# wustl-cig/FLAIR

Measured on AMD Instinct MI355X. Metric: restored frames/sec at 256x256, 16-frame clip, 250-step DDIM, higher is better.
Workload: dtype bf16

## Files before the change

flair_amd/csrc/chain.hip:

```cpp
#include <type_traits>

#include "common.h"
#include "mfma_tile.h"

namespace {

struct ChainArgs {
    const void* x[4];
    int segC[4], segLd[4], nseg;
    unsigned segBytes[4];
    const void* wA; const float* biasA; int actA; int CinA; unsigned wABytes;
    const void* wB; const float* biasB; int actB; int CoutB; unsigned wBBytes;
    const void* res0; const void* res1; int res0Ld, res1Ld;
    float outScale;
    float actParam; int actPeriod;
    void* y; int yLd;
    int T, H, W;
};

template <int N>
__device__ __forceinline__ void act_vec(float (&v)[N], int act) {
    if (act == FLAIR_ACT_SILU) {
#pragma unroll
        for (int e = 0; e < N; ++e) v[e] = silu_f(v[e]);
    } else if (act != FLAIR_ACT_NONE) {
        const float slope = act == FLAIR_ACT_RELU ? 0.f : 0.1f;
#pragma unroll
        for (int e = 0; e < N; ++e) v[e] = fmaxf(v[e], v[e] * slope);
    }
}

constexpr int CHAIN_MAX_COUTB = 512;

template <typename E, int C, int TH, int TW, bool HASA>
__global__ __launch_bounds__(512, 2) void conv_chain_kernel(ChainArgs a) {
    prefetch_kernargs<sizeof(ChainArgs)>();
    constexpr int NT = 512, NW = 8;
    constexpr int BKE = Mma<E>::BKE;
    constexpr int VEC = ET<E>::VEC;
    constexpr unsigned ESZ = sizeof(E);
    constexpr int PITCH = 80;
    constexpr int WM = TW + 2, RM = TH + 2, NPM = RM * WM;
    constexpr int WA = TW + 4, RA = TH + 4, NPA = RA * WA;
    constexpr int NCH = C / BKE;
    constexpr int NB = C / 64;
    constexpr int WROWS = 64 * NB;
    constexpr int MID_BYTES = NCH * NPM * PITCH;
    constexpr int W_BYTES = WROWS * 9 * PITCH;
    constexpr int NGA = (NPM + 31) / 32, NITA = NGA * NB, MAXIA = (NITA + NW - 1) / NW;
    constexpr int NGB = TH * TW / 32, NITB = NGB * NB, MAXIB = (NITB + NW - 1) / NW;
    constexpr int IN_PIECES = (HASA ? NPA : NCH * NPM) * 4;
    constexpr int HI = (IN_PIECES + NT - 1) / NT;
    constexpr int W_PIECES = WROWS * 9 * 4;
    constexpr int WI = (W_PIECES + NT - 1) / NT;
    static_assert(TH * TW % 32 == 0 && C % 64 == 0, "tile");
    extern __shared__ __attribute__((aligned(16))) char smem[];
    char* smid = smem;
    char* sw = smem + MID_BYTES;
    char* sin = sw + W_BYTES;
    float* sbias = reinterpret_cast<float*>(sin + (HASA ? NPA * PITCH : 0));

    const int tid = threadIdx.x, lane = tid & 63, wave = tid >> 6;
    const int lr = lane & 31, lh = lane >> 5;
    const int tilesW = a.W / TW, tilesH = (a.H + TH - 1) / TH;
    const int perFrame = tilesW * tilesH;
    const int bid = xcd_remap(blockIdx.x, gridDim.x);
    const int t = bid / perFrame;
    const int tile = bid % perFrame;
    const int h0 = (tile / tilesW) * TH, w0 = (tile % tilesW) * TW;
    const long frameOff = (long)t * a.H * a.W;
    for (int i = C + tid; i < C + CHAIN_MAX_COUTB; i += NT)
        sbias[i] = (a.biasB && i - C < a.CoutB) ? a.biasB[i - C] : 0.f;

    int ipix[HI], idst[HI];
    unsigned iq[HI];
#pragma unroll
    for (int i = 0; i < HI; ++i) {
        const int id = i * NT + tid;
        constexpr int NP = HASA ? NPA : NPM, WR = HASA ? WA : WM, ORG = HASA ? 2 : 1;
        const int pc = id >> 2;
        const int ch = HASA ? 0 : pc / NP;
        const int pix = HASA ? pc : pc % NP;
        const int r = pix / WR, c = pix % WR;
        const int hh = h0 - ORG + r, ww = w0 - ORG + c;
        const bool ok = id < IN_PIECES && (unsigned)hh < (unsigned)a.H && (unsigned)ww < (unsigned)a.W;
        ipix[i] = ok ? hh * a.W + ww : -1;
        iq[i] = (unsigned)(ch * BKE + (id & 3) * VEC) * ESZ;
        idst[i] = id < IN_PIECES ? (ch * NP + pix) * PITCH + (id & 3) * 16 : -1;
    }
    uint4 hreg[2][HI], wreg[2][WI];

    int seg = 0, cb = 0, segOff = 0;
    auto issue_in = [&](int set) {
        const unsigned ld = (unsigned)a.segLd[seg] * ESZ;
        const char* frame = reinterpret_cast<const char*>(a.x[seg]) + (size_t)frameOff * ld;
        const __amdgpu_buffer_rsrc_t xr = make_rsrc(frame, a.segBytes[seg]);
        const unsigned cofs = (unsigned)(cb * BKE) * ESZ;
#pragma unroll
        for (int i = 0; i < HI; ++i)
            hreg[set][i] = buf_load16(xr, ipix[i] >= 0 ? (unsigned)ipix[i] * ld + cofs + iq[i] : FLAIR_OOB);
    };
    auto advance_in = [&]() {
        ++cb;
        if (cb * BKE >= a.segC[seg]) {
            cb = 0;
            segOff += a.segC[seg];
            ++seg;
        }
    };
    auto issue_w = [&](int set, const __amdgpu_buffer_rsrc_t& wrs, int co0, int coutTot, int cin, int kofs) {
#pragma unroll
        for (int i = 0; i < WI; ++i) {
            const int id = i * NT + tid;
            const int row = id >> 2;
            const int co = row / 9, tap9 = row % 9;
            const bool ok = id < W_PIECES && co0 + co < coutTot;
            wreg[set][i] = buf_load16(wrs, ok ? (unsigned)(((co0 + co) * 9 + tap9) * cin + kofs + (id & 3) * VEC) * ESZ
                                              : FLAIR_OOB);
        }
    };
    auto write_w = [&](int set) {
#pragma unroll
        for (int i = 0; i < WI; ++i) {
            const int id = i * NT + tid;
            if (id < W_PIECES) *reinterpret_cast<uint4*>(sw + (id >> 2) * PITCH + (id & 3) * 16) = wreg[set][i];
        }
    };
    auto write_in = [&](char* dst, int set) {
#pragma unroll
        for (int i = 0; i < HI; ++i)
            if (idst[i] >= 0) *reinterpret_cast<uint4*>(dst + idst[i]) = hreg[set][i];
    };

    auto compute = [&](const char* pb, int inW, const char* wb0, const char* wb1, f32x16 (&acc)[2]) {
        uint4 fa0[2][2], fa1[2][2], fb[2][2];
        auto load_tap = [&](int set, int tap9) {
            const int kh = tap9 / 3, kw = tap9 % 3;
            fa0[set][0] = *reinterpret_cast<const uint4*>(wb0 + tap9 * PITCH + 16 * Mma<E>::chunk(0, lh));
            fa0[set][1] = *reinterpret_cast<const uint4*>(wb0 + tap9 * PITCH + 16 * Mma<E>::chunk(1, lh));
            fa1[set][0] = *reinterpret_cast<const uint4*>(wb1 + tap9 * PITCH + 16 * Mma<E>::chunk(0, lh));
            fa1[set][1] = *reinterpret_cast<const uint4*>(wb1 + tap9 * PITCH + 16 * Mma<E>::chunk(1, lh));
            const char* hp = pb + (kh * inW + kw) * PITCH;
            fb[set][0] = *reinterpret_cast<const uint4*>(hp + 16 * Mma<E>::chunk(0, lh));
            fb[set][1] = *reinterpret_cast<const uint4*>(hp + 16 * Mma<E>::chunk(1, lh));
        };
        load_tap(0, 0);
        __builtin_amdgcn_sched_group_barrier(0x100, 6, 0);
#pragma unroll
        for (int tap9 = 0; tap9 < 9; ++tap9) {
            const int set = tap9 & 1;
            if (tap9 < 8) load_tap(set ^ 1, tap9 + 1);
            Mma<E>::run(fa0[set], fb[set], acc[0]);
            Mma<E>::run(fa1[set], fb[set], acc[1]);
            if (tap9 < 8) __builtin_amdgcn_sched_group_barrier(0x100, 6, 0);
            __builtin_amdgcn_sched_group_barrier(0x8, 2 * Mma<E>::MFMA_PER_STEP, 0);
        }
    };

    const __amdgpu_buffer_rsrc_t wBrs = make_rsrc(a.wB, a.wBBytes);
    const int nBatch = (a.CoutB + WROWS - 1) / WROWS;

    if constexpr (HASA) {
        const __amdgpu_buffer_rsrc_t wArs = make_rsrc(a.wA, a.wABytes);
        const int nkA = a.CinA / BKE;
        auto issue_step = [&](int k, int set) {
            if (k < nkA) {
                issue_in(set);
                issue_w(set, wArs, 0, C, a.CinA, segOff + cb * BKE);
                advance_in();
            } else if (k == nkA) {
                issue_w(set, wBrs, 0, a.CoutB, C, 0);
            }
        };
        issue_step(0, 0);
        issue_step(1, 1);
        f32x16 accA[MAXIA][2];
        int pbOff[MAXIA], wbOff[MAXIA];
#pragma unroll
        for (int ii = 0; ii < MAXIA; ++ii) {
            const int it = wave + ii * NW;
            const int g = it % NGA, blk = (it / NGA) % NB;
            int q = g * 32 + lr;
            if (q >= NPM) q = NPM - 1;
            pbOff[ii] = ((q / WM) * WA + (q % WM)) * PITCH;
            wbOff[ii] = ((blk * 64 + lr) * 9) * PITCH;
#pragma unroll
            for (int i = 0; i < 2; ++i)
#pragma unroll
                for (int gq = 0; gq < 4; ++gq) {
                    float4 bq = make_float4(0.f, 0.f, 0.f, 0.f);
                    if (a.biasA) bq = *reinterpret_cast<const float4*>(a.biasA + blk * 64 + i * 32 + 8 * gq + 4 * lh);
                    accA[ii][i][4 * gq] = bq.x; accA[ii][i][4 * gq + 1] = bq.y;
                    accA[ii][i][4 * gq + 2] = bq.z; accA[ii][i][4 * gq + 3] = bq.w;
                }
        }
        write_in(sin, 0);
        write_w(0);
        __syncthreads();
        auto step = [&](int k, auto setTag) {
            constexpr int SET = decltype(setTag)::value;
            issue_step(k + 2, SET);
#pragma unroll
            for (int ii = 0; ii < MAXIA; ++ii)
                if (wave + ii * NW < NITA)
                    compute(sin + pbOff[ii], WA, sw + wbOff[ii], sw + wbOff[ii] + 32 * 9 * PITCH, accA[ii]);
            __syncthreads();
            if (k + 1 < nkA) write_in(sin, SET ^ 1);
            write_w(SET ^ 1);
            if (k + 1 < nkA) __syncthreads();
        };
        for (int k = 0; k < nkA; k += 2) {
            step(k, std::integral_constant<int, 0>{});
            if (k + 1 < nkA) step(k + 1, std::integral_constant<int, 1>{});
        }
#pragma unroll
        for (int ii = 0; ii < MAXIA; ++ii) {
            const int it = wave + ii * NW;
            if (it >= NITA) continue;
            const int g = it % NGA, blk = (it / NGA) % NB;
            const int q = g * 32 + lr;
            if (q >= NPM) continue;
            const int hh = h0 - 1 + q / WM, ww = w0 - 1 + q % WM;
            const bool inimg = (unsigned)hh < (unsigned)a.H && (unsigned)ww < (unsigned)a.W;
#pragma unroll
            for (int i = 0; i < 2; ++i)
#pragma unroll
                for (int gq = 0; gq < 4; ++gq) {
                    const int co = blk * 64 + i * 32 + 8 * gq + 4 * lh;
                    float v[4] = {accA[ii][i][4 * gq], accA[ii][i][4 * gq + 1], accA[ii][i][4 * gq + 2],
                                  accA[ii][i][4 * gq + 3]};
                    act_vec<4>(v, a.actA);
                    char* dst = smid + ((co / BKE) * NPM + q) * PITCH + (co % BKE) * ESZ;
                    if constexpr (sizeof(E) == 4) {
                        *reinterpret_cast<float4*>(dst) = inimg ? make_float4(v[0], v[1], v[2], v[3])
                                                                : make_float4(0.f, 0.f, 0.f, 0.f);
                    } else {
                        uint2 pk;
                        pk.x = inimg ? pack2bf(v[0], v[1]) : 0u;
                        pk.y = inimg ? pack2bf(v[2], v[3]) : 0u;
                        *reinterpret_cast<uint2*>(dst) = pk;
                    }
                }
        }
        __syncthreads();
    } else {
        issue_in(0);
        issue_w(0, wBrs, 0, a.CoutB, C, 0);
        write_in(smid, 0);
        write_w(0);
        __syncthreads();
    }

    int pbB[MAXIB], wbB[MAXIB];
#pragma unroll
    for (int ii = 0; ii < MAXIB; ++ii) {
        const int it = wave + ii * NW;
        const int g = it % NGB, blk = it / NGB;
        const int q = g * 32 + lr;
        pbB[ii] = ((q / TW) * WM + (q % TW)) * PITCH;
        wbB[ii] = ((blk * 64 + lr) * 9) * PITCH;
    }
    for (int batch = 0; batch < nBatch; ++batch) {
        f32x16 acc[MAXIB][2];
#pragma unroll
        for (int ii = 0; ii < MAXIB; ++ii) {
            const int blk = ((wave + ii * NW) / NGB) % NB;
#pragma unroll
            for (int i = 0; i < 2; ++i)
#pragma unroll
                for (int gq = 0; gq < 4; ++gq) {
                    const float4 bq = *reinterpret_cast<const float4*>(sbias + C + batch * WROWS + blk * 64 + i * 32 +
                                                                       8 * gq + 4 * lh);
                    acc[ii][i][4 * gq] = bq.x; acc[ii][i][4 * gq + 1] = bq.y;
                    acc[ii][i][4 * gq + 2] = bq.z; acc[ii][i][4 * gq + 3] = bq.w;
                }
        }
        for (int ch = 0; ch < NCH; ++ch) {
            const bool lastChunk = ch + 1 == NCH;
            const bool more = !lastChunk || batch + 1 < nBatch;
            if (more) issue_w(0, wBrs, lastChunk ? (batch + 1) * WROWS : batch * WROWS, a.CoutB, C, lastChunk ? 0 : (ch + 1) * BKE);
#pragma unroll
            for (int ii = 0; ii < MAXIB; ++ii)
                if (wave + ii * NW < NITB)
                    compute(smid + ch * NPM * PITCH + pbB[ii], WM, sw + wbB[ii], sw + wbB[ii] + 32 * 9 * PITCH, acc[ii]);
            __syncthreads();
            if (!lastChunk) {
                write_w(0);
                __syncthreads();
            }
        }
#pragma unroll
        for (int ii = 0; ii < MAXIB; ++ii) {
            const int it = wave + ii * NW;
            if (it >= NITB) continue;
            const int g = it % NGB, blk = it / NGB;
            const int q = g * 32 + lr;
            const int hh = h0 + q / TW, ww = w0 + q % TW;
            const long p = frameOff + (long)hh * a.W + ww;
#pragma unroll
            for (int i = 0; i < 2; ++i) {
                const int cofrag = batch * WROWS + blk * 64 + i * 32;
                if constexpr (sizeof(E) == 4) {
#pragma unroll
                    for (int gq = 0; gq < 4; ++gq) {
                        const int co = cofrag + 8 * gq + 4 * lh;
                        float v[4] = {acc[ii][i][4 * gq], acc[ii][i][4 * gq + 1], acc[ii][i][4 * gq + 2], acc[ii][i][4 * gq + 3]};
                        if (a.actB == FLAIR_ACT_DCN_OFFSETS)
                            dcn_offset_act<4>(v, co, a.actParam, a.actPeriod);
                        else
                            act_vec<4>(v, a.actB);
                        if (co < a.CoutB && hh < a.H) {
                            if (a.res0) add_piece<E>(v, reinterpret_cast<const E*>(a.res0) + p * a.res0Ld + co);
                            if (a.res1) add_piece<E>(v, reinterpret_cast<const E*>(a.res1) + p * a.res1Ld + co);
#pragma unroll
                            for (int e = 0; e < VEC; ++e) v[e] *= a.outScale;
                            Vec16<E>::store(reinterpret_cast<E*>(a.y) + p * a.yLd + co, v);
                        }
                    }
                } else {
#pragma unroll
                    for (int j = 0; j < 2; ++j) {
// ... 358 lines not shown
#pragma unroll
                for (int cf = 0; cf < 2; ++cf)
#pragma unroll
                    for (int ks = 0; ks < 2; ++ks)
                        accA[1][cf] = __builtin_amdgcn_mfma_f32_32x32x16_bf16(__builtin_bit_cast(bf16x8, fa[set][cf][ks]), __builtin_bit_cast(bf16x8, fb[set][1][ks]), accA[1][cf], 0, 0, 0);
            }
        }
    };

    asm volatile("s_waitcnt vmcnt(%0)" ::"n"(NH + NWS) : "memory");
    __builtin_amdgcn_s_barrier();
    init_from_bias(accA[0], sbias);
    init_from_bias(accA[1], sbias);
    compute_A(0, 0);
    asm volatile("s_waitcnt vmcnt(0)" ::: "memory");
    __builtin_amdgcn_s_barrier();
    issue_w(wBdesc, 0, 0);
    compute_A(1, 1);
    __builtin_amdgcn_s_barrier();
    issue_w(wBdesc, 1, 1);

    {
        const float slopeA = a.actA == FLAIR_ACT_NONE ? 1.f : a.actA == FLAIR_ACT_RELU ? 0.f : 0.1f;
#pragma unroll
        for (int ii = 0; ii < 2; ++ii) {
            if (ii == 1 && !two) break;
            const int qraw = (wave + ii * NW) * 32 + lr;
            const int hh = h0 - 1 + qr_[ii], ww = w0 - 1 + qc_[ii];
            const bool inimg = (unsigned)hh < (unsigned)a.H && (unsigned)ww < (unsigned)a.W;
            const unsigned sw = (unsigned)((qc_[ii] >> 2) & 3);
#pragma unroll
            for (int cf = 0; cf < 2; ++cf)
#pragma unroll
                for (int jj = 0; jj < 2; ++jj) {
                    float v[8];
                    acc_octet(accA[ii][cf], jj, v);
#pragma unroll
                    for (int e = 0; e < 8; ++e) v[e] = inimg ? fmaxf(v[e], v[e] * slopeA) : 0.f;
                    alignas(16) E out[8];
                    Vec16<E>::store(out, v);
                    if (qraw < NPMID)
                        *reinterpret_cast<uint4*>(smem + cf * MID_IMG + q_[ii] * 64 + (((2 * jj + lh) ^ sw) << 4)) = *reinterpret_cast<const uint4*>(out);
                }
        }
    }

    const long prow = ((long)t * a.H + h0 + wave) * a.W + w0;
    const unsigned yLdB = (unsigned)a.yLd * 2u, r0LdB = (unsigned)a.res0Ld * 2u, r1LdB = (unsigned)a.res1Ld * 2u;
    const __amdgpu_buffer_rsrc_t yd = make_rsrc(reinterpret_cast<char*>(a.y) + prow * a.yLd * 2, (unsigned)a.W * yLdB);
    const __amdgpu_buffer_rsrc_t r0d = make_rsrc(a.res0 ? reinterpret_cast<const char*>(a.res0) + prow * a.res0Ld * 2 : nullptr, a.res0 ? (unsigned)a.W * r0LdB : 0u);
    const __amdgpu_buffer_rsrc_t r1d = make_rsrc(a.res1 ? reinterpret_cast<const char*>(a.res1) + prow * a.res1Ld * 2 : nullptr, a.res1 ? (unsigned)a.W * r1LdB : 0u);
    uint4 r0v[4], r1v[4];
#pragma unroll
    for (int g = 0; g < 4; ++g) r0v[g] = r1v[g] = make_uint4(0u, 0u, 0u, 0u);
    const int nres = (a.res0 ? 4 : 0) + (a.res1 ? 4 : 0);
    if (a.res0) {
#pragma unroll
        for (int g = 0; g < 4; ++g) r0v[g] = buf_load16(r0d, (unsigned)lr * r0LdB + (unsigned)(32 * g + 16 * lh));
    }
    if (a.res1) {
#pragma unroll
        for (int g = 0; g < 4; ++g) r1v[g] = buf_load16(r1d, (unsigned)lr * r1LdB + (unsigned)(32 * g + 16 * lh));
    }
    unsigned aoffB[2], boffB[3][2];
    dma_frag_offsets(lr, lh, wave * WMID, aoffB, boffB);
    f32x16 accB[2];
    auto compute_B = [&](int slot, int ch) { dma_tap_loop(smem + RING + slot * SLOT, smem + ch * MID_IMG, aoffB, boffB, accB, dma_no_hook{}); };
    if (nres == 0) asm volatile("s_waitcnt vmcnt(%0) lgkmcnt(0)" ::"n"(NWS) : "memory");
    else if (nres == 4) asm volatile("s_waitcnt vmcnt(%0) lgkmcnt(0)" ::"n"(NWS + 4) : "memory");
    else asm volatile("s_waitcnt vmcnt(%0) lgkmcnt(0)" ::"n"(NWS + 8) : "memory");
    __builtin_amdgcn_s_barrier();
    init_from_bias(accB, sbias + 256);
    compute_B(0, 0);
    if (nres == 0) asm volatile("s_waitcnt vmcnt(0)" ::: "memory");
    else if (nres == 4) asm volatile("s_waitcnt vmcnt(4)" ::: "memory");
    else asm volatile("s_waitcnt vmcnt(8)" ::: "memory");
    __builtin_amdgcn_s_barrier();
    compute_B(1, 1);

    const float slopeB = a.actB == FLAIR_ACT_NONE ? 1.f : a.actB == FLAIR_ACT_RELU ? 0.f : 0.1f;
    const float scale = a.outScale;
#pragma unroll
    for (int cf = 0; cf < 2; ++cf)
#pragma unroll
        for (int jj = 0; jj < 2; ++jj) {
            const int g = 2 * cf + jj;
            float v[8];
            acc_octet(accB[cf], jj, v);
            leaky_act(v, slopeB);
            add_piece<E>(v, r0v[g]);
            add_piece<E>(v, r1v[g]);
#pragma unroll
            for (int e = 0; e < 8; ++e) v[e] *= scale;
            store_piece(yd, pack_piece<E>(v), (unsigned)lr * yLdB + (unsigned)(32 * g + 16 * lh));
        }
}

int launch_pair(const ChainArgs& c, hipStream_t s) {
    PairArgs a;
    a.x = c.x[0]; a.xLd = c.segLd[0]; a.xBytes = c.segBytes[0];
    a.wA = c.wA; a.wB = c.wB; a.wBytes = 64u * 9u * 64u * 2u;
    a.biasA = c.biasA; a.biasB = c.biasB; a.actA = c.actA; a.actB = c.actB; a.outScale = c.outScale;
    a.res0 = c.res0; a.res1 = c.res1; a.res0Ld = c.res0Ld; a.res1Ld = c.res1Ld;
    a.y = c.y; a.yLd = c.yLd; a.T = c.T; a.H = c.H; a.W = c.W;
    constexpr size_t lds = 2 * 27 * 1024 + 2 * 36 * 1024 + 2048;
    static LdsAttrOnce attr;
    const hipError_t e = flair_max_lds_once(attr, reinterpret_cast<const void*>(&conv_pair_kernel));
    FLAIR_CHECK(e == hipSuccess, "flair_conv_chain: hipFuncSetAttribute: %s", hipGetErrorString(e));
    hipLaunchKernelGGL(conv_pair_kernel, dim3(c.T * (c.H / 8) * (c.W / 32)), dim3(512), lds, s, a);
    FLAIR_LAUNCH_CHECK();
    return FLAIR_OK;
}

template <typename E, int C, int TH, int TW, bool HASA>
int launch_chain(const ChainArgs& a, hipStream_t s) {
    constexpr int BKE = Mma<E>::BKE;
    constexpr size_t lds = (size_t)(C / BKE) * (TH + 2) * (TW + 2) * 80 + (size_t)C * 9 * 80 +
                           (HASA ? (size_t)(TH + 4) * (TW + 4) * 80 : 0) + (size_t)(C + CHAIN_MAX_COUTB) * 4;
    static_assert(lds <= 160 * 1024, "LDS budget");
    static LdsAttrOnce attr;
    {
        const hipError_t e = flair_max_lds_once(attr, reinterpret_cast<const void*>(&conv_chain_kernel<E, C, TH, TW, HASA>));
        FLAIR_CHECK(e == hipSuccess, "flair_conv_chain: hipFuncSetAttribute: %s", hipGetErrorString(e));
    }
    const int grid = a.T * cdiv(a.H, TH) * (a.W / TW);
    hipLaunchKernelGGL((conv_chain_kernel<E, C, TH, TW, HASA>), dim3(grid), dim3(512), lds, s, a);
    FLAIR_LAUNCH_CHECK();
    return FLAIR_OK;
}

template <typename E, bool HASA>
int dispatch_chain(const ChainArgs& a, int C, hipStream_t s) {
    constexpr int TALL = sizeof(E) == 4 ? 4 : 8;
    const bool wide = a.W % 32 == 0 && (long)a.T * cdiv(a.H, TALL) * (a.W / 32) >= 192;
    if (C == 64) return wide ? launch_chain<E, 64, TALL, 32, HASA>(a, s) : launch_chain<E, 64, TALL, 8, HASA>(a, s);
    return launch_chain<E, 128, TALL, 8, HASA>(a, s);
}

}

extern "C" int flair_conv_chain(const flair_chain_params* p, const void* const* x, const void* wA, const float* biasA,
                                const void* wB, const float* biasB, const void* res0, const void* res1, void* y,
                                hipStream_t stream) {
    FLAIR_CHECK(p && x && wB && y, "flair_conv_chain: null argument");
    FLAIR_CHECK_DTYPE("flair_conv_chain", p->dtype);
    FLAIR_CHECK(p->nseg >= 1 && p->nseg <= 4, "flair_conv_chain: nseg %d not in 1..4", p->nseg);
    FLAIR_CHECK(p->T > 0 && p->H > 0 && p->W > 0, "flair_conv_chain: empty shape");
    FLAIR_CHECK(p->C == 64 || p->C == 128, "flair_conv_chain: intermediate width %d unsupported (64 or 128)", p->C);
    FLAIR_CHECK(p->W % 8 == 0, "flair_conv_chain: W %% 8 must be 0 (got %d x %d)", p->H, p->W);
    const int esz = p->dtype == FLAIR_BF16 ? 2 : 4, bke = p->dtype == FLAIR_BF16 ? 32 : 16;
    FLAIR_CHECK(p->CoutB > 0 && p->CoutB % (16 / esz) == 0 && p->CoutB <= CHAIN_MAX_COUTB,
                "flair_conv_chain: CoutB %d must be a multiple of %d and at most %d", p->CoutB, 16 / esz, CHAIN_MAX_COUTB);
    ChainArgs a{};
    int cin = 0;
    for (int i = 0; i < p->nseg; ++i) {
        FLAIR_CHECK(x[i], "flair_conv_chain: segment %d is null", i);
        FLAIR_CHECK(p->seg_c[i] > 0 && p->seg_c[i] % bke == 0, "flair_conv_chain: segment %d has %d channels; must be a "
                    "multiple of %d", i, p->seg_c[i], bke);
        FLAIR_CHECK(p->seg_ld[i] >= p->seg_c[i] && (p->seg_ld[i] * esz) % 16 == 0 && ((uintptr_t)x[i]) % 16 == 0,
                    "flair_conv_chain: segment %d stride/alignment", i);
        const unsigned long long bytes = (unsigned long long)p->H * p->W * p->seg_ld[i] * esz;
        FLAIR_CHECK(bytes < 0x40000000ull, "flair_conv_chain: one frame of segment %d spans %llu bytes (limit 1 GiB)", i, bytes);
        a.x[i] = x[i]; a.segC[i] = p->seg_c[i]; a.segLd[i] = p->seg_ld[i]; a.segBytes[i] = (unsigned)bytes;
        cin += p->seg_c[i];
    }
    a.nseg = p->nseg;
    const bool hasA = wA != nullptr;
    FLAIR_CHECK(hasA || (p->nseg == 1 && cin == p->C), "flair_conv_chain: without stage A the single input must have C channels");
    a.wA = wA; a.biasA = biasA; a.actA = p->actA; a.CinA = cin;
    a.wABytes = (unsigned)((unsigned long long)p->C * 9 * cin * esz);
    a.wB = wB; a.biasB = biasB; a.actB = p->actB; a.CoutB = p->CoutB;
    {
        const unsigned long long wb = (unsigned long long)p->CoutB * 9 * p->C * esz;
        FLAIR_CHECK(wb < 0x80000000ull, "flair_conv_chain: stage-B weights span %llu bytes", wb);
        a.wBBytes = (unsigned)wb;
    }
    FLAIR_CHECK(((uintptr_t)wB) % 16 == 0 && (!wA || ((uintptr_t)wA) % 16 == 0), "flair_conv_chain: weight alignment");
    FLAIR_CHECK_VIEW("flair_conv_chain", "y", y, p->y_ld, p->CoutB, 16 / esz);
    if (res0) FLAIR_CHECK_VIEW("flair_conv_chain", "res0", res0, p->res_ld[0], p->CoutB, 16 / esz);
    if (res1) FLAIR_CHECK_VIEW("flair_conv_chain", "res1", res1, p->res_ld[1], p->CoutB, 16 / esz);
    a.res0 = res0; a.res1 = res1; a.res0Ld = p->res_ld[0]; a.res1Ld = p->res_ld[1];
    a.outScale = p->out_scale;
    a.actParam = p->act_param; a.actPeriod = p->act_period;
    FLAIR_CHECK(p->actA != FLAIR_ACT_DCN_OFFSETS && (p->actB != FLAIR_ACT_DCN_OFFSETS ||
                                                       (p->act_period > 0 && p->act_period % 24 == 0)),
                "flair_conv_chain: FLAIR_ACT_DCN_OFFSETS is a stage-B activation with act_period = 3 * deform_groups");
    {
        auto plain = [](int c) { return c == FLAIR_ACT_NONE || c == FLAIR_ACT_RELU || c == FLAIR_ACT_LRELU01 || c == FLAIR_ACT_SILU; };
        FLAIR_CHECK(plain(p->actA) && (plain(p->actB) || p->actB == FLAIR_ACT_DCN_OFFSETS),
                    "flair_conv_chain: activation codes (%d, %d) unsupported: NONE / RELU / LRELU01 / SILU (+ DCN_OFFSETS for stage B)",
                    p->actA, p->actB);
    }
    a.y = y; a.yLd = p->y_ld;
    a.T = p->T; a.H = p->H; a.W = p->W;
    if (!hasA && p->dtype == FLAIR_BF16 && p->C == 64 && p->W % 32 == 0 && p->H % 8 == 0 && !res0 && !res1 &&
        (p->y_ld * 2) % 16 == 0 && p->CoutB % 8 == 0 &&
        (unsigned long long)p->H * p->W * p->y_ld * 2 < 0x40000000ull)
        return launch_resident(a, stream);
    {
        auto lin = [](int c) { return c == FLAIR_ACT_NONE || c == FLAIR_ACT_RELU || c == FLAIR_ACT_LRELU01; };
        if (hasA && p->dtype == FLAIR_BF16 && p->C == 64 && p->nseg == 1 && cin == 64 && p->CoutB == 64 && p->W % 32 == 0 &&
            p->H % 8 == 0 && lin(p->actA) && lin(p->actB) && (unsigned long long)p->H * p->W * p->y_ld * 2 < 0x40000000ull &&
            (!res0 || (unsigned long long)p->H * p->W * p->res_ld[0] * 2 < 0x40000000ull) &&
            (!res1 || (unsigned long long)p->H * p->W * p->res_ld[1] * 2 < 0x40000000ull))
            return launch_pair(a, stream);
    }
    if (p->dtype == FLAIR_BF16)
        return hasA ? dispatch_chain<bf16_t, true>(a, p->C, stream) : dispatch_chain<bf16_t, false>(a, p->C, stream);
    return hasA ? dispatch_chain<float, true>(a, p->C, stream) : dispatch_chain<float, false>(a, p->C, stream);
}
```

flair_amd/csrc/conv.hip:

```cpp
#include <type_traits>

#include "common.h"
#include "mfma_tile.h"

namespace {

struct ConvArgs {
    const void* x[4];
    int segC[4];
    int segLd[4];
    int nseg;
    const void* w;
    const float* bias;
    const void* res0;
    const void* res1;
    int res0Ld, res1Ld;
    void* y;
    int yLd;
    int T, H, W;
    int KT, KH, KW;
    int Cout, CinTot;
    int act;
    float outScale;
    long P;
    int nPixTiles, nCoTiles;
    int tFast;
    unsigned segBytes[4];
    unsigned wBytes;
    float* part;
    int splitK;
    const float* fbias;
    int fbiasLd;
    int stride;
    int tapShift;
    int reflect;
    float actParam;
    int actPeriod;
    int Hin, Win;
    int esz;
};

__device__ __forceinline__ int lds_off(int row, int chunk) {
    return row * 64 + ((chunk ^ ((row >> 2) & 3)) << 4);
}

__device__ __forceinline__ int staged_row(int id) {
    const int g = id >> 3;
    return (g >> 2) * 8 + (g & 3) + 4 * ((id >> 2) & 1);
}

template <typename E>
__device__ __forceinline__ void store_quad(const ConvArgs& a, long p, int co, float v0, float v1, float v2, float v3) {
    if (co >= a.Cout) return;
    float v[4] = {v0, v1, v2, v3};
    if (a.bias) {
        const float4 b = *reinterpret_cast<const float4*>(a.bias + co);
        v[0] += b.x; v[1] += b.y; v[2] += b.z; v[3] += b.w;
    }
    if (a.fbias) {
        const float* fb = a.fbias + (p / ((long)a.H * a.W)) * a.fbiasLd + co;
        v[0] += fb[0]; v[1] += fb[1]; v[2] += fb[2]; v[3] += fb[3];
    }
    if (a.act == FLAIR_ACT_DCN_OFFSETS) {
        dcn_offset_act<4>(v, co, a.actParam, a.actPeriod);
    } else {
#pragma unroll
        for (int e = 0; e < 4; ++e) v[e] = apply_act(v[e], a.act);
    }
    const E* r0 = reinterpret_cast<const E*>(a.res0);
    const E* r1 = reinterpret_cast<const E*>(a.res1);
    if (r0) {
#pragma unroll
        for (int e = 0; e < 4; ++e) v[e] += ET<E>::ld(r0 + p * a.res0Ld + co + e);
    }
    if (r1) {
#pragma unroll
        for (int e = 0; e < 4; ++e) v[e] += ET<E>::ld(r1 + p * a.res1Ld + co + e);
    }
#pragma unroll
    for (int e = 0; e < 4; ++e) v[e] *= a.outScale;
    E* dst = reinterpret_cast<E*>(a.y) + p * a.yLd + co;
    if constexpr (sizeof(E) == 4) {
        *reinterpret_cast<float4*>(dst) = make_float4(v[0], v[1], v[2], v[3]);
    } else {
        uint2 pk;
        pk.x = pack2bf(v[0], v[1]);
        pk.y = pack2bf(v[2], v[3]);
        *reinterpret_cast<uint2*>(dst) = pk;
    }
}

template <typename E, int ACT, int FC, int FP>
__device__ __forceinline__ void igemm_epilogue(const ConvArgs& a, const f32x16 (&acc)[FC][FP], long pbase, int cobase, int lr, int lh) {
    constexpr unsigned ESZ = sizeof(E);
    constexpr int VEC = ET<E>::VEC, NV = 8 / VEC;
    const float slope = leaky_slope(a.act);
    const unsigned yLdB = (unsigned)a.yLd * ESZ, r0LdB = (unsigned)a.res0Ld * ESZ, r1LdB = (unsigned)a.res1Ld * ESZ;
    constexpr unsigned SPAN = FP * 32;
    const __amdgpu_buffer_rsrc_t yd = make_rsrc(reinterpret_cast<char*>(a.y) + ((size_t)pbase * a.yLd + cobase) * ESZ, SPAN * yLdB);
    const __amdgpu_buffer_rsrc_t r0d = make_rsrc(reinterpret_cast<const char*>(a.res0) + (a.res0 ? ((size_t)pbase * a.res0Ld + cobase) * ESZ : 0),
                                                 a.res0 ? SPAN * r0LdB : 0u);
    const __amdgpu_buffer_rsrc_t r1d = make_rsrc(reinterpret_cast<const char*>(a.res1) + (a.res1 ? ((size_t)pbase * a.res1Ld + cobase) * ESZ : 0),
                                                 a.res1 ? SPAN * r1LdB : 0u);
    const int coLeft = a.Cout - cobase;
    const __amdgpu_buffer_rsrc_t bd = make_rsrc(a.bias ? a.bias + cobase : nullptr, a.bias && coLeft > 0 ? (unsigned)coLeft * 4u : 0u);
    const long hw = (long)a.H * a.W;
#pragma unroll
    for (int j = 0; j < FP; ++j) {
        const long p = pbase + j * 32 + lr;
        const bool pvalid = p < a.P;
        const unsigned pl = (unsigned)(j * 32 + lr);
        const float* fbrow = a.fbias ? a.fbias + (pvalid ? p / hw : 0) * a.fbiasLd + cobase : nullptr;
#pragma unroll
        for (int i = 0; i < FC; ++i) {
            uint4 bq[2][2], r0v[2][NV], r1v[2][NV], fq[2][2];
#pragma unroll
            for (int jj = 0; jj < 2; ++jj) {
                const int cw = i * 32 + 16 * jj + 8 * lh;
                const bool ok = pvalid && cw < coLeft;
                bq[jj][0] = buf_load16(bd, 4u * (unsigned)cw);
                bq[jj][1] = buf_load16(bd, 4u * (unsigned)cw + 16u);
#pragma unroll
                for (int q = 0; q < NV; ++q) {
                    r0v[jj][q] = buf_load16(r0d, ok ? pl * r0LdB + (unsigned)(cw + q * VEC) * ESZ : FLAIR_OOB);
                    r1v[jj][q] = buf_load16(r1d, ok ? pl * r1LdB + (unsigned)(cw + q * VEC) * ESZ : FLAIR_OOB);
                }
                fq[jj][0] = fq[jj][1] = make_uint4(0u, 0u, 0u, 0u);
            }
            if (a.fbias) {
#pragma unroll
                for (int jj = 0; jj < 2; ++jj) {
                    const int cw = i * 32 + 16 * jj + 8 * lh;
                    const float* fp = fbrow + (cw < coLeft ? cw : 0);
                    fq[jj][0] = *reinterpret_cast<const uint4*>(fp);
                    fq[jj][1] = *reinterpret_cast<const uint4*>(fp + 4);
                }
            }
#pragma unroll
            for (int jj = 0; jj < 2; ++jj) {
                float v[8];
                acc_octet(acc[i][j], jj, v);
                const int cw = i * 32 + 16 * jj + 8 * lh;
                const bool ok = pvalid && cw < coLeft;
                {
                    const uint4 b0 = bq[jj][0], b1 = bq[jj][1], f0 = fq[jj][0], f1 = fq[jj][1];
                    v[0] += __uint_as_float(b0.x) + __uint_as_float(f0.x); v[1] += __uint_as_float(b0.y) + __uint_as_float(f0.y);
                    v[2] += __uint_as_float(b0.z) + __uint_as_float(f0.z); v[3] += __uint_as_float(b0.w) + __uint_as_float(f0.w);
                    v[4] += __uint_as_float(b1.x) + __uint_as_float(f1.x); v[5] += __uint_as_float(b1.y) + __uint_as_float(f1.y);
                    v[6] += __uint_as_float(b1.z) + __uint_as_float(f1.z); v[7] += __uint_as_float(b1.w) + __uint_as_float(f1.w);
                }
                if constexpr (ACT == 0) {
                    leaky_act(v, slope);
                } else if constexpr (ACT == 1) {
                    dcn_offset_act<8>(v, cobase + cw, a.actParam, a.actPeriod);
                } else if constexpr (ACT == 2) {
#pragma unroll
                    for (int e = 0; e < 8; ++e) v[e] = silu_f(v[e]);
                } else {
#pragma unroll
                    for (int e = 0; e < 8; ++e) v[e] = 0.5f * v[e] * (1.f + erff(v[e] * 0.70710678118654752f));
                }
                add_piece<E>(v, r0v[jj][0]);
                add_piece<E>(v, r1v[jj][0]);
                if constexpr (NV == 2) {
                    add_piece<E, VEC>(v, r0v[jj][1]);
                    add_piece<E, VEC>(v, r1v[jj][1]);
                }
#pragma unroll
                for (int e = 0; e < 8; ++e) v[e] *= a.outScale;
#pragma unroll
                for (int q = 0; q < NV; ++q)
                    store_piece(yd, pack_piece<E>(v + q * VEC), ok ? pl * yLdB + (unsigned)(cw + q * VEC) * ESZ : FLAIR_OOB);
            }
        }
    }
}

template <typename E, int TH>
__global__ __launch_bounds__(64 * TH, (2 * 64 * TH + 255) / 256)
void conv3x3_halo_kernel(ConvArgs a) {
    prefetch_kernargs<sizeof(ConvArgs)>();
    constexpr int RPW = 1, PF = 1;
    constexpr int BKE = Mma<E>::BKE;
    constexpr int VEC = ET<E>::VEC;
    constexpr int NT = 64 * TH / RPW;
    constexpr int HW_ = 34;
    constexpr int PITCH = 80;
    constexpr int HALO_ROWS = (TH + 2) * HW_;
    constexpr int HALO_PIECES = (HALO_ROWS + 7) / 8 * 8 * 4;
    constexpr int W_PIECES = 64 * 9 * 4;
    constexpr int HI = (HALO_PIECES + NT - 1) / NT;
    constexpr int WI = (W_PIECES + NT - 1) / NT;
    constexpr int HALO_BYTES = (TH + 2) * HW_ * PITCH;
    extern __shared__ __attribute__((aligned(16))) char smem[];
    char* sh = smem;
    char* sw = smem + HALO_BYTES;

    const int tid = threadIdx.x, lane = tid & 63, wave = tid >> 6;
    const int lr = lane & 31, lh = lane >> 5;
    const int bid = xcd_remap(blockIdx.x, gridDim.x);
    const int coTile = bid % a.nCoTiles;
    int rest = bid / a.nCoTiles;
    const int tilesW = a.W / 32, tilesH = (a.H + TH - 1) / TH;
    const int tw = rest % tilesW;
    rest /= tilesW;
    const int th = rest % tilesH;
    const int t = rest / tilesH;
    const int h0 = th * TH, w0 = tw * 32, co0 = coTile * 64;
    const int taps = a.KT * 9;
    const int pt = a.KT / 2;

    uint4 hreg[PF][HI], wreg[PF][WI];
    int dt = -pt, seg = 0, cb = 0, segOff = 0;
    auto dt_valid = [&](int d) { return (unsigned)(t + d) < (unsigned)a.T; };
    while (dt <= pt && !dt_valid(dt)) ++dt;

    constexpr unsigned ESZ = sizeof(E);
    int hpix[HI];
    unsigned hq[HI], woff[WI];
#pragma unroll
    for (int i = 0; i < HI; ++i) {
        const int id = i * NT + tid;
        const int pix = staged_row(id);
        const int r = pix / HW_, c = pix % HW_;
        const int hh = h0 + r - 1, ww = w0 + c - 1;
        const bool ok = pix < HALO_ROWS && (unsigned)hh < (unsigned)a.H && (unsigned)ww < (unsigned)a.W;
        hpix[i] = ok ? hh * a.W + ww : -1;
        hq[i] = (id & 3) * VEC * ESZ;
    }
    const __amdgpu_buffer_rsrc_t wrs = make_rsrc(a.w, a.wBytes);
#pragma unroll
    for (int i = 0; i < WI; ++i) {
        const int id = i * NT + tid;
        const int row = staged_row(id);
        const int co = row / 9, tap9 = row % 9;
        const bool ok = id < W_PIECES && co0 + co < a.Cout;
        woff[i] = ok ? (unsigned)(((co0 + co) * taps + tap9) * a.CinTot + (id & 3) * VEC) * ESZ : FLAIR_OOB;
    }

    auto issue = [&](uint4 (&hr)[HI], uint4 (&wr)[WI]) {
        const unsigned ld = (unsigned)a.segLd[seg] * ESZ;
        const char* frame = reinterpret_cast<const char*>(a.x[seg]) + (size_t)(t + dt) * a.H * a.W * ld;
        const __amdgpu_buffer_rsrc_t xr = make_rsrc(frame, a.segBytes[seg]);
        const unsigned cofs = (unsigned)(cb * BKE) * ESZ;
#pragma unroll
        for (int i = 0; i < HI; ++i) {
            const unsigned off = hpix[i] >= 0 ? (unsigned)hpix[i] * ld + cofs + hq[i] : FLAIR_OOB;
            hr[i] = buf_load16(xr, off);
        }
        const unsigned kofs = (unsigned)((dt + pt) * 9 * a.CinTot + segOff + cb * BKE) * ESZ;
#pragma unroll
        for (int i = 0; i < WI; ++i) wr[i] = buf_load16(wrs, woff[i] == FLAIR_OOB ? FLAIR_OOB : woff[i] + kofs);
    };
    auto advance = [&]() {
        ++cb;
        if (cb * BKE >= a.segC[seg]) {
            cb = 0;
            segOff += a.segC[seg];
            if (++seg >= a.nseg) {
                seg = 0;
                segOff = 0;
                ++dt;
                while (dt <= pt && !dt_valid(dt)) ++dt;
            }
        }
    };
    auto write_lds = [&](const uint4 (&hr)[HI], const uint4 (&wr)[WI]) {
#pragma unroll
        for (int i = 0; i < HI; ++i) {
            const int id = i * NT + tid;
            const int row = staged_row(id);
            if (row < HALO_ROWS) *reinterpret_cast<uint4*>(sh + row * PITCH + (id & 3) * 16) = hr[i];
        }
#pragma unroll
        for (int i = 0; i < WI; ++i) {
            const int id = i * NT + tid;
            if (id < W_PIECES) *reinterpret_cast<uint4*>(sw + staged_row(id) * PITCH + (id & 3) * 16) = wr[i];
        }
    };
    int nValidDt = 0;
    for (int d = -pt; d <= pt; ++d) nValidDt += dt_valid(d) ? 1 : 0;
    const int nch = nValidDt * (a.CinTot / BKE);

    f32x16 acc[RPW][2];
#pragma unroll
    for (int j = 0; j < RPW; ++j)
#pragma unroll
        for (int i = 0; i < 2; ++i)
#pragma unroll
            for (int r = 0; r < 16; ++r) acc[j][i][r] = 0.f;

    auto compute = [&]() {
        const char* hb = sh + ((wave * RPW * HW_) + lr) * PITCH;
        const char* wb0 = sw + (lr * 9) * PITCH;
        const char* wb1 = sw + ((lr + 32) * 9) * PITCH;
        uint4 fa0[2][2], fa1[2][2], fb[2][RPW][2];
        auto load_tap = [&](int set, int tap9) {
            const int kh = tap9 / 3, kw = tap9 % 3;
            fa0[set][0] = *reinterpret_cast<const uint4*>(wb0 + tap9 * PITCH + 16 * Mma<E>::chunk(0, lh));
            fa0[set][1] = *reinterpret_cast<const uint4*>(wb0 + tap9 * PITCH + 16 * Mma<E>::chunk(1, lh));
            fa1[set][0] = *reinterpret_cast<const uint4*>(wb1 + tap9 * PITCH + 16 * Mma<E>::chunk(0, lh));
            fa1[set][1] = *reinterpret_cast<const uint4*>(wb1 + tap9 * PITCH + 16 * Mma<E>::chunk(1, lh));
#pragma unroll
            for (int j = 0; j < RPW; ++j) {
                const char* hp = hb + ((j + kh) * HW_ + kw) * PITCH;
                fb[set][j][0] = *reinterpret_cast<const uint4*>(hp + 16 * Mma<E>::chunk(0, lh));
                fb[set][j][1] = *reinterpret_cast<const uint4*>(hp + 16 * Mma<E>::chunk(1, lh));
            }
        };
        load_tap(0, 0);
        __builtin_amdgcn_sched_group_barrier(0x100, 4 + 2 * RPW, 0);
#pragma unroll
        for (int tap9 = 0; tap9 < 9; ++tap9) {
            const int set = tap9 & 1;
            if (tap9 < 8) load_tap(set ^ 1, tap9 + 1);
#pragma unroll
            for (int j = 0; j < RPW; ++j) {
                Mma<E>::run(fa0[set], fb[set][j], acc[j][0]);
                Mma<E>::run(fa1[set], fb[set][j], acc[j][1]);
            }
            if (tap9 < 8) __builtin_amdgcn_sched_group_barrier(0x100, 4 + 2 * RPW, 0);
            __builtin_amdgcn_sched_group_barrier(0x8, (sizeof(E) == 2 ? 4 : 16) * RPW, 0);
        }
    };

    int issued = 0;
#pragma unroll
    for (int s_ = 0; s_ < PF; ++s_)
        if (issued < nch) {
            issue(hreg[s_], wreg[s_]);
            advance();
            ++issued;
        }
    write_lds(hreg[0], wreg[0]);
    __syncthreads();
    for (int k = 0; k < nch; k += PF) {
#pragma unroll
        for (int par = 0; par < PF; ++par) {
            const int kk = k + par;
            if (kk < nch) {
                if (issued < nch) {
                    issue(hreg[par], wreg[par]);
                    advance();
                    ++issued;
                }
                compute();
                if (kk + 1 < nch) {
                    __syncthreads();
                    write_lds(hreg[(par + 1) % PF], wreg[(par + 1) % PF]);
                    __syncthreads();
                }
            }
        }
    }

    if ((a.Cout & 7) == 0) {
        constexpr int VEC = ET<E>::VEC;
        constexpr int CHUNKS = 64 / VEC;
        __syncthreads();
#pragma unroll
        for (int j = 0; j < RPW; ++j) {
            char* tile = smem + (wave * RPW + j) * 32 * (64 * 4 + 16);
#pragma unroll
            for (int i = 0; i < 2; ++i)
#pragma unroll
                for (int g = 0; g < 4; ++g)
                    *reinterpret_cast<float4*>(tile + lr * (64 * 4 + 16) + (i * 32 + 8 * g + 4 * lh) * 4) =
                        make_float4(acc[j][i][4 * g], acc[j][i][4 * g + 1], acc[j][i][4 * g + 2],
                                    acc[j][i][4 * g + 3]);
        }
        __syncthreads();
        constexpr int FPITCH = 64 * 4 + 16;
#pragma unroll
        for (int j = 0; j < RPW; ++j) {
            const int h = h0 + wave * RPW + j;
            if (h >= a.H) continue;
            const char* tile = smem + (wave * RPW + j) * 32 * FPITCH;
            const long prow = ((long)t * a.H + h) * a.W + w0;
#pragma unroll
            for (int it = 0; it < 32 * CHUNKS / 64; ++it) {
                const int id = it * 64 + lane;
                const int px = id / CHUNKS, ch = id % CHUNKS;
                const int co = co0 + ch * VEC;
                if (co >= a.Cout) continue;
                const long p = prow + px;
                float v[VEC];
                const float* src = reinterpret_cast<const float*>(tile + px * FPITCH) + ch * VEC;
#pragma unroll
                for (int e = 0; e < VEC; e += 4) {
                    const float4 q = *reinterpret_cast<const float4*>(src + e);
                    v[e] = q.x; v[e + 1] = q.y; v[e + 2] = q.z; v[e + 3] = q.w;
                }
                if (a.bias) {
#pragma unroll
                    for (int e = 0; e < VEC; ++e) v[e] += a.bias[co + e];
                }
                if (a.fbias) {
                    const float* fb = a.fbias + (long)t * a.fbiasLd + co;
#pragma unroll
                    for (int e = 0; e < VEC; ++e) v[e] += fb[e];
                }
                if (a.act == FLAIR_ACT_DCN_OFFSETS) {
                    dcn_offset_act<VEC>(v, co, a.actParam, a.actPeriod);
                } else {
#pragma unroll
                    for (int e = 0; e < VEC; ++e) v[e] = apply_act(v[e], a.act);
                }
                if (a.res0) {
                    float r[VEC];
                    Vec16<E>::load(reinterpret_cast<const E*>(a.res0) + p * a.res0Ld + co, r);
#pragma unroll
                    for (int e = 0; e < VEC; ++e) v[e] += r[e];
                }
                if (a.res1) {
                    float r[VEC];
                    Vec16<E>::load(reinterpret_cast<const E*>(a.res1) + p * a.res1Ld + co, r);
#pragma unroll
                    for (int e = 0; e < VEC; ++e) v[e] += r[e];
                }
#pragma unroll
                for (int e = 0; e < VEC; ++e) v[e] *= a.outScale;
                Vec16<E>::store(reinterpret_cast<E*>(a.y) + p * a.yLd + co, v);
            }
        }
        return;
    }
#pragma unroll
    for (int j = 0; j < RPW; ++j) {
        const int h = h0 + wave * RPW + j, w = w0 + lr;
        if (h >= a.H) continue;
        const long p = ((long)t * a.H + h) * a.W + w;
#pragma unroll
        for (int i = 0; i < 2; ++i)
#pragma unroll
            for (int g = 0; g < 4; ++g)
                store_quad<E>(a, p, co0 + i * 32 + 8 * g + 4 * lh, acc[j][i][4 * g], acc[j][i][4 * g + 1],
                              acc[j][i][4 * g + 2], acc[j][i][4 * g + 3]);
    }
}

template <typename E, int TH>
int launch_halo(const ConvArgs& a0, hipStream_t s) {
    ConvArgs a = a0;
    a.nCoTiles = cdiv(a.Cout, 64);
    const int grid = a.T * cdiv(a.H, TH) * (a.W / 32) * a.nCoTiles;
    const size_t lds = (size_t)(TH + 2) * 34 * 80 + 64 * 9 * 80;
    hipLaunchKernelGGL((conv3x3_halo_kernel<E, TH>), dim3(grid), dim3(64 * TH), lds, s, a);
    FLAIR_LAUNCH_CHECK();
    return FLAIR_OK;
}

template <typename E, int TH>
__global__ __launch_bounds__(128 * TH, (128 * TH) / 256) void conv3x3_halo_ks_kernel(ConvArgs a) {
    prefetch_kernargs<sizeof(ConvArgs)>();
    constexpr int NW = 2 * TH;
    constexpr int NT = 64 * NW;
    constexpr int BKE = Mma<E>::BKE;
    constexpr int VEC = ET<E>::VEC;
    constexpr unsigned ESZ = sizeof(E);
    constexpr int HW_ = 34, PITCH = 80;
    constexpr int HALO_ROWS = (TH + 2) * HW_;
    constexpr int HALO_PIECES = (HALO_ROWS + 7) / 8 * 8 * 4;
    constexpr int W_PIECES = 64 * 9 * 4;
    constexpr int HI = (HALO_PIECES + NT - 1) / NT;
    constexpr int WI = (W_PIECES + NT - 1) / NT;
    constexpr int HALO_BYTES = (TH + 2) * HW_ * PITCH;
    constexpr int STAGE_BYTES = HALO_BYTES + 64 * 9 * PITCH;
    constexpr int FPITCH = 64 * 4 + 16;
    constexpr int CHUNKS = 64 / VEC;
    extern __shared__ __attribute__((aligned(16))) char smem[];

    const int tid = threadIdx.x, lane = tid & 63, wave = tid >> 6;
    const int lr = lane & 31, lh = lane >> 5;
    const int rp = wave % TH, kh2 = (wave / TH) & 1;
    const int bid = xcd_remap(blockIdx.x, gridDim.x);
    const int coTile = bid % a.nCoTiles;
    int rest = bid / a.nCoTiles;
    const int tilesW = a.W / 32, tilesH = (a.H + TH - 1) / TH;
    const int tw = rest % tilesW;
    rest /= tilesW;
    const int th = rest % tilesH;
    const int t = rest / tilesH;
    const int h0 = th * TH, w0 = tw * 32, co0 = coTile * 64;
    const int taps = a.KT * 9;
    const int pt = a.KT / 2;

    float biasv[VEC];
    {
        const int bco = co0 + (lane % (64 / VEC)) * VEC;
#pragma unroll
        for (int e = 0; e < VEC; ++e) biasv[e] = (a.bias && bco < a.Cout) ? a.bias[bco + e] : 0.f;
    }
    uint4 hreg[HI], wreg[WI];
    int dt = -pt, seg = 0, cb = 0, segOff = 0;
    auto dt_valid = [&](int d) { return (unsigned)(t + d) < (unsigned)a.T; };
    while (dt <= pt && !dt_valid(dt)) ++dt;

    int hpix[HI];
    unsigned hq[HI], woff[WI];
#pragma unroll
    for (int i = 0; i < HI; ++i) {
        const int id = i * NT + tid;
        const int pix = staged_row(id);
        const int r = pix / HW_, c = pix % HW_;
        const int hh = h0 + r - 1, ww = w0 + c - 1;
        const bool ok = pix < HALO_ROWS && (unsigned)hh < (unsigned)a.H && (unsigned)ww < (unsigned)a.W;
        hpix[i] = ok ? hh * a.W + ww : -1;
        hq[i] = (id & 3) * VEC * ESZ;
    }
    const __amdgpu_buffer_rsrc_t wrs = make_rsrc(a.w, a.wBytes);
#pragma unroll
    for (int i = 0; i < WI; ++i) {
        const int id = i * NT + tid;
        const int row = staged_row(id);
        const int co = row / 9, tap9 = row % 9;
        const bool ok = id < W_PIECES && co0 + co < a.Cout;
        woff[i] = ok ? (unsigned)(((co0 + co) * taps + tap9) * a.CinTot + (id & 3) * VEC) * ESZ : FLAIR_OOB;
    }
    auto issue = [&]() {
        const unsigned ld = (unsigned)a.segLd[seg] * ESZ;
        const char* frame = reinterpret_cast<const char*>(a.x[seg]) + (size_t)(t + dt) * a.H * a.W * ld;
        const __amdgpu_buffer_rsrc_t xr = make_rsrc(frame, a.segBytes[seg]);
        const unsigned cofs = (unsigned)(cb * BKE) * ESZ;
#pragma unroll
        for (int i = 0; i < HI; ++i)
            hreg[i] = buf_load16(xr, hpix[i] >= 0 ? (unsigned)hpix[i] * ld + cofs + hq[i] : FLAIR_OOB);
        const unsigned kofs = (unsigned)((dt + pt) * 9 * a.CinTot + segOff + cb * BKE) * ESZ;
#pragma unroll
        for (int i = 0; i < WI; ++i) wreg[i] = buf_load16(wrs, woff[i] == FLAIR_OOB ? FLAIR_OOB : woff[i] + kofs);
        ++cb;
        if (cb * BKE >= a.segC[seg]) {
            cb = 0;
            segOff += a.segC[seg];
            if (++seg >= a.nseg) {
                seg = 0;
                segOff = 0;
                ++dt;
                while (dt <= pt && !dt_valid(dt)) ++dt;
            }
        }
    };
    auto write_lds = [&](int stage) {
        char* sh = smem + stage * STAGE_BYTES;
        char* sw = sh + HALO_BYTES;
#pragma unroll
        for (int i = 0; i < HI; ++i) {
            const int id = i * NT + tid;
            const int row = staged_row(id);
            if (row < HALO_ROWS) *reinterpret_cast<uint4*>(sh + row * PITCH + (id & 3) * 16) = hreg[i];
        }
#pragma unroll
        for (int i = 0; i < WI; ++i) {
            const int id = i * NT + tid;
            if (id < W_PIECES) *reinterpret_cast<uint4*>(sw + staged_row(id) * PITCH + (id & 3) * 16) = wreg[i];
        }
    };
    int nValidDt = 0;
    for (int d = -pt; d <= pt; ++d) nValidDt += dt_valid(d) ? 1 : 0;
    const int nch = nValidDt * (a.CinTot / BKE);

    f32x16 acc[2];
#pragma unroll
    for (int i = 0; i < 2; ++i)
#pragma unroll
        for (int r = 0; r < 16; ++r) acc[i][r] = 0.f;

    const int ck = 16 * Mma<E>::chunk(kh2, lh);
    auto compute = [&](int stage) {
        const char* sh = smem + stage * STAGE_BYTES;
        const char* hb = sh + ((rp * HW_) + lr) * PITCH + ck;
        const char* wb0 = sh + HALO_BYTES + (lr * 9) * PITCH + ck;
        uint4 fa[2][2], fb[2];
        auto load_tap = [&](int set, int tap9) {
            const int kh = tap9 / 3, kw = tap9 % 3;
#pragma unroll
            for (int i = 0; i < 2; ++i)
                fa[set][i] = *reinterpret_cast<const uint4*>(wb0 + (i * 32 * 9 + tap9) * PITCH);
            fb[set] = *reinterpret_cast<const uint4*>(hb + (kh * HW_ + kw) * PITCH);
        };
        load_tap(0, 0);
        __builtin_amdgcn_sched_group_barrier(0x100, 3, 0);
#pragma unroll
        for (int tap9 = 0; tap9 < 9; ++tap9) {
            const int set = tap9 & 1;
            if (tap9 < 8) load_tap(set ^ 1, tap9 + 1);
#pragma unroll
            for (int i = 0; i < 2; ++i) Mma<E>::run1(fa[set][i], fb[set], acc[i]);
            if (tap9 < 8) __builtin_amdgcn_sched_group_barrier(0x100, 3, 0);
            __builtin_amdgcn_sched_group_barrier(0x8, 2 * Mma<E>::MFMA_PER_HALF, 0);
        }
    };

    issue();
    write_lds(0);
    if (nch > 1) issue();
    __syncthreads();
    for (int k = 0; k < nch; ++k) {
        compute(k & 1);
        if (k + 1 < nch) {
            write_lds((k + 1) & 1);
            if (k + 2 < nch) issue();
            __syncthreads();
        }
    }

    constexpr int PARTS = NW / TH;
    constexpr int NIT = 32 * CHUNKS / 64 / PARTS;
    const int orow = wave % TH, part = wave / TH;
    const int h = h0 + orow;
    const long prow = ((long)t * a.H + h) * a.W + w0;
    const int ech = lane % CHUNKS;
    const int eco = co0 + ech * VEC;
    const bool eok = h < a.H && eco < a.Cout;
    uint4 r0v[NIT], r1v[NIT];
#pragma unroll
    for (int k = 0; k < NIT; ++k) {
        const int px = ((k * PARTS + part) * 64 + lane) / CHUNKS;
        const long p = prow + px;
        r0v[k] = r1v[k] = make_uint4(0u, 0u, 0u, 0u);
        if (eok && a.res0) r0v[k] = *reinterpret_cast<const uint4*>(reinterpret_cast<const E*>(a.res0) + p * a.res0Ld + eco);
        if (eok && a.res1) r1v[k] = *reinterpret_cast<const uint4*>(reinterpret_cast<const E*>(a.res1) + p * a.res1Ld + eco);
    }
    __syncthreads();
#pragma unroll
    for (int pass = 0; pass < 2; ++pass) {
        if (kh2 == pass) {
            char* tile = smem + rp * 32 * FPITCH + lr * FPITCH;
#pragma unroll
            for (int i = 0; i < 2; ++i)
#pragma unroll
                for (int g = 0; g < 4; ++g) {
                    float4* dst = reinterpret_cast<float4*>(tile + (i * 32 + 8 * g + 4 * lh) * 4);
                    float4 v = make_float4(acc[i][4 * g], acc[i][4 * g + 1], acc[i][4 * g + 2], acc[i][4 * g + 3]);
                    if (pass == 1) {
                        const float4 o = *dst;
                        v.x += o.x; v.y += o.y; v.z += o.z; v.w += o.w;
                    }
                    *dst = v;
                }
        }
        __syncthreads();
    }
    if (!eok) return;
    const float slope = leaky_slope(a.act);
    const bool leaky = a.act == FLAIR_ACT_NONE || a.act == FLAIR_ACT_RELU || a.act == FLAIR_ACT_LRELU01 || a.act == FLAIR_ACT_LRELU02;
    const char* tile = smem + orow * 32 * FPITCH;
#pragma unroll
    for (int k = 0; k < NIT; ++k) {
        const int px = ((k * PARTS + part) * 64 + lane) / CHUNKS;
        const long p = prow + px;
        float v[VEC];
        const float* src = reinterpret_cast<const float*>(tile + px * FPITCH) + ech * VEC;
#pragma unroll
        for (int e = 0; e < VEC; e += 4) {
            const float4 q = *reinterpret_cast<const float4*>(src + e);
            v[e] = q.x; v[e + 1] = q.y; v[e + 2] = q.z; v[e + 3] = q.w;
        }
#pragma unroll
        for (int e = 0; e < VEC; ++e) v[e] += biasv[e];
        if (a.fbias) {
            const float* fb = a.fbias + (long)t * a.fbiasLd + eco;
#pragma unroll
            for (int e = 0; e < VEC; ++e) v[e] += fb[e];
        }
        if (leaky) {
            leaky_act(v, slope);
        } else if (a.act == FLAIR_ACT_DCN_OFFSETS) {
            dcn_offset_act<VEC>(v, eco, a.actParam, a.actPeriod);
        } else if (a.act == FLAIR_ACT_SILU) {
#pragma unroll
            for (int e = 0; e < VEC; ++e) v[e] = silu_f(v[e]);
        } else {
#pragma unroll
            for (int e = 0; e < VEC; ++e) v[e] = apply_act(v[e], a.act);
        }
        if (a.res0) add_piece<E>(v, r0v[k]);
        if (a.res1) add_piece<E>(v, r1v[k]);
#pragma unroll
        for (int e = 0; e < VEC; ++e) v[e] *= a.outScale;
        Vec16<E>::store(reinterpret_cast<E*>(a.y) + p * a.yLd + eco, v);
    }
}

template <typename E, int TH>
int launch_halo_ks(const ConvArgs& a0, hipStream_t s) {
    ConvArgs a = a0;
    a.nCoTiles = cdiv(a.Cout, 64);
    const int grid = a.T * cdiv(a.H, TH) * (a.W / 32) * a.nCoTiles;
    const size_t lds = 2 * ((size_t)(TH + 2) * 34 * 80 + 64 * 9 * 80);
    static LdsAttrOnce attr;
    {
        const hipError_t e = flair_max_lds_once(attr, reinterpret_cast<const void*>(&conv3x3_halo_ks_kernel<E, TH>));
        FLAIR_CHECK(e == hipSuccess, "flair_conv_nhwc: hipFuncSetAttribute: %s", hipGetErrorString(e));
    }
    hipLaunchKernelGGL((conv3x3_halo_ks_kernel<E, TH>), dim3(grid), dim3(128 * TH), lds, s, a);
    FLAIR_LAUNCH_CHECK();
    return FLAIR_OK;
}

struct DmaTile {
    int t, h0, w0, co0;
};

template <int RPW>
__device__ __forceinline__ void conv3x3_dma_body(const ConvArgs& a, int nTiles, int tilesPerXcd) {
    using E = bf16_t;
    static_assert(RPW == 1 || RPW == 2, "the clip-level and one-tile forms");
    constexpr int NW = 8, NSTAGE = 2;
    constexpr int KSTEPS = 2;
    constexpr int TH = NW * RPW, HWP = 34;
    constexpr int HALO_ROWS = (TH + 2) * HWP;
    constexpr int HALO_INSTR = (HALO_ROWS + 15) / 16;
    constexpr int W_INSTR = 64 * 9 / 16;
    constexpr int HALO_BYTES = HALO_INSTR * 1024;
    constexpr int STAGE_BYTES = HALO_BYTES + W_INSTR * 1024;
    constexpr int NSLOT = (HALO_INSTR + W_INSTR + NW - 1) / NW;
    constexpr int BIAS_OFF = NSTAGE * STAGE_BYTES + NW * 1024;
    extern __shared__ __attribute__((aligned(16))) char smem[];

    const int tid = threadIdx.x, lane = tid & 63;
    const int wave = __builtin_amdgcn_readfirstlane(tid >> 6);
    const int lr = lane & 31, lh = lane >> 5;
    const int taps = a.KT * 9, pt = a.KT / 2;
    const int chunksPerTap = a.CinTot / 32;
    const int H = a.H, W = a.W, T = a.T;

    const int xcd = blockIdx.x & 7, slot = blockIdx.x >> 3, slotsPerXcd = gridDim.x >> 3;
    const int tilesW = W / 32, tilesH = H / TH, nCoTiles = a.nCoTiles;
    auto tile_at = [&](int i, DmaTile& tl) -> bool {
        const int inXcd = slot + i * slotsPerXcd;
        const int id = xcd * tilesPerXcd + inXcd;
        if (inXcd >= tilesPerXcd || id >= nTiles) return false;
        int rest = id;
        tl.co0 = (rest % nCoTiles) * 64;
        rest /= nCoTiles;
        if (a.tFast) {
            tl.t = rest % T;
            rest /= T;
            tl.w0 = (rest % tilesW) * 32;
            tl.h0 = (rest / tilesW) * TH;
            return true;
        }
        tl.w0 = (rest % tilesW) * 32;
        rest /= tilesW;
        tl.h0 = (rest % tilesH) * TH;
        tl.t = rest / tilesH;
        return true;
    };

    const int lrow = lane >> 2, lchunk = lane & 3;
    unsigned slotv[NSLOT], hchunk[NSLOT];
#pragma unroll
    for (int i = 0; i < NSLOT; ++i) {
        const int id = wave * NSLOT + i;
        const int c = (id * 16 + lrow) % HWP;
        hchunk[i] = (unsigned)((lchunk ^ ((c >> 2) & 3)) << 4);
    }
    auto setup_tile = [&](const DmaTile& tl) {
#pragma unroll
        for (int i = 0; i < NSLOT; ++i) {
            const int id = wave * NSLOT + i;
            const int R = id * 16 + lrow;
            const int hr = R / HWP, c = R - hr * HWP;
            const int hh = tl.h0 - 1 + hr, ww = tl.w0 - 1 + c;
            const bool okh = R < HALO_ROWS && (unsigned)hh < (unsigned)H && (unsigned)ww < (unsigned)W;
            const unsigned hv = okh ? (unsigned)(hh * W + ww) : 0xffffffffu;
            const int row = R - HALO_INSTR * 16;
            const int tap9 = row >> 6, co = row & 63;
            const bool okw = row >= 0 && row < 576 && tl.co0 + co < a.Cout;
            const unsigned wv = okw ? (unsigned)(((tl.co0 + co) * taps + tap9) * a.CinTot) * 2u + ((lchunk ^ ((co >> 2) & 3)) << 4) : FLAIR_OOB;
            slotv[i] = id >= HALO_INSTR ? wv : hv;
        }
    };

    const u32x4_t wdesc = make_desc(a.w, a.wBytes);
    struct Walk {
        int dt, seg, cb, segOff, j;
    };
    auto dt_at = [&](int t, int j) { return a.tFast ? (j + a.KT * T - t) % a.KT - pt : j - pt; };
    auto walk_first = [&](int t, Walk& wk) {
        wk.j = 0; wk.seg = 0; wk.cb = 0; wk.segOff = 0;
        while (wk.j < a.KT && (unsigned)(t + dt_at(t, wk.j)) >= (unsigned)T) ++wk.j;
        wk.dt = dt_at(t, wk.j);
    };
    auto walk_next = [&](int t, Walk& wk) {
        ++wk.cb;
        if (wk.cb * 32 >= a.segC[wk.seg]) {
            wk.cb = 0;
            wk.segOff += a.segC[wk.seg];
            if (++wk.seg >= a.nseg) {
                wk.seg = 0;
                wk.segOff = 0;
                ++wk.j;
                while (wk.j < a.KT && (unsigned)(t + dt_at(t, wk.j)) >= (unsigned)T) ++wk.j;
                wk.dt = dt_at(t, wk.j);
            }
        }
    };
    auto chunks_of = [&](int t) {
        int n = 0;
        for (int d = -pt; d <= pt; ++d) n += (unsigned)(t + d) < (unsigned)T ? 1 : 0;
        return n * chunksPerTap;
    };
    auto issue = [&](const DmaTile& tl, const Walk& wk, int stage) {
        const unsigned ld = (unsigned)a.segLd[wk.seg] * 2u;
        const char* frame = reinterpret_cast<const char*>(a.x[wk.seg]) + (size_t)(tl.t + wk.dt) * H * W * ld;
        const u32x4_t xdesc = make_desc(frame, a.segBytes[wk.seg]);
        const unsigned cofs = (unsigned)(wk.cb * 64);
        const unsigned kofs = (unsigned)((wk.dt + pt) * 9 * a.CinTot + wk.segOff + wk.cb * 32) * 2u;
        const unsigned sbase = (unsigned)(stage * STAGE_BYTES + wave * NSLOT * 1024);
#pragma unroll
        for (int i = 0; i < NSLOT; ++i) {
            const bool isw = wave * NSLOT + i >= HALO_INSTR;
            const unsigned sv = slotv[i];
            const unsigned offh = sv == 0xffffffffu ? FLAIR_OOB : sv * ld + cofs + hchunk[i];
            const unsigned offw = sv == FLAIR_OOB ? FLAIR_OOB : sv + kofs;
            u32x4_t d;
            d.x = isw ? wdesc.x : xdesc.x;
            d.y = isw ? wdesc.y : xdesc.y;
            d.z = isw ? wdesc.z : xdesc.z;
            d.w = 0x00020000u;
            const bool idle = wave * NSLOT + i >= HALO_INSTR + W_INSTR;
            dma16(d, isw ? offw : offh, idle ? (unsigned)(NSTAGE * STAGE_BYTES + ((wave * NSLOT + i - HALO_INSTR - W_INSTR) % NW) * 1024) : sbase + i * 1024);
        }
    };

    unsigned aoff[KSTEPS], boff[3][KSTEPS];
#pragma unroll
    for (int s_ = 0; s_ < KSTEPS; ++s_) {
        aoff[s_] = (unsigned)(HALO_BYTES + lr * 64 + (((2 * s_ + lh) ^ ((lr >> 2) & 3)) << 4));
#pragma unroll
        for (int kw = 0; kw < 3; ++kw)
            boff[kw][s_] = (unsigned)((RPW * wave * HWP + kw + lr) * 64 + (((2 * s_ + lh) ^ (((kw + lr) >> 2) & 3)) << 4));
    }

    f32x16 acc[RPW][2];
    auto zero_acc = [&]() {
#pragma unroll
        for (int j = 0; j < RPW; ++j)
#pragma unroll
            for (int i = 0; i < 2; ++i)
#pragma unroll
                for (int r = 0; r < 16; ++r) acc[j][i][r] = 0.f;
    };
    auto compute = [&](int stage) {
        const char* sb = smem + stage * STAGE_BYTES;
        uint4 fb[2][RPW + 2][KSTEPS];
        uint4 fa[2][2][KSTEPS];
        auto load_b = [&](int set, int kw) {
#pragma unroll
            for (int h = 0; h < RPW + 2; ++h)
#pragma unroll
                for (int s_ = 0; s_ < KSTEPS; ++s_)
                    fb[set][h][s_] = *reinterpret_cast<const uint4*>(sb + h * (HWP * 64) + boff[kw][s_]);
        };
        auto load_a = [&](int set, int kh, int kw) {
#pragma unroll
            for (int cf = 0; cf < 2; ++cf)
#pragma unroll
                for (int s_ = 0; s_ < KSTEPS; ++s_)
                    fa[set][cf][s_] = *reinterpret_cast<const uint4*>(sb + (kh * 3 + kw) * 4096 + cf * 2048 + aoff[s_]);
        };
        load_b(0, 0);
        load_a(0, 0, 0);
        __builtin_amdgcn_sched_group_barrier(0x100, KSTEPS * (RPW + 2) + 2 * KSTEPS, 0);
#pragma unroll
        for (int step = 0; step < 9; ++step) {
            const int kq = step / 3, kh = step % 3;
            const int nkq = (step + 1) / 3, nkh = (step + 1) % 3;
            if (step < 8) {
                if (nkh == 0) load_b(nkq & 1, nkq);
                load_a((step + 1) & 1, nkh, nkq);
            }
#pragma unroll
            for (int j = 0; j < RPW; ++j)
#pragma unroll
                for (int cf = 0; cf < 2; ++cf) Mma<E>::run(fa[step & 1][cf], fb[kq & 1][j + kh], acc[j][cf]);
            if (step < 8) {
                if (nkh == 0) __builtin_amdgcn_sched_group_barrier(0x100, KSTEPS * (RPW + 2) + 2 * KSTEPS, 0);
                else __builtin_amdgcn_sched_group_barrier(0x100, 2 * KSTEPS, 0);
            }
            __builtin_amdgcn_sched_group_barrier(0x8, 2 * KSTEPS * RPW, 0);
        }
    };
    auto epilogue_as = [&](const DmaTile& tl, int biasSlot, auto actTag, auto resTag) {
        constexpr int ACT = decltype(actTag)::value;
        constexpr bool HASRES = decltype(resTag)::value;
        const float slope = leaky_slope(a.act);
        const long p0w = ((long)tl.t * H + tl.h0 + RPW * wave) * W + tl.w0;
        const int cl = 8 * lh;
        const unsigned yLdB = (unsigned)a.yLd * 2u, rLdB = (unsigned)a.res0Ld * 2u;
        const unsigned span = (unsigned)(RPW * W);
        const __amdgpu_buffer_rsrc_t yd = make_rsrc(reinterpret_cast<char*>(a.y) + (p0w * a.yLd + tl.co0) * 2, span * yLdB);
        const __amdgpu_buffer_rsrc_t r0d = make_rsrc(reinterpret_cast<const char*>(a.res0) + (a.res0 ? (p0w * a.res0Ld + tl.co0) * 2 : 0),
                                                     a.res0 ? span * rLdB : 0u);
        const E* r1b = a.res1 ? reinterpret_cast<const E*>(a.res1) + (p0w + lr) * a.res1Ld + tl.co0 + cl : nullptr;
        const float* bl = reinterpret_cast<const float*>(smem + BIAS_OFF + (biasSlot & 1) * 256) + cl;
        const float scale = a.outScale;
        const unsigned yLane = (unsigned)lr * yLdB + 2u * cl, rLane = (unsigned)lr * rLdB + 2u * cl;
        uint4 r0v[2][2][RPW];
        auto res_request = [&](int i) {
#pragma unroll
            for (int jj = 0; jj < 2; ++jj) {
                const int cofs = i * 32 + 16 * jj;
                const bool lane_ok = tl.co0 + cofs + cl < a.Cout;
#pragma unroll
                for (int j = 0; j < RPW; ++j)
                    r0v[i][jj][j] = buf_load16(r0d, lane_ok ? rLane + (unsigned)(j * W) * rLdB + 2u * cofs : FLAIR_OOB);
            }
        };
        if constexpr (HASRES) {
            res_request(0);
            res_request(1);
        }
#pragma unroll
        for (int i = 0; i < 2; ++i) {
#pragma unroll
            for (int jj = 0; jj < 2; ++jj) {
                const int cofs = i * 32 + 16 * jj;
                const bool lane_ok = tl.co0 + cofs + cl < a.Cout;
                float bv[8];
                {
                    const float4 b0 = *reinterpret_cast<const float4*>(bl + cofs);
                    const float4 b1 = *reinterpret_cast<const float4*>(bl + cofs + 4);
                    bv[0] = b0.x; bv[1] = b0.y; bv[2] = b0.z; bv[3] = b0.w; bv[4] = b1.x; bv[5] = b1.y; bv[6] = b1.z; bv[7] = b1.w;
                }
#pragma unroll
                for (int j = 0; j < RPW; ++j) {
                    float v[8];
#pragma unroll
                    for (int e = 0; e < 4; ++e) {
                        const auto sw2 = __builtin_amdgcn_permlane32_swap(__float_as_uint(acc[j][i][8 * jj + e]),
                                                                          __float_as_uint(acc[j][i][8 * jj + 4 + e]), false, false);
                        v[e] = __uint_as_float(sw2[0]) + bv[e];
                        v[4 + e] = __uint_as_float(sw2[1]) + bv[4 + e];
                    }
                    if constexpr (ACT == 0) {
#pragma unroll
                        for (int e = 0; e < 8; ++e) v[e] = fmaxf(v[e], v[e] * slope);
                    } else if constexpr (ACT == 1) {
                        dcn_offset_act_fast<8>(v, tl.co0 + cofs + cl, a.actParam, a.actPeriod, 1.f);
                    } else if constexpr (ACT == 2) {
#pragma unroll
                        for (int e = 0; e < 8; ++e) v[e] *= __builtin_amdgcn_rcpf(1.f + __expf(-v[e]));
                    }
                    if constexpr (HASRES) {
                        float r[8];
                        Vec16<E>::load(reinterpret_cast<const E*>(&r0v[i][jj][j]), r);
#pragma unroll
                        for (int e = 0; e < 8; ++e) v[e] += r[e];
                        if (r1b && lane_ok) {
                            Vec16<E>::load(r1b + (long)j * W * a.res1Ld + cofs, r);
#pragma unroll
                            for (int e = 0; e < 8; ++e) v[e] += r[e];
                        }
                    }
                    if constexpr (ACT != 3) {
#pragma unroll
                        for (int e = 0; e < 8; ++e) v[e] *= scale;
                    }
                    alignas(16) E out[8];
                    Vec16<E>::store(out, v);
// ... 43 lines not shown
                    } else if constexpr (ACT == 1) {
                        dcn_offset_act<8>(v, tl.co0 + cofs + cl, a.actParam, a.actPeriod);
                    } else {
#pragma unroll
                        for (int e = 0; e < 8; ++e) v[e] = silu_f(v[e]);
                    }
                    const long ro = (long)j * W;
                    if (r0b && lane_ok) add_piece<E>(v, r0b + ro * a.res0Ld + cofs);
                    if (r1b && lane_ok) add_piece<E>(v, r1b + ro * a.res1Ld + cofs);
#pragma unroll
                    for (int e = 0; e < 8; ++e) v[e] *= scale;
                    if (!lane_ok) continue;
                    Vec16<E>::store(yb + ro * a.yLd + cofs, v);
                }
            }
    };
    auto epilogue = [&](const DmaTile& tl, int biasSlot) {
        const bool res = a.res0 || a.res1;
        auto go = [&](auto actTag) {
            if constexpr (RPW == 1) {
                epilogue_plain_as(tl, biasSlot, actTag);
            } else {
                if (res) epilogue_as(tl, biasSlot, actTag, std::true_type{});
                else epilogue_as(tl, biasSlot, actTag, std::false_type{});
            }
        };
        if (a.act == FLAIR_ACT_DCN_OFFSETS) go(std::integral_constant<int, 1>{});
        else if (a.act == FLAIR_ACT_SILU) go(std::integral_constant<int, 2>{});
        else if (RPW >= 2 && a.act == FLAIR_ACT_NONE && a.outScale == 1.f) go(std::integral_constant<int, 3>{});
        else go(std::integral_constant<int, 0>{});
    };

    DmaTile cur, nxt;
    int iCur = 0, iNxt = 0;
    if (!tile_at(0, cur)) return;
    nxt = cur;
    Walk wk;
    walk_first(nxt.t, wk);
    setup_tile(nxt);
    float4 biasReg = make_float4(0.f, 0.f, 0.f, 0.f);
    bool biasPending = false;
    auto bias_request = [&](const DmaTile& tl) {
        if (tid < 16) {
            const int bco = tl.co0 + 4 * tid;
            biasReg = (a.bias && bco < a.Cout) ? *reinterpret_cast<const float4*>(a.bias + bco) : make_float4(0.f, 0.f, 0.f, 0.f);
            if (a.fbias && bco < a.Cout) {
                const float* fb = a.fbias + (long)tl.t * a.fbiasLd + bco;
                biasReg.x += fb[0]; biasReg.y += fb[1]; biasReg.z += fb[2]; biasReg.w += fb[3];
            }
        }
        biasPending = true;
    };
    auto bias_commit = [&](int slot_) {
        if (tid < 16) *reinterpret_cast<float4*>(smem + BIAS_OFF + (slot_ & 1) * 256 + 16 * tid) = biasReg;
        biasPending = false;
    };
    bias_request(nxt);
    bias_commit(0);
    const bool res0any = a.res0 || a.res1;
    int remIssue = chunks_of(nxt.t);
    int remCompute = remIssue;
    bool more = true;
    int stage = 0;
    issue(nxt, wk, 0);
    walk_next(nxt.t, wk);
    --remIssue;
    asm volatile("s_waitcnt vmcnt(0)" ::: "memory");
    __syncthreads();
    zero_acc();
    while (true) {
        if (more && remIssue == 0) {
            ++iNxt;
            more = tile_at(iNxt, nxt);
            if (more) {
                walk_first(nxt.t, wk);
                setup_tile(nxt);
                remIssue = chunks_of(nxt.t);
                bias_request(nxt);
            }
        }
        if (more) {
            issue(nxt, wk, stage ^ 1);
            walk_next(nxt.t, wk);
            --remIssue;
        }
        compute(stage);
        if (biasPending) bias_commit(iNxt);
        bool storesInFlight = false;
        if (--remCompute == 0) {
            epilogue(cur, iCur);
            storesInFlight = RPW >= 2 ? !a.res1 : cur.co0 + 64 <= a.Cout && !res0any;
            ++iCur;
            if (!tile_at(iCur, cur)) break;
            remCompute = chunks_of(cur.t);
            zero_acc();
        }
        if (storesInFlight) {
            asm volatile("s_waitcnt vmcnt(%0)" ::"n"(4 * RPW) : "memory");
        } else {
            asm volatile("s_waitcnt vmcnt(0)" ::: "memory");
        }
        __syncthreads();
        stage ^= 1;
    }
}

template <int RPW>
__global__ __launch_bounds__(512, 2) void conv3x3_dma_kernel(ConvArgs a, int nTiles, int tilesPerXcd) {
    prefetch_kernargs<sizeof(ConvArgs) + 8>();
    conv3x3_dma_body<RPW>(a, nTiles, tilesPerXcd);
}

template <int RPW>
int launch_dma(const ConvArgs& a0, hipStream_t s) {
    constexpr int NW = 8, NSTAGE = 2, TH = NW * RPW;
    ConvArgs a = a0;
    a.nCoTiles = cdiv(a.Cout, 64);
    a.tFast = a.KT == 3 && a.T > 1;
    const int nTiles = a.T * (a.H / TH) * (a.W / 32) * a.nCoTiles;
    const int nCu = flair_cu_count();
    int grid = nTiles < nCu ? (nTiles + 7) / 8 * 8 : nCu / 8 * 8;
    if (grid < 8) grid = 8;
    const int tilesPerXcd = (nTiles + 7) / 8;
    constexpr int HALO_INSTR = ((TH + 2) * 34 + 15) / 16;
    const size_t lds = NSTAGE * (size_t)(HALO_INSTR + 36) * 1024 + NW * 1024 + 512;
    static LdsAttrOnce attr;
    {
        const hipError_t e = flair_max_lds_once(attr, reinterpret_cast<const void*>(&conv3x3_dma_kernel<RPW>));
        FLAIR_CHECK(e == hipSuccess, "flair_conv_nhwc: hipFuncSetAttribute: %s", hipGetErrorString(e));
    }
    hipLaunchKernelGGL(conv3x3_dma_kernel<RPW>, dim3(grid), dim3(64 * NW), lds, s, a, nTiles, tilesPerXcd);
    FLAIR_LAUNCH_CHECK();
    return FLAIR_OK;
}


__global__ __launch_bounds__(512, 2) void conv_frame_kernel(ConvArgs a) {
    prefetch_kernargs<sizeof(ConvArgs)>();
    using E = bf16_t;
    constexpr int NW = 8, HWP = 34;
    constexpr int HINSTR = 22, HIMG = HINSTR * 1024, WINSTR = 36, SLOT = WINSTR * 1024;
    constexpr int HR = 3, WR = 2;
    constexpr int RING = HR * HIMG, BIAS = RING + WR * SLOT;
    constexpr int NH = (HINSTR + NW - 1) / NW, NWS = (WINSTR + NW - 1) / NW;
    extern __shared__ __attribute__((aligned(16))) char smem[];
    const int tid = threadIdx.x, lane = tid & 63;
    const int wave = __builtin_amdgcn_readfirstlane(tid >> 6);
    const int lr = lane & 31, lh = lane >> 5;
    const int lrow = lane >> 2, lchunk = lane & 3;
    const int tilesW = a.W / 32, perFrame = tilesW * (a.H / 8);
    const int bid = xcd_remap(blockIdx.x, gridDim.x);
    const int t = bid / perFrame, tile = bid - t * perFrame;
    const int h0 = (tile / tilesW) * 8, w0 = (tile % tilesW) * 32;
    const int nS = a.CinTot / 32;

    const u32x4_t wdesc = make_desc(a.w, a.wBytes);
    const u32x4_t bdesc = make_desc(a.bias, a.bias ? (unsigned)a.Cout * 4u : 0u);
    dma16(bdesc, (unsigned)(lane * 16), (unsigned)BIAS);
    unsigned hpix[NH], hpiece[NH];
#pragma unroll
    for (int i = 0; i < NH; ++i) dma_halo_coords((wave * NH + i) % HINSTR, lrow, lchunk, 10, h0, w0, a.H, a.W, hpix[i], hpiece[i]);
    unsigned wlane[NWS];
#pragma unroll
    for (int i = 0; i < NWS; ++i) {
        const int id = (wave * NWS + i) % WINSTR;
        const int row = id * 16 + lrow, tap9 = row >> 6, co = row & 63;
        wlane[i] = co < a.Cout ? (unsigned)((co * 9 + tap9) * a.CinTot) * 2u + (unsigned)((lchunk ^ ((co >> 2) & 3)) << 4) : FLAIR_OOB;
    }
    int hseg = 0, hcb = 0;
    auto issue_halo = [&](int slot) {
        const unsigned ld = (unsigned)a.segLd[hseg] * 2u;
        const u32x4_t xdesc = make_desc(reinterpret_cast<const char*>(a.x[hseg]) + (size_t)t * a.H * a.W * ld, a.segBytes[hseg]);
        const unsigned cofs = (unsigned)(hcb * 64);
#pragma unroll
        for (int i = 0; i < NH; ++i) {
            const int k = (wave * NH + i) % HINSTR;
            dma16(xdesc, hpix[i] == 0xffffffffu ? FLAIR_OOB : hpix[i] * ld + cofs + hpiece[i], (unsigned)(slot * HIMG + k * 1024));
        }
        if (++hcb * 32 >= a.segC[hseg]) {
            hcb = 0;
            ++hseg;
        }
    };
    auto issue_w = [&](int s_) {
#pragma unroll
        for (int i = 0; i < NWS; ++i) {
            const int id = (wave * NWS + i) % WINSTR;
            dma16(wdesc, wlane[i] == FLAIR_OOB ? FLAIR_OOB : wlane[i] + (unsigned)(s_ * 64), (unsigned)(RING + (s_ % WR) * SLOT + id * 1024));
        }
    };
    issue_halo(0);
    issue_w(0);
    if (nS > 1) {
        issue_halo(1);
        issue_w(1);
    }
    if (nS > 2) issue_halo(2);

    unsigned aoff[2], boff[3][2];
    dma_frag_offsets(lr, lh, wave * HWP, aoff, boff);
    f32x16 acc[2];
    auto compute = [&](int wslot, int hslot) { dma_tap_loop(smem + RING + wslot * SLOT, smem + hslot * HIMG, aoff, boff, acc, dma_no_hook{}); };

    const long prow = ((long)t * a.H + h0 + wave) * a.W + w0;
    const unsigned yLdB = (unsigned)a.yLd * 2u, r0LdB = (unsigned)a.res0Ld * 2u, r1LdB = (unsigned)a.res1Ld * 2u;
    const __amdgpu_buffer_rsrc_t yd = make_rsrc(reinterpret_cast<char*>(a.y) + prow * a.yLd * 2, (unsigned)a.W * yLdB);
    const __amdgpu_buffer_rsrc_t r0d = make_rsrc(a.res0 ? reinterpret_cast<const char*>(a.res0) + prow * a.res0Ld * 2 : nullptr, a.res0 ? (unsigned)a.W * r0LdB : 0u);
    const __amdgpu_buffer_rsrc_t r1d = make_rsrc(a.res1 ? reinterpret_cast<const char*>(a.res1) + prow * a.res1Ld * 2 : nullptr, a.res1 ? (unsigned)a.W * r1LdB : 0u);
    uint4 r0v[4], r1v[4];
#pragma unroll
    for (int g = 0; g < 4; ++g) r0v[g] = r1v[g] = make_uint4(0u, 0u, 0u, 0u);

    for (int s_ = 0; s_ < nS; ++s_) {
        if (s_ + 1 >= nS) asm volatile("s_waitcnt vmcnt(0)" ::: "memory");
        else if (s_ == 0 && nS > 2) asm volatile("s_waitcnt vmcnt(%0)" ::"n"(2 * NH + NWS) : "memory");
        else if (s_ == 0) asm volatile("s_waitcnt vmcnt(%0)" ::"n"(NH + NWS) : "memory");
        else asm volatile("s_waitcnt vmcnt(%0)" ::"n"(NH) : "memory");
        __builtin_amdgcn_s_barrier();
        if (s_ == 0) {
            const float* sb = reinterpret_cast<const float*>(smem + BIAS);
#pragma unroll
            for (int cf = 0; cf < 2; ++cf)
#pragma unroll
                for (int g = 0; g < 4; ++g) {
                    const float4 bq = *reinterpret_cast<const float4*>(sb + cf * 32 + 8 * g + 4 * lh);
                    acc[cf][4 * g] = bq.x; acc[cf][4 * g + 1] = bq.y; acc[cf][4 * g + 2] = bq.z; acc[cf][4 * g + 3] = bq.w;
                }
        }
        if (s_ >= 1 && s_ + 1 < nS) issue_w(s_ + 1);
        if (s_ >= 1 && s_ + 2 < nS) issue_halo((s_ + 2) % 3);
        if (s_ + 1 == nS) {
            if (a.res0) {
#pragma unroll
                for (int g = 0; g < 4; ++g) r0v[g] = buf_load16(r0d, 16 * g + 8 * lh < a.Cout ? (unsigned)lr * r0LdB + (unsigned)(32 * g + 16 * lh) : FLAIR_OOB);
            }
            if (a.res1) {
#pragma unroll
                for (int g = 0; g < 4; ++g) r1v[g] = buf_load16(r1d, 16 * g + 8 * lh < a.Cout ? (unsigned)lr * r1LdB + (unsigned)(32 * g + 16 * lh) : FLAIR_OOB);
            }
        }
        compute(s_ % WR, s_ % HR);
    }

    const float slope = leaky_slope(a.act);
    const float scale = a.outScale;
#pragma unroll
    for (int cf = 0; cf < 2; ++cf)
#pragma unroll
        for (int jj = 0; jj < 2; ++jj) {
            const int g = 2 * cf + jj;
            float v[8];
            acc_octet(acc[cf], jj, v);
            leaky_act(v, slope);
            add_piece<E>(v, r0v[g]);
            add_piece<E>(v, r1v[g]);
#pragma unroll
            for (int e = 0; e < 8; ++e) v[e] *= scale;
            store_piece(yd, pack_piece<E>(v), 16 * g + 8 * lh < a.Cout ? (unsigned)lr * yLdB + (unsigned)(32 * g + 16 * lh) : FLAIR_OOB);
        }
}

static bool frame_kernel_ok(const ConvArgs& a) {
    if (a.esz != 2 || a.KT != 1 || a.KH != 3 || a.KW != 3 || a.stride != 1 || a.fbias || a.Cout > 64 || a.Cout % 8 || a.W % 32 || a.H % 8) return false;
    if (!(a.act == FLAIR_ACT_NONE || a.act == FLAIR_ACT_RELU || a.act == FLAIR_ACT_LRELU01 || a.act == FLAIR_ACT_LRELU02)) return false;
    if (a.tapShift || a.reflect || a.CinTot % 32 || a.CinTot < 32) return false;
    for (int i = 0; i < a.nseg; ++i)
        if (a.segC[i] % 32) return false;
    return true;
}

static int launch_frame(const ConvArgs& a, hipStream_t s) {
    constexpr size_t lds = (3 * 22 + 2 * 36) * 1024 + 1024;
    static LdsAttrOnce attr;
    const hipError_t e = flair_max_lds_once(attr, reinterpret_cast<const void*>(&conv_frame_kernel));
    FLAIR_CHECK(e == hipSuccess, "flair_conv_nhwc: hipFuncSetAttribute: %s", hipGetErrorString(e));
    hipLaunchKernelGGL(conv_frame_kernel, dim3(a.T * (a.H / 8) * (a.W / 32)), dim3(512), lds, s, a);
    FLAIR_LAUNCH_CHECK();
    return FLAIR_OK;
}

template <typename E, int TC, int TP, int WC, int WP, int PD, int KWID>
__global__ __launch_bounds__(256) void conv_igemm_kernel(ConvArgs a) {
    prefetch_kernargs<sizeof(ConvArgs)>();
    constexpr int BKE = Mma<E>::BKE * KWID;
    constexpr int ROWB = 64 * KWID;
    constexpr int CPR = 4 * KWID;
    constexpr int RPP = 256 / CPR;
    constexpr int VEC = ET<E>::VEC;
    constexpr int FC = TC / WC / 32;
    constexpr int FP = TP / WP / 32;
    constexpr int XR = TP / RPP;
    constexpr int WR = TC / RPP;
    static_assert(WC * WP == 4 && FC >= 1 && FP >= 1 && XR >= 1 && WR >= 1, "tile");

    extern __shared__ __attribute__((aligned(16))) char smem[];
    constexpr int BUF = (TC + TP) * ROWB;
    auto loff = [](int row, int chunk) { return KWID == 1 ? lds_off(row, chunk) : row * 128 + ((chunk ^ ((row >> 1) & 7)) << 4); };

    const int tid = threadIdx.x;
    const int lane = tid & 63, wave = __builtin_amdgcn_readfirstlane(tid >> 6);
    const int wc = wave / WP, wp = wave % WP;

    const int bid = xcd_remap(blockIdx.x, gridDim.x);
    const int coTile = bid % a.nCoTiles;
    const int pixTile = bid / a.nCoTiles;
    const long p0 = (long)pixTile * TP;
    const int co0 = coTile * TC;

    const int chunk = tid % CPR;
    const int srow = tid / CPR;
    int xt[XR], xh[XR], xw[XR];
    bool xvalid[XR];
#pragma unroll
    for (int i = 0; i < XR; ++i) {
        long p = p0 + srow + RPP * i;
        xvalid[i] = p < a.P;
        if (!xvalid[i]) p = 0;
        int w_ = (int)(p % a.W);
        long q = p / a.W;
        xw[i] = w_;
        xh[i] = (int)(q % a.H);
        xt[i] = (int)(q / a.H);
    }
    const int taps = a.KT * a.KH * a.KW;
    const int pt = a.KT / 2, ph = a.KH / 2, pw = a.KW / 2;
    const int tFirst = (int)(p0 / ((long)a.H * a.W));
    const int tileFrames = (int)((TP + (long)a.H * a.W - 1) / ((long)a.H * a.W)) + 1;

    uint4 xreg[PD][XR], wreg[PD][WR];

    const int nkAll = taps * (a.CinTot / BKE);
    const int ks0 = (int)((long)blockIdx.y * nkAll / a.splitK);
    const int ks1 = (int)((long)(blockIdx.y + 1) * nkAll / a.splitK);
    int tap = ks0 / (a.CinTot / BKE), seg = 0, cb = ks0 % (a.CinTot / BKE), segOff = 0;
    while (cb * BKE >= a.segC[seg]) {
        cb -= a.segC[seg] / BKE;
        segOff += a.segC[seg];
        ++seg;
    }
    int dw = tap % a.KW - pw, dh = (tap / a.KW) % a.KH - ph, dt = tap / (a.KW * a.KH) - pt;

// ... 114 lines not shown
                    for (int j = 0; j < FP; ++j) Mma<E>::run(af[i], bfr[j], acc[i][j]);
            }
            if (k + 1 < nk) write_lds(cur ^ 1, (u + 1) % PD);
            __syncthreads();
        }
    }

    if (a.splitK > 1) {
#pragma unroll
        for (int j = 0; j < FP; ++j) {
            const long p = p0 + wp * (TP / WP) + j * 32 + lr;
            if (p >= a.P) continue;
#pragma unroll
            for (int i = 0; i < FC; ++i)
#pragma unroll
                for (int g = 0; g < 4; ++g) {
                    const int co = co0 + wc * (TC / WC) + i * 32 + 8 * g + 4 * lh;
                    if (co < a.Cout)
                        *reinterpret_cast<float4*>(a.part + ((long)blockIdx.y * a.P + p) * a.Cout + co) =
                            make_float4(acc[i][j][4 * g], acc[i][j][4 * g + 1], acc[i][j][4 * g + 2],
                                        acc[i][j][4 * g + 3]);
                }
        }
        return;
    }
    if ((a.Cout & 7) == 0 && ((uintptr_t)a.y & 15) == 0 && (a.yLd * (int)sizeof(E)) % 16 == 0 &&
        (!a.res0 || (((uintptr_t)a.res0 & 15) == 0 && (a.res0Ld * (int)sizeof(E)) % 16 == 0)) &&
        (!a.res1 || (((uintptr_t)a.res1 & 15) == 0 && (a.res1Ld * (int)sizeof(E)) % 16 == 0))) {
        auto run = [&](auto actTag) {
            igemm_epilogue<E, decltype(actTag)::value, FC, FP>(a, acc, p0 + wp * (TP / WP), co0 + wc * (TC / WC), lr, lh);
        };
        if (a.act == FLAIR_ACT_DCN_OFFSETS) run(std::integral_constant<int, 1>{});
        else if (a.act == FLAIR_ACT_SILU) run(std::integral_constant<int, 2>{});
        else if (a.act == FLAIR_ACT_GELU) run(std::integral_constant<int, 3>{});
        else run(std::integral_constant<int, 0>{});
        return;
    }
#pragma unroll
    for (int j = 0; j < FP; ++j) {
        const long p = p0 + wp * (TP / WP) + j * 32 + lr;
        if (p >= a.P) continue;
#pragma unroll
        for (int i = 0; i < FC; ++i)
#pragma unroll
            for (int g = 0; g < 4; ++g)
                store_quad<E>(a, p, co0 + wc * (TC / WC) + i * 32 + 8 * g + 4 * lh, acc[i][j][4 * g],
                              acc[i][j][4 * g + 1], acc[i][j][4 * g + 2], acc[i][j][4 * g + 3]);
    }
}

template <typename E>
__global__ void conv_splitk_reduce_kernel(ConvArgs a) {
    const unsigned cq = (unsigned)(a.Cout / 4);
    const unsigned quads = (unsigned)a.P * cq;
    const size_t slice = (size_t)a.P * a.Cout;
    for (unsigned i = blockIdx.x * blockDim.x + threadIdx.x; i < quads; i += gridDim.x * blockDim.x) {
        const unsigned p = i / cq;
        const int co = (int)(i - p * cq) * 4;
        const float* src = a.part + (size_t)p * a.Cout + co;
        float4 s = make_float4(0.f, 0.f, 0.f, 0.f);
        int k = 0;
        for (; k + 4 <= a.splitK; k += 4) {
            float4 v[4];
#pragma unroll
            for (int u = 0; u < 4; ++u) v[u] = *reinterpret_cast<const float4*>(src + (size_t)(k + u) * slice);
#pragma unroll
            for (int u = 0; u < 4; ++u) {
                s.x += v[u].x; s.y += v[u].y; s.z += v[u].z; s.w += v[u].w;
            }
        }
        for (; k < a.splitK; ++k) {
            const float4 v = *reinterpret_cast<const float4*>(src + (size_t)k * slice);
            s.x += v.x; s.y += v.y; s.z += v.z; s.w += v.w;
        }
        store_quad<E>(a, p, co, s.x, s.y, s.z, s.w);
    }
}

template <typename E, int TC, int TP, int WC, int WP, int PD, int KWID>
int launch_pd(const ConvArgs& a0, hipStream_t s) {
    ConvArgs a = a0;
    a.nPixTiles = cdiv(a.P, TP);
    a.nCoTiles = cdiv(a.Cout, TC);
    const int grid = a.nPixTiles * a.nCoTiles;
    const size_t lds = 2 * (TC + TP) * 64 * KWID;
    hipLaunchKernelGGL((conv_igemm_kernel<E, TC, TP, WC, WP, PD, KWID>), dim3(grid, a.splitK), dim3(256), lds, s, a);
    FLAIR_LAUNCH_CHECK();
    if (a.splitK > 1) {
        hipLaunchKernelGGL(conv_splitk_reduce_kernel<E>, dim3(grid_for(a.P * (a.Cout / 4), 256, 2048)), dim3(256), 0, s, a);
        FLAIR_LAUNCH_CHECK();
    }
    return FLAIR_OK;
}

template <typename E, int TC, int TP, int WC, int WP>
int launch(const ConvArgs& a, hipStream_t s) {
    if constexpr (sizeof(E) == 2) {
        bool ok = true;
        for (int i = 0; i < a.nseg; ++i) ok = ok && a.segC[i] % 64 == 0;
        if (ok) return launch_pd<E, TC, TP, WC, WP, 2, 2>(a, s);
    }
    return launch_pd<E, TC, TP, WC, WP, 4, 1>(a, s);
}

enum ConvVariant {
    IGEMM_128x128 = 0,
    IGEMM_64x128 = 1,
    IGEMM_64x64 = 2,
    HALO_8 = 3,
    HALO_4 = 4,
    HALO_2 = 5,
    HALO_KS_8 = 6,
    HALO_KS_4 = 7,
    DMA_CLIP = 8,
    DMA_FRAME = 9,
};

int choose_split(const ConvArgs& a, ConvVariant variant) {
    if (variant > IGEMM_64x64) return 1;
    const int maxBlocks = variant == IGEMM_128x128 ? 512 : 1024, maxSplit = 16;
    const int tc = variant == IGEMM_128x128 ? 128 : 64, tp = variant == IGEMM_64x64 ? 64 : 128;
    const int bke = 64 / (a.wBytes && a.CinTot ? (int)(a.wBytes / ((unsigned long long)a.Cout * a.KT * a.KH * a.KW * a.CinTot)) : 2);
    const long nk = (long)a.KT * a.KH * a.KW * (a.CinTot / bke);
    const long tiles = (long)cdiv(a.P, tp) * cdiv(a.Cout, tc);
    if (tiles >= 384 || nk < 32) return 1;
    long s = maxBlocks / tiles;
    if (s > maxSplit) s = maxSplit;
    if (s > nk / 8) s = nk / 8;
    return s < 1 ? 1 : (int)s;
}

ConvVariant choose_variant(const ConvArgs& a) {
    if (!a.reflect && a.stride == 1 && a.KH == 3 && a.KW == 3 && a.W % 32 == 0 && a.H >= 2) {
        const long per = (long)a.T * (a.W / 32) * cdiv(a.Cout, 64);
        const bool ks = a.Cout % 8 == 0;
        if (a.esz == 2 && ks && a.act != FLAIR_ACT_GELU && a.H % 16 == 0 && per * cdiv(a.H, 8) > 256 && per * (a.H / 16) >= 192) return DMA_CLIP;
        const bool dmaOk = a.esz == 2 && ks && a.act != FLAIR_ACT_GELU;
        if (per * cdiv(a.H, 8) >= 256) return ks && per * cdiv(a.H, 8) <= 256 ? (dmaOk && a.H % 8 == 0 ? DMA_FRAME : HALO_KS_8) : HALO_8;
        if (per * cdiv(a.H, 4) >= 256) return ks && per * cdiv(a.H, 4) <= 256 ? HALO_KS_4 : HALO_4;
        return HALO_2;
    }
    const long tiles128 = (long)cdiv(a.P, 128) * cdiv(a.Cout, 128);
    if (a.Cout > 64 && tiles128 >= 512) return IGEMM_128x128;
    if (a.Cout >= 128 && a.P >= 1024 && tiles128 <= 64 && (long)a.KT * a.KH * a.KW * a.CinTot >= 2304) return IGEMM_128x128;
    const long tiles64x128 = (long)cdiv(a.P, 128) * cdiv(a.Cout, 64);
    if (tiles64x128 >= 512) return IGEMM_64x128;
    return IGEMM_64x64;
}

template <typename E>
int dispatch(const ConvArgs& a0, hipStream_t s) {
    ConvArgs a = a0;
    const ConvVariant variant = choose_variant(a);
    a.splitK = a.part ? choose_split(a, variant) : 1;
    switch (variant) {
        case IGEMM_128x128: return launch<E, 128, 128, 2, 2>(a, s);
        case IGEMM_64x128: return launch<E, 64, 128, 1, 4>(a, s);
        case IGEMM_64x64: return launch<E, 64, 64, 2, 2>(a, s);
        case HALO_8: return launch_halo<E, 8>(a, s);
        case HALO_4: return launch_halo<E, 4>(a, s);
        case HALO_KS_8: return launch_halo_ks<E, 8>(a, s);
        case HALO_KS_4: return launch_halo_ks<E, 4>(a, s);
        case DMA_CLIP: return launch_dma<2>(a, s);
        case DMA_FRAME:
            if (frame_kernel_ok(a)) return launch_frame(a, s);
            return launch_dma<1>(a, s);
        case HALO_2: break;
    }
    return launch_halo<E, 2>(a, s);
}

}

extern "C" int flair_conv_variant(const flair_conv_params* p);

static void fill_geometry(ConvArgs& a, const flair_conv_params* p) {
    a.stride = p->stride > 1 ? p->stride : 1;
    a.Hin = p->H; a.Win = p->W;
    a.T = p->T; a.KT = p->KT; a.KH = p->KH; a.KW = p->KW; a.Cout = p->Cout;
    a.reflect = p->reflect_pad ? 1 : 0;
    a.act = p->act;
    a.H = (p->H + a.stride - 1) / a.stride;
    a.W = (p->W + a.stride - 1) / a.stride;
    a.P = (long)p->T * a.H * a.W;
    a.CinTot = 0;
    for (int i = 0; i < p->nseg && i < 4; ++i) a.CinTot += p->seg_c[i];
    const int esz = p->dtype == FLAIR_BF16 ? 2 : 4;
    a.esz = esz;
    a.wBytes = (unsigned)((unsigned long long)p->Cout * p->KT * p->KH * p->KW * a.CinTot * esz);
}

extern "C" size_t flair_conv_workspace_bytes(const flair_conv_params* p) {
    if (!p) return 0;
    ConvArgs a{};
    fill_geometry(a, p);
    const int split = choose_split(a, choose_variant(a));
    return split > 1 ? (size_t)split * a.P * a.Cout * sizeof(float) : 0;
}

extern "C" int flair_conv_nhwc(const flair_conv_params* p, const void* const* x, const void* w,
                               const float* bias, const float* frame_bias, const void* res0, const void* res1,
                               void* y, void* workspace, size_t workspace_bytes, hipStream_t stream) {
    FLAIR_CHECK(p && x && w && y, "flair_conv_nhwc: null argument");
    FLAIR_CHECK_DTYPE("flair_conv_nhwc", p->dtype);
    FLAIR_CHECK(p->nseg >= 1 && p->nseg <= 4, "flair_conv_nhwc: nseg %d not in 1..4", p->nseg);
    FLAIR_CHECK(p->T > 0 && p->H > 0 && p->W > 0 && p->Cout > 0, "flair_conv_nhwc: empty shape");
    FLAIR_CHECK((p->KT & 1) && (p->KH & 1) && (p->KW & 1), "flair_conv_nhwc: kernel taps must be odd");
    FLAIR_CHECK(p->Cout % 4 == 0, "flair_conv_nhwc: Cout %d must be a multiple of 4", p->Cout);
    const int bke = p->dtype == FLAIR_BF16 ? 32 : 16;
    const int esz = p->dtype == FLAIR_BF16 ? 2 : 4;
    ConvArgs a{};
    fill_geometry(a, p);
    for (int i = 0; i < p->nseg; ++i) {
        FLAIR_CHECK(x[i], "flair_conv_nhwc: segment %d is null", i);
        FLAIR_CHECK(p->seg_c[i] > 0 && p->seg_c[i] % bke == 0,
                    "flair_conv_nhwc: segment %d has %d channels; must be a multiple of %d", i, p->seg_c[i], bke);
        FLAIR_CHECK(p->seg_ld[i] >= p->seg_c[i] && (p->seg_ld[i] * esz) % 16 == 0 &&
                        ((uintptr_t)x[i]) % 16 == 0,
                    "flair_conv_nhwc: segment %d stride/alignment", i);
        a.x[i] = x[i];
        a.segC[i] = p->seg_c[i];
        a.segLd[i] = p->seg_ld[i];
        const unsigned long long bytes = (unsigned long long)p->H * p->W * p->seg_ld[i] * esz;
        FLAIR_CHECK(bytes < 0x40000000ull, "flair_conv_nhwc: one frame of segment %d spans %llu bytes (limit 1 GiB)",
                    i, bytes);
        a.segBytes[i] = (unsigned)bytes;
    }
    {
        const unsigned long long wb = (unsigned long long)p->Cout * p->KT * p->KH * p->KW * a.CinTot * esz;
        FLAIR_CHECK(wb < 0x80000000ull, "flair_conv_nhwc: weights span %llu bytes (limit 2 GiB)", wb);
    }
    const int gran = (p->dtype == FLAIR_BF16 && p->Cout % 8 != 0) ? 8 : 16;
    FLAIR_CHECK(p->y_ld >= p->Cout && (p->y_ld * esz) % gran == 0 && ((uintptr_t)y) % 16 == 0,
                "flair_conv_nhwc: output stride/alignment (y_ld = %d: >= Cout = %d, a multiple of %d bytes; y 16-byte aligned)",
                p->y_ld, p->Cout, gran);
    FLAIR_CHECK(!res0 || (p->res_ld[0] >= p->Cout && (p->res_ld[0] * esz) % gran == 0 && ((uintptr_t)res0) % gran == 0),
                "flair_conv_nhwc: res0 stride/alignment (res_ld = %d: >= Cout = %d; stride and pointer multiples of %d bytes)",
                p->res_ld[0], p->Cout, gran);
    FLAIR_CHECK(!res1 || (p->res_ld[1] >= p->Cout && (p->res_ld[1] * esz) % gran == 0 && ((uintptr_t)res1) % gran == 0),
                "flair_conv_nhwc: res1 stride/alignment (res_ld = %d: >= Cout = %d; stride and pointer multiples of %d bytes)",
                p->res_ld[1], p->Cout, gran);
    FLAIR_CHECK(((uintptr_t)w) % 16 == 0, "flair_conv_nhwc: weight alignment");
    FLAIR_CHECK(!bias || ((uintptr_t)bias) % 16 == 0, "flair_conv_nhwc: bias alignment");
    a.nseg = p->nseg;
    a.w = w;
    a.bias = bias;
    a.fbias = frame_bias;
    a.fbiasLd = p->frame_bias_ld;
    FLAIR_CHECK(!frame_bias || p->frame_bias_ld >= p->Cout, "flair_conv_nhwc: frame_bias_ld");
    {
        const unsigned long long hw = (unsigned long long)p->H * p->W * esz;
        FLAIR_CHECK(hw * p->y_ld < 0x40000000ull && (!res0 || hw * p->res_ld[0] < 0x40000000ull) && (!res1 || hw * p->res_ld[1] < 0x40000000ull),
                    "flair_conv_nhwc: one frame of the output / a residual spans more than 1 GiB");
    }
    a.res0 = res0;
    a.res1 = res1;
    a.res0Ld = p->res_ld[0];
    a.res1Ld = p->res_ld[1];
    a.y = y;
    a.yLd = p->y_ld;
    a.actParam = p->act_param;
    a.actPeriod = p->act_period;
    FLAIR_CHECK(p->act != FLAIR_ACT_DCN_OFFSETS || (p->act_period > 0 && p->act_period % 24 == 0),
                "flair_conv_nhwc: FLAIR_ACT_DCN_OFFSETS needs act_period = 3 * deform_groups (multiple of 24), got %d",
                p->act_period);
    a.outScale = p->out_scale;
    FLAIR_CHECK(a.stride == 1 || a.stride == 2, "flair_conv_nhwc: stride %d unsupported", p->stride);
    FLAIR_CHECK(!p->asym_pad || (a.stride == 2 && a.KH == a.KW && a.KT == 1 && p->H % 2 == 0 && p->W % 2 == 0),
                "flair_conv_nhwc: asym_pad needs a square 2-D stride-2 kernel on even frames");
    a.tapShift = p->asym_pad ? a.KH / 2 : 0;
    FLAIR_CHECK(!p->reflect_pad || (!p->asym_pad && a.KT == 1 && p->H > a.KH / 2 && p->W > a.KW / 2),
                "flair_conv_nhwc: reflect_pad needs a 2-D kernel smaller than the frame");
    a.part = nullptr;
    a.splitK = 1;

    const size_t need = flair_conv_workspace_bytes(p);
    if (workspace && need > 0 && workspace_bytes >= need) {
        FLAIR_CHECK(((uintptr_t)workspace) % 16 == 0, "flair_conv_nhwc: workspace alignment");
        a.part = reinterpret_cast<float*>(workspace);
    }
    if (p->dtype == FLAIR_BF16) return dispatch<bf16_t>(a, stream);
    return dispatch<float>(a, stream);
}

extern "C" int flair_conv_variant(const flair_conv_params* p) {
    if (!p) return -1;
    ConvArgs a{};
    fill_geometry(a, p);
    return choose_variant(a);
}
```

flair_amd/csrc/dcn.hip:

```cpp


#include "common.h"
#include "mfma_tile.h"

namespace {

struct DcnArgs {
    const void* x[2];
    int xLd[2];
    int Cin;
    const void* raw; int rawLd;
    const float* flow1;
    const float* flow2;
    const void* w;
    const float* bias;
    void* y; int yLd;
    int F, H, W, Cout, G;
    float maxMag;
    int activated;
    long P;
    unsigned xBytes[2], rawBytes, wBytes;
};

template <int CPR>
__device__ __forceinline__ int tile_off(int row, int chunk) {
    const int s = CPR == 4 ? (row >> 2) & 3 : CPR == 8 ? (row >> 1) & 7 : row & 15;
    return row * (CPR * 16) + ((chunk ^ s) << 4);
}

__device__ __forceinline__ int mul_i24(int a, int b) {
    int r;
    asm("v_mul_i32_i24 %0, %1, %2" : "=v"(r) : "v"(a), "v"(b));
    return r;
}

__device__ __forceinline__ unsigned cvt_pk_bf16(float lo, float hi) {
    unsigned r;
    asm("v_cvt_pk_bf16_f32 %0, %1, %2" : "=v"(r) : "v"(lo), "v"(hi));
    return r;
}

__device__ __forceinline__ float fast_tanh(float x) {
    const float e = __expf(2.f * x);
    return 1.f - 2.f * __builtin_amdgcn_rcpf(e + 1.f);
}

constexpr bool dcn_dot2(int esz, int offs, bool oneframe) { return esz == 2 && offs == 1 && oneframe; }
constexpr int dcn_pfd(int esz, int ncf, int npf, int tpp, int offs, bool oneframe) {
    return dcn_dot2(esz, offs, oneframe) && ncf == 2 && npf == 4 ? 1 : ncf >= 4 && tpp <= 8 ? 3 : 2;
}

template <typename E, int NCF, int NPF, int TPP, int OFFS, bool ONEFRAME>
__global__ __launch_bounds__(32 * NPF * TPP, (dcn_pfd(sizeof(E), NCF, NPF, TPP, OFFS, ONEFRAME) == 1 ? 8 : NCF >= 4 ? 32 * NPF * TPP / 256 : 4))
void dcn_kernel(DcnArgs a) {
    constexpr int PFD = dcn_pfd(sizeof(E), NCF, NPF, TPP, OFFS, ONEFRAME);
    constexpr bool DOT2 = dcn_dot2(sizeof(E), OFFS, ONEFRAME);
    static_assert(OFFS != 2 || !ONEFRAME, "raw offsets: the general (batched) form only");
    prefetch_kernargs<sizeof(DcnArgs)>();
    constexpr int NT = 32 * NPF * TPP, NW = NT / 64;

    constexpr int TP = 32 * NPF, TC = 32 * NCF, CPR = TPP;
    constexpr int VEC = ET<E>::VEC;
    constexpr unsigned ESZ = sizeof(E);
    constexpr int BKE = CPR * VEC;
    constexpr int NPAIR = NCF * NPF;
    constexpr int KSPLIT = NW > NPAIR ? NW / NPAIR : 1;
    constexpr int PAIRS = NW > NPAIR ? 1 : NPAIR / NW;
    constexpr int KSUB = CPR / 4 / KSPLIT;
    static_assert((NW > NPAIR ? NPAIR * KSPLIT == NW : PAIRS * NW == NPAIR) && KSUB >= 1 && KSUB * KSPLIT * 4 == CPR,
                  "tile shape");
    constexpr int WR = (TC * CPR + NT - 1) / NT;
    constexpr int RAWR = (TP * 3 * (int)ESZ + NT - 1) / NT;
    constexpr int BUF = (TC + TP) * CPR * 16;
    extern __shared__ __attribute__((aligned(16))) char smem[];
    const int G = a.G;
    const int slabBytes = OFFS == 2 ? (3 * G * (int)ESZ + 15) & ~15 : 3 * G * (int)ESZ;
    const int slabPieces = slabBytes / 16;
    const int rawPitch = slabBytes + 16;
    char* sraw = smem;
    char* stile = smem + 2 * TP * rawPitch;

    const int tid = threadIdx.x, lane = tid & 63, wave = tid >> 6;
    const int lr = lane & 31, lh = lane >> 5;
    const long p0 = (long)xcd_remap(blockIdx.x, gridDim.x) * TP;
    const int q = tid % TPP, srow = tid / TPP;
    long p = p0 + srow;
    const bool pvalid = p < a.P;
    if (!pvalid) p = a.P - 1;
    const int pw = (int)(p % a.W);
    const int ph = (int)((p / a.W) % a.H);
    const int pf = (int)((ONEFRAME ? p0 : p) / ((long)a.W * a.H));
    float2 fl1 = make_float2(0.f, 0.f), fl2 = make_float2(0.f, 0.f);
    if (a.flow1) fl1 = *reinterpret_cast<const float2*>(a.flow1 + p * 2);
    if (a.flow2) fl2 = *reinterpret_cast<const float2*>(a.flow2 + p * 2);

    const __amdgpu_buffer_rsrc_t rr = make_rsrc(a.raw, a.rawBytes);
    auto raw_issue = [&](int tap, uint4 (&reg)[RAWR]) {
#pragma unroll
        for (int j = 0; j < RAWR; ++j) {
            const int id = tid + j * NT;
            const int px = id / slabPieces, pc = id - px * slabPieces;
            const long pp = p0 + px;
            const unsigned within = (unsigned)(3 * tap * G) * ESZ + pc * 16;
            reg[j] = buf_load16(rr, px < TP && pp < a.P ? (unsigned)(pp * a.rawLd * ESZ) + within : FLAIR_OOB);
        }
    };
    auto raw_write = [&](int tap, const uint4 (&reg)[RAWR]) {
#pragma unroll
        for (int j = 0; j < RAWR; ++j) {
            const int id = tid + j * NT;
            const int px = id / slabPieces, pc = id - px * slabPieces;
            if (px < TP) *reinterpret_cast<uint4*>(sraw + ((tap & 1) * TP + px) * rawPitch + pc * 16) = reg[j];
        }
    };
    auto stage_raw = [&](int tap) {
        uint4 reg[RAWR];
        raw_issue(tap, reg);
        raw_write(tap, reg);
    };

    const int cpg = a.Cin / G;
    int cpgShift = 0;
    while ((1 << cpgShift) < cpg) ++cpgShift;
    const int halfC = a.Cin / 2;
    const int cbPerTap = a.Cin / BKE;
    const int nk = 9 * cbPerTap;
    const size_t fo0 = ONEFRAME ? (size_t)pf * a.H * a.W * a.xLd[0] * ESZ : 0, fo1 = ONEFRAME ? (size_t)pf * a.H * a.W * a.xLd[1] * ESZ : 0;
    const __amdgpu_buffer_rsrc_t xr0 = make_rsrc(reinterpret_cast<const char*>(a.x[0]) + fo0, a.xBytes[0]);
    const __amdgpu_buffer_rsrc_t xr1 = make_rsrc(reinterpret_cast<const char*>(a.x[1]) + fo1, a.xBytes[1]);
    const __amdgpu_buffer_rsrc_t wrs = make_rsrc(a.w, a.wBytes);
    const unsigned frameBase = (unsigned)pf * a.H * a.W;

    struct Regs {
        uint4 c[4];
        uint4 w[WR];
        float wt[4];
    } rs[PFD];

    unsigned wrow[WR];
#pragma unroll
    for (int j = 0; j < WR; ++j) {
        const int id = tid + j * NT;
        const int n = id / CPR, ch = id % CPR;
        wrow[j] = n < a.Cout && n < TC ? (unsigned)(n * 9 * a.Cin + ch * VEC) * ESZ : FLAIR_OOB;
    }
    int itap = 0, icb = 0, ikh = 0, ikw = 0;
    const int rawRow = srow * rawPitch;
    const float fH = (float)a.H, fW = (float)a.W;
    const float phm1 = (float)(ph - 1), pwm1 = (float)(pw - 1);
    auto issue = [&](Regs& r) {
        const int tap = itap, cb = icb;
        const int c = cb * BKE + q * VEC;
        const int g = c >> cpgShift;
        const E* myraw = reinterpret_cast<const E*>(sraw + (tap & 1) * TP * rawPitch + rawRow);
        const float ry = ET<E>::ld(myraw + 2 * g), rx = ET<E>::ld(myraw + 2 * g + 1);
        const float rm = ET<E>::ld(myraw + 2 * G + g);
        const bool second = cb * BKE >= halfC;
        const float2 fl = second ? fl2 : fl1;
        float sy = phm1 + (float)ikh + fl.y, sx = pwm1 + (float)ikw + fl.x, mk;
        if constexpr (OFFS == 1) {
            sy += ry;
            sx += rx;
            mk = rm;
        } else if constexpr (OFFS == 2) {
            sy += ry;
            sx += rx;
            mk = __builtin_amdgcn_rcpf(1.f + __expf(-rm));
        } else {
            sy += a.maxMag * fast_tanh(ry);
            sx += a.maxMag * fast_tanh(rx);
            mk = __builtin_amdgcn_rcpf(1.f + __expf(-rm));
        }
        const float fy = floorf(sy), fx = floorf(sx);
        const float ay = sy - fy, ax = sx - fx;
        const int y0 = (int)__builtin_amdgcn_fmed3f(fy, -2.f, fH), x0 = (int)__builtin_amdgcn_fmed3f(fx, -2.f, fW);
        const unsigned ld = (unsigned)(second ? a.xLd[1] : a.xLd[0]) * ESZ;
        const unsigned coff = (unsigned)(c - (second ? halfC : 0)) * ESZ;
        const __amdgpu_buffer_rsrc_t xr = second ? xr1 : xr0;
        const unsigned rowStep = (unsigned)a.W * ld;
        if constexpr (ONEFRAME) {
            const float wx0 = (unsigned)x0 < (unsigned)a.W ? (1.f - ax) * mk : 0.f;
            const float wx1 = (unsigned)(x0 + 1) < (unsigned)a.W ? ax * mk : 0.f;
            r.wt[0] = (1.f - ay) * wx0;
            r.wt[1] = (1.f - ay) * wx1;
            r.wt[2] = ay * wx0;
            r.wt[3] = ay * wx1;
            const unsigned o00 =
                (unsigned)mul_i24(mul_i24(y0, a.W) + x0, (int)ld) + coff;
            r.c[0] = buf_load16(xr, o00);
            r.c[1] = buf_load16(xr, o00 + ld);
            r.c[2] = buf_load16(xr, o00 + rowStep);
            r.c[3] = buf_load16(xr, o00 + rowStep + ld);
        } else {
            r.wt[0] = (1.f - ay) * (1.f - ax) * mk;
            r.wt[1] = (1.f - ay) * ax * mk;
            r.wt[2] = ay * (1.f - ax) * mk;
            r.wt[3] = ay * ax * mk;
            const unsigned o00 = (unsigned)mul_i24(
                                     (int)frameBase + mul_i24(y0, a.W) + x0, (int)ld) + coff;
            const bool yok0 = pvalid && (unsigned)y0 < (unsigned)a.H, yok1 = pvalid && (unsigned)(y0 + 1) < (unsigned)a.H;
            const bool xok0 = (unsigned)x0 < (unsigned)a.W, xok1 = (unsigned)(x0 + 1) < (unsigned)a.W;
            r.c[0] = buf_load16(xr, yok0 && xok0 ? o00 : FLAIR_OOB);
            r.c[1] = buf_load16(xr, yok0 && xok1 ? o00 + ld : FLAIR_OOB);
            r.c[2] = buf_load16(xr, yok1 && xok0 ? o00 + rowStep : FLAIR_OOB);
            r.c[3] = buf_load16(xr, yok1 && xok1 ? o00 + rowStep + ld : FLAIR_OOB);
        }
        const unsigned wk = (unsigned)(tap * a.Cin + cb * BKE) * ESZ;
#pragma unroll
        for (int j = 0; j < WR; ++j) r.w[j] = buf_load16(wrs, wrow[j] == FLAIR_OOB ? FLAIR_OOB : wrow[j] + wk);
        if (++icb == cbPerTap) {
            icb = 0;
            ++itap;
            if (++ikw == 3) {
                ikw = 0;
                ++ikh;
            }
        }
    };
    auto blend_and_stage = [&](const Regs& r, int buf) {
        char* base = stile + buf * BUF;
        uint4 outv;
        if constexpr (sizeof(E) == 2 && DOT2) {
            typedef __attribute__((ext_vector_type(2))) __bf16 bf16x2_t;
            const bf16x2_t w01 = __builtin_bit_cast(bf16x2_t, cvt_pk_bf16(r.wt[0], r.wt[1]));
            const bf16x2_t w23 = __builtin_bit_cast(bf16x2_t, cvt_pk_bf16(r.wt[2], r.wt[3]));
            unsigned o[4];
            const unsigned c0[4] = {r.c[0].x, r.c[0].y, r.c[0].z, r.c[0].w}, c1[4] = {r.c[1].x, r.c[1].y, r.c[1].z, r.c[1].w};
            const unsigned c2[4] = {r.c[2].x, r.c[2].y, r.c[2].z, r.c[2].w}, c3[4] = {r.c[3].x, r.c[3].y, r.c[3].z, r.c[3].w};
            float lo[4], hi[4];
#pragma unroll
            for (int d = 0; d < 4; ++d) {
                const bf16x2_t tlo = __builtin_bit_cast(bf16x2_t, __builtin_amdgcn_perm(c1[d], c0[d], 0x05040100u));
                const bf16x2_t thi = __builtin_bit_cast(bf16x2_t, __builtin_amdgcn_perm(c1[d], c0[d], 0x07060302u));
                const bf16x2_t blo = __builtin_bit_cast(bf16x2_t, __builtin_amdgcn_perm(c3[d], c2[d], 0x05040100u));
                const bf16x2_t bhi = __builtin_bit_cast(bf16x2_t, __builtin_amdgcn_perm(c3[d], c2[d], 0x07060302u));
                lo[d] = __builtin_amdgcn_fdot2_f32_bf16(tlo, w01, 0.f, false);
                hi[d] = __builtin_amdgcn_fdot2_f32_bf16(thi, w01, 0.f, false);
                lo[d] = __builtin_amdgcn_fdot2_f32_bf16(blo, w23, lo[d], false);
                hi[d] = __builtin_amdgcn_fdot2_f32_bf16(bhi, w23, hi[d], false);
            }
            asm volatile("s_nop 2" : "+v"(lo[0]), "+v"(lo[1]), "+v"(lo[2]), "+v"(lo[3]), "+v"(hi[0]), "+v"(hi[1]), "+v"(hi[2]), "+v"(hi[3]));
#pragma unroll
            for (int d = 0; d < 4; ++d) o[d] = cvt_pk_bf16(lo[d], hi[d]);
            outv = make_uint4(o[0], o[1], o[2], o[3]);
        } else if constexpr (sizeof(E) == 2) {
            typedef float f32x2 __attribute__((ext_vector_type(2)));
            f32x2 lo[2] = {{0.f, 0.f}, {0.f, 0.f}}, hi[2] = {{0.f, 0.f}, {0.f, 0.f}};
#pragma unroll
            for (int i = 0; i < 4; ++i) {
                const unsigned d[4] = {r.c[i].x, r.c[i].y, r.c[i].z, r.c[i].w};
                const f32x2 w = {r.wt[i], r.wt[i]};
#pragma unroll
                for (int j = 0; j < 2; ++j) {
                    const f32x2 vl = {__uint_as_float(d[2 * j] << 16), __uint_as_float(d[2 * j + 1] << 16)};
                    const f32x2 vh = {__uint_as_float(d[2 * j] & 0xffff0000u), __uint_as_float(d[2 * j + 1] & 0xffff0000u)};
                    lo[j] = __builtin_elementwise_fma(w, vl, lo[j]);
                    hi[j] = __builtin_elementwise_fma(w, vh, hi[j]);
                }
            }
            outv = make_uint4(cvt_pk_bf16(lo[0].x, hi[0].x), cvt_pk_bf16(lo[0].y, hi[0].y), cvt_pk_bf16(lo[1].x, hi[1].x),
                              cvt_pk_bf16(lo[1].y, hi[1].y));
        } else {
            float acc[VEC];
#pragma unroll
            for (int e = 0; e < VEC; ++e) acc[e] = 0.f;
#pragma unroll
            for (int i = 0; i < 4; ++i) {
                float v[VEC];
                Vec16<E>::load(reinterpret_cast<const E*>(&r.c[i]), v);
#pragma unroll
                for (int e = 0; e < VEC; ++e) acc[e] = fmaf(r.wt[i], v[e], acc[e]);
            }
            alignas(16) E out[VEC];
            Vec16<E>::store(out, acc);
            outv = *reinterpret_cast<const uint4*>(out);
        }
        *reinterpret_cast<uint4*>(base + TC * CPR * 16 + tile_off<CPR>(srow, q)) = outv;
#pragma unroll
        for (int j = 0; j < WR; ++j) {
            const int id = tid + j * NT;
            if (id < TC * CPR) *reinterpret_cast<uint4*>(base + tile_off<CPR>(id / CPR, id % CPR)) = r.w[j];
        }
    };

    f32x16 acc[PAIRS];
#pragma unroll
    for (int i = 0; i < PAIRS; ++i)
#pragma unroll
        for (int r = 0; r < 16; ++r) acc[i][r] = 0.f;

    constexpr int LEAD = PFD + 1;
    int stageTap = 0;
    {
        uint4 r0[RAWR], r1[RAWR];
        const bool two = cbPerTap - LEAD < 0;
        raw_issue(0, r0);
        if (two) raw_issue(1, r1);
        raw_write(0, r0);
        if (two) raw_write(1, r1);
        stageTap = two ? 2 : 1;
    }
    int stageAt = stageTap * cbPerTap - LEAD;
    __syncthreads();
    auto mfma_step = [&](int buf) {
        const char* wb = stile + buf * BUF;
        const char* xb = wb + TC * CPR * 16;
#pragma unroll
        for (int i = 0; i < PAIRS; ++i) {
            const int pair = KSPLIT > 1 ? wave % NPAIR : wave * PAIRS + i;
            const int kpart = KSPLIT > 1 ? wave / NPAIR : 0;
            const int pfrag = pair % NPF, cf = pair / NPF;
#pragma unroll
            for (int kk = 0; kk < KSUB; ++kk) {
                const int ks = kpart * KSUB + kk;
                uint4 af[2], bf[2];
#pragma unroll
                for (int h = 0; h < 2; ++h) {
                    const int ch = ks * 4 + Mma<E>::chunk(h, lh);
                    bf[h] = *reinterpret_cast<const uint4*>(xb + tile_off<CPR>(pfrag * 32 + lr, ch));
                    af[h] = *reinterpret_cast<const uint4*>(wb + tile_off<CPR>(cf * 32 + lr, ch));
                }
                Mma<E>::run(af, bf, acc[i]);
            }
        }
    };
#pragma unroll
    for (int u = 0; u < PFD - 1; ++u)
        if (u < nk) issue(rs[u]);
    constexpr int UNR = 2 * PFD;
    for (int k = 0; k < nk; k += UNR) {
#pragma unroll
        for (int u = 0; u < UNR; ++u) {
            if (k + u < nk) {
                if (k + u + PFD - 1 < nk) issue(rs[(u + PFD - 1) % PFD]);
                blend_and_stage(rs[u % PFD], u & 1);
                __syncthreads();
                mfma_step(u & 1);
                if (k + u == stageAt && stageTap < 9) {
                    stage_raw(stageTap);
                    ++stageTap;
                    stageAt += cbPerTap;
                }
            }
        }
    }
    if constexpr (KSPLIT > 1) {
        __syncthreads();
        float* red = reinterpret_cast<float*>(stile);
        const int pair0 = wave % NPAIR, kpart0 = wave / NPAIR;
        if (kpart0 > 0) {
            float* dst = red + ((kpart0 - 1) * NPAIR + pair0) * 64 * 16 + lane * 16;
#pragma unroll
            for (int r = 0; r < 16; r += 4)
                *reinterpret_cast<float4*>(dst + r) = make_float4(acc[0][r], acc[0][r + 1], acc[0][r + 2], acc[0][r + 3]);
        }
        __syncthreads();
        if (kpart0 > 0) return;
#pragma unroll
        for (int kp = 1; kp < KSPLIT; ++kp) {
            const float* src = red + ((kp - 1) * NPAIR + pair0) * 64 * 16 + lane * 16;
#pragma unroll
            for (int r = 0; r < 16; r += 4) {
                const float4 v = *reinterpret_cast<const float4*>(src + r);
                acc[0][r] += v.x; acc[0][r + 1] += v.y; acc[0][r + 2] += v.z; acc[0][r + 3] += v.w;
            }
        }
    }
    E* y = reinterpret_cast<E*>(a.y);
    if constexpr (sizeof(E) == 2) {
        if ((a.Cout & 7) == 0 && (a.yLd & 7) == 0 && (reinterpret_cast<uintptr_t>(a.y) & 15) == 0) {
            const __amdgpu_buffer_rsrc_t bd = make_rsrc(a.bias, a.bias ? (unsigned)a.Cout * 4u : 0u);
            const __amdgpu_buffer_rsrc_t yd = make_rsrc(a.y, (unsigned)a.P * a.yLd * 2u);
#pragma unroll
            for (int i = 0; i < PAIRS; ++i) {
                const int pair = KSPLIT > 1 ? wave % NPAIR : wave * PAIRS + i;
                const int pfrag = pair % NPF, cf = pair / NPF;
                const long po = p0 + pfrag * 32 + lr;
                uint4 bq[2][2];
#pragma unroll
                for (int j = 0; j < 2; ++j) {
                    const int co = cf * 32 + 16 * j + 8 * lh;
                    bq[j][0] = buf_load16(bd, co < a.Cout ? 4u * co : FLAIR_OOB);
                    bq[j][1] = buf_load16(bd, co < a.Cout ? 4u * co + 16u : FLAIR_OOB);
                }
#pragma unroll
                for (int j = 0; j < 2; ++j) {
                    const int co = cf * 32 + 16 * j + 8 * lh;
                    float v[8];
                    acc_octet(acc[i], j, v);
                    v[0] += __uint_as_float(bq[j][0].x); v[1] += __uint_as_float(bq[j][0].y);
                    v[2] += __uint_as_float(bq[j][0].z); v[3] += __uint_as_float(bq[j][0].w);
                    v[4] += __uint_as_float(bq[j][1].x); v[5] += __uint_as_float(bq[j][1].y);
                    v[6] += __uint_as_float(bq[j][1].z); v[7] += __uint_as_float(bq[j][1].w);
                    store_piece(yd, pack_piece<E>(v), po < a.P && co < a.Cout ? ((unsigned)po * a.yLd + co) * 2u : FLAIR_OOB);
                }
            }
            return;
        }
    }
#pragma unroll
    for (int i = 0; i < PAIRS; ++i) {
        const int pair = KSPLIT > 1 ? wave % NPAIR : wave * PAIRS + i;
        const int pfrag = pair % NPF, cf = pair / NPF;
        const long po = p0 + pfrag * 32 + lr;
        if (po >= a.P) continue;
#pragma unroll
        for (int g = 0; g < 4; ++g) {
            const int co = cf * 32 + 8 * g + 4 * lh;
            if (co >= a.Cout) continue;
            float v[4];
#pragma unroll
            for (int e = 0; e < 4; ++e) v[e] = acc[i][4 * g + e] + (a.bias ? a.bias[co + e] : 0.f);
            E* dst = y + po * a.yLd + co;
            if constexpr (sizeof(E) == 4) {
                *reinterpret_cast<float4*>(dst) = make_float4(v[0], v[1], v[2], v[3]);
            } else {
                uint2 pk;
                pk.x = pack2bf(v[0], v[1]);
                pk.y = pack2bf(v[2], v[3]);
                *reinterpret_cast<uint2*>(dst) = pk;
            }
        }
    }
}

}

template <typename E, int NCF, int NPF, int TPP, int OFFS, bool ONEFRAME>
static int launch_dcn_v(const DcnArgs& a0, hipStream_t stream) {
    DcnArgs a = a0;
    if (ONEFRAME) {
        const unsigned long long half = a.Cin / 2, hw = (unsigned long long)a.H * a.W;
        a.xBytes[0] = (unsigned)(((hw - 1) * a.xLd[0] + half) * sizeof(E));
        a.xBytes[1] = (unsigned)(((hw - 1) * a.xLd[1] + half) * sizeof(E));
    }
    constexpr int NT = 32 * NPF * TPP, TP = 32 * NPF, TC = 32 * NCF;
    const int rawPitch = (OFFS == 2 ? (3 * a.G * (int)sizeof(E) + 15) & ~15 : 3 * a.G * (int)sizeof(E)) + 16;
    const size_t lds = (size_t)2 * TP * rawPitch + 2 * (TC + TP) * TPP * 16;
    static LdsAttrOnce attr;
    {
        const hipError_t e = flair_max_lds_once(attr, reinterpret_cast<const void*>(&dcn_kernel<E, NCF, NPF, TPP, OFFS, ONEFRAME>));
        FLAIR_CHECK(e == hipSuccess, "flair_dcn_align: hipFuncSetAttribute: %s", hipGetErrorString(e));
    }
    hipLaunchKernelGGL((dcn_kernel<E, NCF, NPF, TPP, OFFS, ONEFRAME>), dim3(cdiv(a.P, TP)), dim3(NT), lds, stream, a);
    FLAIR_LAUNCH_CHECK();
    return FLAIR_OK;
}

template <typename E, int NCF, int NPF, int TPP>
static int launch_dcn(const DcnArgs& a, hipStream_t stream) {
    const bool oneframe = ((long)a.H * a.W) % (32 * NPF) == 0;
    if (a.activated && oneframe) return launch_dcn_v<E, NCF, NPF, TPP, 1, true>(a, stream);
    if (a.activated) return launch_dcn_v<E, NCF, NPF, TPP, 1, false>(a, stream);
    return launch_dcn_v<E, NCF, NPF, TPP, 0, false>(a, stream);
}

struct VqfrTile {
    int bke, tc;
};

static VqfrTile vqfr_tile(const flair_dcn_params* p) {
    if (p->dtype == FLAIR_BF16) {
        if ((p->Cin / 2) % 64 != 0) return {32, 64};
        if (p->Cout <= 64) return {64, 64};
        const long P = (long)p->F * p->H * p->W;
        return {P >= 64 * 256 && (p->Cin / 2) % 128 == 0 ? 128 : 64, 128};
    }
    return p->Cout <= 64 ? VqfrTile{16, 64} : VqfrTile{32, 128};
}

template <typename E>
static int launch_dcn_vqfr(const flair_dcn_params* p, const DcnArgs& a, hipStream_t stream) {
    if constexpr (sizeof(E) == 2) {
        if ((a.Cin / 2) % 64 != 0) return launch_dcn_v<E, 2, 4, 4, 2, false>(a, stream);
        if (a.Cout <= 64) return a.P >= 128 * 512 ? launch_dcn_v<E, 2, 4, 8, 2, false>(a, stream) : launch_dcn_v<E, 2, 2, 8, 2, false>(a, stream);
        if (a.P >= 64 * 256 && (a.Cin / 2) % 128 == 0) return launch_dcn_v<E, 4, 2, 16, 2, false>(a, stream);
        if (a.P >= 64 * 256) return launch_dcn_v<E, 4, 2, 8, 2, false>(a, stream);
        return launch_dcn_v<E, 4, 1, 8, 2, false>(a, stream);
    } else {
        (void)p;
        return a.Cout <= 64 ? launch_dcn_v<E, 2, 2, 4, 2, false>(a, stream) : launch_dcn_v<E, 4, 1, 8, 2, false>(a, stream);
    }
}

static int dcn_vqfr(const flair_dcn_params* p, const DcnArgs& a0, hipStream_t stream) {
    const VqfrTile t = vqfr_tile(p);
    const int esz = p->dtype == FLAIR_BF16 ? 2 : 4;
    for (int co0 = 0; co0 < p->Cout; co0 += t.tc) {
        DcnArgs a = a0;
        a.Cout = p->Cout - co0 < t.tc ? p->Cout - co0 : t.tc;
        a.w = static_cast<const char*>(a0.w) + (size_t)co0 * 9 * p->Cin * esz;
        a.bias = a0.bias ? a0.bias + co0 : nullptr;
        a.y = static_cast<char*>(a0.y) + (size_t)co0 * esz;
        a.wBytes = (unsigned)((unsigned long long)a.Cout * 9 * p->Cin * esz);
        const int rc = p->dtype == FLAIR_BF16 ? launch_dcn_vqfr<bf16_t>(p, a, stream) : launch_dcn_vqfr<float>(p, a, stream);
        if (rc != FLAIR_OK) return rc;
    }
    return FLAIR_OK;
}

extern "C" int flair_dcn_align(const flair_dcn_params* p, const void* x0, const void* x1, const void* raw,
                               const float* flow1, const float* flow2, const void* w, const float* bias, void* y,
                               hipStream_t stream) {
    FLAIR_CHECK(p && x0 && x1 && raw && w && y, "flair_dcn_align: null argument");
    FLAIR_CHECK_DTYPE("flair_dcn_align", p->dtype);
    FLAIR_CHECK(p->raw_activated >= 0 && p->raw_activated <= 2, "flair_dcn_align: raw_activated = %d (0, 1 or 2)", p->raw_activated);
    const bool vqfr = p->raw_activated == 2;
    FLAIR_CHECK(!vqfr || (!flow1 && !flow2), "flair_dcn_align: raw_activated = 2 takes no flows");
    const int vec = p->dtype == FLAIR_BF16 ? 8 : 4;
    const int bke = vqfr ? vqfr_tile(p).bke : vec * (p->Cout <= 64 && p->dtype != FLAIR_BF16 ? 4 : 8);
    const int esz = p->dtype == FLAIR_BF16 ? 2 : 4;
    const int cpg = p->G > 0 ? p->Cin / p->G : 0;
    FLAIR_CHECK(p->G > 0 && (p->G % 8 == 0 || (vqfr && p->G == 4)) && p->G <= 16 && p->Cin % p->G == 0 && cpg % vec == 0 &&
                    (cpg & (cpg - 1)) == 0 && (p->Cin / 2) % bke == 0 && (!vqfr || p->Cin <= 1024),
                "flair_dcn_align: Cin=%d G=%d not supported", p->Cin, p->G);
    FLAIR_CHECK(p->Cout > 0 && p->Cout % 4 == 0 && (vqfr ? p->Cout <= 1024 : p->Cout <= 128) && p->raw_ld >= 27 * p->G &&
                    (p->raw_ld * esz) % 16 == 0,
                "flair_dcn_align: Cout = %d (a multiple of 4, <= 128; <= 1024 with raw_activated = 2) / raw_ld = %d (>= 27 G, "
                "16-byte granular)", p->Cout, p->raw_ld);
    FLAIR_CHECK(p->x_ld[0] >= p->Cin / 2 && p->x_ld[1] >= p->Cin / 2 && (p->x_ld[0] * esz) % 16 == 0 &&
                    (p->x_ld[1] * esz) % 16 == 0 && ((uintptr_t)x0) % 16 == 0 && ((uintptr_t)x1) % 16 == 0 &&
                    ((uintptr_t)raw) % 16 == 0 && p->y_ld >= p->Cout,
                "flair_dcn_align: strides/alignment (x_ld = %d, %d: >= Cin / 2 = %d, 16-byte granular; x0, x1, raw 16-byte "
                "aligned; y_ld = %d >= Cout = %d)", p->x_ld[0], p->x_ld[1], p->Cin / 2, p->y_ld, p->Cout);
    DcnArgs a;
    a.x[0] = x0; a.x[1] = x1; a.xLd[0] = p->x_ld[0]; a.xLd[1] = p->x_ld[1];
    a.Cin = p->Cin; a.raw = raw; a.rawLd = p->raw_ld; a.flow1 = flow1; a.flow2 = flow2;
    a.w = w; a.bias = bias; a.y = y; a.yLd = p->y_ld;
    a.F = p->F; a.H = p->H; a.W = p->W; a.Cout = p->Cout; a.G = p->G; a.maxMag = p->max_residue_magnitude;
    a.activated = p->raw_activated;
    a.P = (long)p->F * p->H * p->W;
    const unsigned long long half = p->Cin / 2;
    const unsigned long long b0 = ((unsigned long long)(a.P - 1) * p->x_ld[0] + half) * esz;
    const unsigned long long b1 = ((unsigned long long)(a.P - 1) * p->x_ld[1] + half) * esz;
    const unsigned long long br = ((unsigned long long)(a.P - 1) * p->raw_ld + 27 * p->G) * esz;
    const unsigned long long by = (unsigned long long)a.P * p->y_ld * esz;
    FLAIR_CHECK(b0 < 0x80000000ull && b1 < 0x80000000ull && br < 0x80000000ull && by < 0x80000000ull, "flair_dcn_align: tensor spans >= 2 GiB");
    FLAIR_CHECK(a.P + 2l * p->W + 2 < (1l << 23) && (long)p->x_ld[0] * esz < (1l << 23) && (long)p->x_ld[1] * esz < (1l << 23),
                "flair_dcn_align: F*H*W = %ld pixels (limit 2^23 per call: call per frame)", a.P);
    a.xBytes[0] = (unsigned)b0; a.xBytes[1] = (unsigned)b1; a.rawBytes = (unsigned)((br + 15) / 16 * 16);
    a.wBytes = (unsigned)((unsigned long long)p->Cout * 9 * p->Cin * esz);
    if (vqfr) return dcn_vqfr(p, a, stream);
    if (p->dtype == FLAIR_BF16) {
        if (p->Cout > 64) {
            if (a.P >= 64 * 256 && (p->Cin / 2) % 128 == 0) return launch_dcn<bf16_t, 4, 2, 16>(a, stream);
            if (a.P >= 64 * 256) return launch_dcn<bf16_t, 4, 2, 8>(a, stream);
            return launch_dcn<bf16_t, 4, 1, 8>(a, stream);
        }
        return a.P >= 128 * 512 ? launch_dcn<bf16_t, 2, 4, 8>(a, stream) : launch_dcn<bf16_t, 2, 2, 8>(a, stream);
    }
    return p->Cout <= 64 ? launch_dcn<float, 2, 2, 4>(a, stream) : launch_dcn<float, 4, 1, 8>(a, stream);
}
```

flair_amd/guided_diffusion/unet_new.py:

```python
import math

import torch
import torch.nn as nn

from .. import ops
from .clip_model import ClipModel
from .nn_new import conv_nd, linear, normalization, zero_module
from .packing import LinearStack, dev_f32, pack_w, packed_conv, pk_int, run_conv

A = ops


class PlaceHolder(nn.Module):

    def __init__(self, module):
        super().__init__()
        self.wrapped_module = module


LazyReshaper2D = LazyReshaper3D = PlaceHolder


class TemporalWrapper(PlaceHolder):
    """unet_new.py:50-59 (skipped when ``enable_cross_frames`` is False)."""
# ... 135 lines not shown
        self._pk = dict(
            film_off=film_off,
            g=dev_f32(self.norm.wrapped_module.weight, device), be=dev_f32(self.norm.wrapped_module.bias, device),
            wqkv=pack_w(self.qkv.weight.unsqueeze(-1), dtype, device, [(c, c)]), bqkv=dev_f32(self.qkv.bias, device),
            wp=pack_w(self.proj_out.weight.unsqueeze(-1), dtype, device, [(c, c)]),
            bp=dev_f32(self.proj_out.bias, device))

    def run(self, ctx, x):
        pk, c = self._pk, self.channels
        n = ops.group_norm(x, pk["g"], pk["be"], eps=self.norm.wrapped_module.eps)
        qkv = ops.conv(n, pk["wqkv"], pk["bqkv"], 3 * c, (1, 1, 1))
        a = ops.qkv_attention(qkv, self.num_heads, new_order=self.new_order)
        if self.bottleneck:
            ops.add_frame_bias(a, ctx.film_all[:, pk["film_off"]:pk["film_off"] + c])
        return ops.conv(a, pk["wp"], pk["bp"], c, (1, 1, 1), res0=x)


class AttentionbottleBlock(AttentionBlock):

    bottleneck = True


class FalshAttn(nn.Module):
    """nn.py:389-394 -- marker only (the window attention kernel replaces flash-attn)."""


class TemporalAttention(nn.Module):

    def __init__(self, channels, num_frames, num_heads=1, num_head_channels=-1, use_checkpoint=False):
        super().__init__()
        self.channels = channels
        if num_head_channels == -1:
            self.num_heads = num_heads
        else:
            assert channels % num_head_channels == 0
            self.num_heads = channels // num_head_channels
        assert num_frames % 2 == 1, "num_frames must be odd"
        self.head_dim = temporal_head_width(channels, self.num_heads)
        self.num_frames = num_frames
        self.q_linear = linear(channels, channels)
        self.k_linear = linear(channels, channels)
        self.v_linear = linear(channels, channels)
        self.attn = FalshAttn()
        self.proj = zero_module(PlaceHolder(conv_nd(2, channels, channels, 1)))
        self.norm = PlaceHolder(normalization(channels))

    def pack(self, dtype, device):
        c, f = self.channels, self.num_frames
        offs = torch.arange(f, dtype=torch.float32, device=device) - f // 2
        mid = f // 2
        wq, wk, wv = (dev_f32(m.weight, device) for m in (self.q_linear, self.k_linear, self.v_linear))
        if torch.device(device).type == "cuda":
            pe = ops.timestep_embedding(offs, c)
            bq = ops.linear(pe[mid:mid + 1].contiguous(), wq, dev_f32(self.q_linear.bias, device))
            kpos = ops.linear(torch.cat([pe[:mid], pe[mid + 1:]]).contiguous(), wk, None)
        else:
            freqs = torch.exp(-math.log(10000.0) * torch.arange(c // 2, dtype=torch.float32) / (c // 2))
            ang = offs[:, None] * freqs[None]
            pe = torch.cat([torch.cos(ang), torch.sin(ang)], dim=-1)
            bq = pe[mid:mid + 1] @ wq.t() + dev_f32(self.q_linear.bias, device)
            kpos = torch.cat([pe[:mid], pe[mid + 1:]]) @ wk.t()
        wqkv = torch.cat([wq, wk, wv]).reshape(3 * c, c, 1, 1)
        bqkv = torch.cat([bq.reshape(-1), dev_f32(self.k_linear.bias, device), dev_f32(self.v_linear.bias, device)])
        self._pk = dict(
            g=dev_f32(self.norm.wrapped_module.weight, device), be=dev_f32(self.norm.wrapped_module.bias, device),
            wqkv=pack_w(wqkv, dtype, device, [(c, c)]), bqkv=bqkv.contiguous(), kpos=kpos,
            wp=pack_w(self.proj.wrapped_module.weight, dtype, device, [(c, c)]),
            bp=dev_f32(self.proj.wrapped_module.bias, device))

    def run(self, ctx, h):
        pk, c = self._pk, self.channels
        n = ops.group_norm(h, pk["g"], pk["be"], eps=self.norm.wrapped_module.eps)
        qkv = ops.conv(n, pk["wqkv"], pk["bqkv"], 3 * c, (1, 1, 1))
        a = ops.temporal_attention(qkv, pk["kpos"], self.num_frames,
                                   round_fp16=(ctx.dtype == torch.float32), head_dim=self.head_dim)
        return ops.conv(a, pk["wp"], pk["bp"], c, (1, 1, 1), res0=h)


class ResidualBlockNoBN(nn.Module):
    def __init__(self, mid_channels):
        super().__init__()
        self.conv1 = nn.Conv2d(mid_channels, mid_channels, 3, 1, 1, bias=True)
        self.conv2 = nn.Conv2d(mid_channels, mid_channels, 3, 1, 1, bias=True)


class ResidualBlocksWithInputConv(nn.Module):

    def __init__(self, in_channels, out_channels=64, num_blocks=1):
        super().__init__()
        if num_blocks != 1:
            raise NotImplementedError("flair_amd: FLAIR uses one residual block per trunk")
        self.main = nn.Sequential(nn.Conv2d(in_channels, out_channels, 3, 1, 1, bias=True),
                                  nn.LeakyReLU(negative_slope=0.1),
                                  nn.Sequential(ResidualBlockNoBN(out_channels)))

    def pack(self, dtype, device, split):
        c = self.main[0].out_channels
        rb = self.main[2][0]
        return dict(w0=pack_w(self.main[0].weight, dtype, device, [(s, s) for s in split]),
                    b0=dev_f32(self.main[0].bias, device),
                    w1=pack_w(rb.conv1.weight, dtype, device, [(c, c)]), b1=dev_f32(rb.conv1.bias, device),
                    w2=pack_w(rb.conv2.weight, dtype, device, [(c, c)]), b2=dev_f32(rb.conv2.bias, device))




def run_trunk(pk, segs, c, *, extra_res=None, out=None, out_scale=1.0):
    k = (1, 3, 3)
    t1 = ops.conv(segs, pk["w0"], pk["b0"], c, k, act=A.ACT_LRELU01)
    if c == 64 and ops.chain_supported(t1, c):
        return ops.conv_chain(t1, pk["w1"], pk["b1"], A.ACT_RELU, pk["w2"], pk["b2"], A.ACT_NONE, c, c,
                              res0=t1, res1=extra_res, out=out, out_scale=out_scale)
    t2 = ops.conv(t1, pk["w1"], pk["b1"], c, k, act=A.ACT_RELU)
    return ops.conv(t2, pk["w2"], pk["b2"], c, k, res0=t1, res1=extra_res, out=out, out_scale=out_scale)


class SecondOrderDeformableAlignment(nn.Module):

    def __init__(self, in_channels, out_channels, kernel_size=3, padding=1, deform_groups=16,
                 max_residue_magnitude=10):
        super().__init__()
        assert kernel_size == 3 and padding == 1
        self.in_channels, self.out_channels = in_channels, out_channels
        self.deform_groups, self.max_residue_magnitude = deform_groups, max_residue_magnitude
        self.weight = nn.Parameter(torch.empty(out_channels, in_channels, 3, 3))
        self.bias = nn.Parameter(torch.zeros(out_channels))
        stdv = 1.0 / math.sqrt(in_channels * 9)
        with torch.no_grad():
            self.weight.uniform_(-stdv, stdv)
        c = out_channels
        self.conv_offset = nn.Sequential(
            nn.Conv2d(3 * c + 4, c, 3, 1, 1), nn.LeakyReLU(negative_slope=0.1),
            nn.Conv2d(c, c, 3, 1, 1), nn.LeakyReLU(negative_slope=0.1),
            nn.Conv2d(c, c, 3, 1, 1), nn.LeakyReLU(negative_slope=0.1),
            nn.Conv2d(c, 27 * deform_groups, 3, 1, 1))
        zero_module(self.conv_offset[-1])

    def pack(self, dtype, device):
        c = self.out_channels
        ka = ops.k_align(dtype)
        co = self.conv_offset
        perm = ops.dcn_raw_permutation(self.deform_groups)
        w6, b6 = co[6].weight.detach()[perm], co[6].bias.detach()[perm]
        return dict(
            w0=pack_w(co[0].weight, dtype, device, [(c, c), (c, c), (c, c), (4, ka)]), b0=dev_f32(co[0].bias, device),
            w2=pack_w(co[2].weight, dtype, device, [(c, c)]), b2=dev_f32(co[2].bias, device),
            w4=pack_w(co[4].weight, dtype, device, [(c, c)]), b4=dev_f32(co[4].bias, device),
            w6=pack_w(w6, dtype, device, [(c, c)]), b6=dev_f32(b6, device),
            wd=pack_w(self.weight, dtype, device, [(2 * c, 2 * c)]), bd=dev_f32(self.bias, device))


class BasicVSRPP(nn.Module):

    def __init__(self, mid_channels=64, max_residue_magnitude=10, use_checkpoint=False):
        super().__init__()
        self.mid_channels = mid_channels
        self.deform_align = nn.ModuleDict()
        self.backbone = nn.ModuleDict()
        for i, name in enumerate(["backward_1", "forward_1"]):
            self.deform_align[name] = SecondOrderDeformableAlignment(
                2 * mid_channels, mid_channels, 3, padding=1, deform_groups=16,
                max_residue_magnitude=max_residue_magnitude)
            self.backbone[name] = ResidualBlocksWithInputConv((2 + i) * mid_channels, mid_channels, 1)
        self.reconstruction = ResidualBlocksWithInputConv(3 * mid_channels, mid_channels, 1)
        self.conv_last = zero_module(nn.Conv2d(mid_channels, mid_channels, 1, 1))

    def pack(self, dtype, device):
        c = self.mid_channels
        self._pk = dict(
            align={n: m.pack(dtype, device) for n, m in self.deform_align.items()},
            trunk={"backward_1": self.backbone["backward_1"].pack(dtype, device, [c, c]),
                   "forward_1": self.backbone["forward_1"].pack(dtype, device, [c, c, c])},
            recon=self.reconstruction.pack(dtype, device, [c, c, c]),
            wl=pack_w(self.conv_last.weight, dtype, device, [(c, c)]), bl=dev_f32(self.conv_last.bias, device))

    def _propagate(self, ctx, hidden, flows, name, others, weight, wmaps, dest):
        pk_a, pk_t = self._pk["align"][name], self._pk["trunk"][name]
        T, H, W, c = hidden.shape
        order = list(range(T))
        flow_idx = list(range(-1, T - 1))
        if "backward" in name:
            order = order[::-1]
            flow_idx = order
        zero_c = torch.zeros((1, H, W, c), dtype=ctx.dtype, device=ctx.device)
        ka = ops.k_align(ctx.dtype)
        k3 = (1, 3, 3)
        G = self.deform_align[name].deform_groups
        mag = float(self.deform_align[name].max_residue_magnitude)
        store = ctx.flows.get("_prop") if isinstance(ctx.flows, dict) else None
        key = (name, H, W, ctx.dtype, ka)
        cached = store.get(key) if store is not None else None
        fill = [] if (cached is None and store is not None) else None
        prop, prev2 = zero_c, None
        for i, idx in enumerate(order):
            cur = hidden[idx:idx + 1]
            if i > 0:
                flow_n1 = flows[flow_idx[i]:flow_idx[i] + 1]
                cond_n1 = torch.empty_like(zero_c)
                second = i > 1
                feat_n2 = prev2 if second else zero_c
                cond_n2 = torch.empty_like(zero_c) if second else zero_c
                if cached is not None:
                    flow_n2, flowpad = cached[i - 1]
                    ops.vsrpp_warp2(prop, feat_n2 if second else None, flow_n1, flow_n2, cond_n1, cond_n2 if second else None)
                else:
                    flowpad = torch.zeros((1, H, W, ka), dtype=ctx.dtype, device=ctx.device)
                    flow_n2 = torch.empty_like(flow_n1) if second else None
                    ops.vsrpp_prep(prop, feat_n2 if second else None, flow_n1,
                                   flows[flow_idx[i - 1]:flow_idx[i - 1] + 1] if second else None,
                                   cond_n1, cond_n2 if second else None, flow_n2, flowpad)
                    if fill is not None:
                        fill.append((flow_n2, flowpad))
                o = ops.conv([cond_n1, cur, cond_n2, flowpad], pk_a["w0"], pk_a["b0"], c, k3, act=A.ACT_LRELU01)
                if c == 64 and ops.chain_supported(o, c):
                    o = ops.conv_chain(o, pk_a["w2"], pk_a["b2"], A.ACT_LRELU01, pk_a["w4"], pk_a["b4"],
                                       A.ACT_LRELU01, c, c)
                else:
                    o = ops.conv(o, pk_a["w2"], pk_a["b2"], c, k3, act=A.ACT_LRELU01)
                    o = ops.conv(o, pk_a["w4"], pk_a["b4"], c, k3, act=A.ACT_LRELU01)
                if c == 64 and ops.chain_supported(o, c) and W % 32 == 0:
                    raw = ops.conv_chain(o, None, None, A.ACT_NONE, pk_a["w6"], pk_a["b6"], A.ACT_DCN_OFFSETS, c, 27 * G,
                                         act_param=mag, act_period=3 * G)
                else:
                    raw = ops.conv(o, pk_a["w6"], pk_a["b6"], 27 * G, k3, act=A.ACT_DCN_OFFSETS, act_param=mag,
                                   act_period=3 * G)
                aligned = ops.dcn_align(prop, feat_n2, raw, flow_n1, flow_n2, pk_a["wd"], pk_a["bd"], c,
                                        groups=G, max_mag=mag, raw_activated=True)

            else:
                aligned = zero_c
            segs = [cur] + [o_[idx:idx + 1] for o_ in others] + [aligned]
            new = run_trunk(pk_t, segs, c, extra_res=aligned, out=dest[idx:idx + 1], out_scale=weight)
            if wmaps is not None:
                ops.scale_pixels(new, wmaps[idx])
            prev2, prop = (prop if i > 0 else None), new
        if fill is not None:
            store[key] = fill
        return dest

    def run(self, ctx, hidden):
        T, H, W, c = hidden.shape
        flows_forward, flows_backward = ctx.flows[W]
        weight, wmaps = 1.0, None
        vw = ctx.vsrpp_weights
        if isinstance(vw, (float, int)):
            weight = float(vw)
        elif vw is not None:
            wm = vw.reshape(T, vw.shape[-2], vw.shape[-1], 1).float().contiguous()
            if wm.shape[1] != H or wm.shape[2] != W:
                wm = ops.resize(wm, (H, W), ops.RESIZE_NEAREST)
            wmaps = [wm[i] for i in range(T)]
        bwd = torch.empty_like(hidden)
        fwd = torch.empty_like(hidden)
        self._propagate(ctx, hidden, flows_backward, "backward_1", [], weight, wmaps, bwd)
        ff = flows_forward if flows_forward is not None else flows_backward.flip(0)
        self._propagate(ctx, hidden, ff, "forward_1", [bwd], weight, wmaps, fwd)
        rec = run_trunk(self._pk["recon"], [hidden, bwd, fwd], c)
        return ops.conv(rec, self._pk["wl"], self._pk["bl"], c, (1, 1, 1), res0=hidden)


class _ConvModule(nn.Module):
    def __init__(self, cin, cout):
        super().__init__()
        self.conv = nn.Conv2d(cin, cout, kernel_size=7, stride=1, padding=3)


class SPyNetBasicModule(nn.Module):
    def __init__(self):
        super().__init__()
        ch = [8, 32, 64, 32, 16, 2]
        self.basic_module = nn.Sequential(*[_ConvModule(ch[i], ch[i + 1]) for i in range(5)])


class SPyNet(nn.Module):

    def __init__(self, pretrained=None):
        super().__init__()
        self.basic_module = nn.ModuleList([SPyNetBasicModule() for _ in range(6)])
        self.register_buffer("mean", torch.tensor([0.485, 0.456, 0.406]).view(1, 3, 1, 1))
        self.register_buffer("std", torch.tensor([0.229, 0.224, 0.225]).view(1, 3, 1, 1))

    def pack(self, dtype, device):
        f32 = torch.float32
        levels = []
        for bm in self.basic_module:
            convs = [m.conv for m in bm.basic_module]
            ws = [pack_w(convs[0].weight, f32, device, [(3, 4), (3, 4), (2, 8)])]
            ws += [pack_w(convs[j].weight, f32, device, [(convs[j].in_channels,) * 2]) for j in (1, 2, 3)]
            ws.append(pack_w(convs[4].weight, f32, device, [(16, 16)], cout_pad=4))
            bs = [dev_f32(convs[j].bias, device) for j in range(4)]
            bs.append(torch.cat([dev_f32(convs[4].bias, device), torch.zeros(2, device=device)]).contiguous())
            levels.append((ws, bs))
        mean = dev_f32(self.mean.reshape(-1), device)
        istd = (1.0 / dev_f32(self.std.reshape(-1), device)).contiguous()
        self._pk = dict(levels=levels, mean=mean, istd=istd)

    def pair_flows(self, raw):
        if raw.shape[0] < 2:
            empty = torch.zeros((0, raw.shape[1], raw.shape[2], 2), dtype=torch.float32, device=raw.device)
            return empty, empty
        norm = torch.zeros_like(raw)
        ops.affine_channels(raw, 3, 0.5, 0.5, 0.0, 1.0, self._pk["mean"], self._pk["istd"], norm)
        a, b = norm[:-1], norm[1:]
        flows_backward = self.run(a, b)
        return self.run(b, a), flows_backward

    def run(self, ref, supp):
        F_, h0, w0, _ = ref.shape
        dev = ref.device
        if F_ == 0:
            return torch.zeros((0, h0, w0, 2), dtype=torch.float32, device=dev)
        h = h0 if h0 % 32 == 0 else 32 * (h0 // 32 + 1)
        w = w0 if w0 % 32 == 0 else 32 * (w0 // 32 + 1)
        if (h, w) != (h0, w0):
            ref = ops.resize(ref, (h, w), ops.RESIZE_BILINEAR, channels=3)
            supp = ops.resize(supp, (h, w), ops.RESIZE_BILINEAR, channels=3)
        sizes = [(h >> (5 - l), w >> (5 - l)) for l in range(6)]
        bufs = [torch.zeros((F_, *sizes[l], 16), dtype=torch.float32, device=dev) for l in range(6)]
        sp = [None] * 6
        ops.cast_channels(ref[..., :3], bufs[5], 0)
        sp[5] = supp
        for l in range(4, -1, -1):
            ops.resize(bufs[l + 1][..., 0:4], sizes[l], ops.RESIZE_AVGPOOL2, channels=3, out=bufs[l][..., 0:4])
            sp[l] = ops.resize(sp[l + 1], sizes[l], ops.RESIZE_AVGPOOL2, channels=3)
        flow = None
        k7 = (1, 7, 7)
        for l in range(6):
            b = bufs[l]
            if l > 0:
                ops.resize(flow, sizes[l], ops.RESIZE_BILINEAR_AC, channels=2, out=b[..., 8:12],
                           scale_c0=2.0, scale_c1=2.0)
            ops.flow_warp(sp[l], b[..., 8:10], border=True, out=b[..., 4:8])
            ws, bs = self._pk["levels"][l]
            y = ops.conv(b, ws[0], bs[0], 32, k7, act=A.ACT_RELU)
            y = ops.conv(y, ws[1], bs[1], 64, k7, act=A.ACT_RELU)
            y = ops.conv(y, ws[2], bs[2], 32, k7, act=A.ACT_RELU)
            y = ops.conv(y, ws[3], bs[3], 16, k7, act=A.ACT_RELU)
            flow = ops.conv(y, ws[4], bs[4], 4, k7, res0=b[..., 8:12])
        out = torch.empty((F_, h0, w0, 2), dtype=torch.float32, device=dev)
        ops.resize(flow, (h0, w0), ops.RESIZE_BILINEAR, channels=2, out=out,
                   scale_c0=float(w0) / float(w), scale_c1=float(h0) / float(h))
        return out


class TimestepEmbedSequential(nn.Sequential):

    def run(self, ctx, h, skip=None):
        for i, layer in enumerate(self):
            inner = layer.wrapped_module if isinstance(layer, PlaceHolder) else layer
            if isinstance(layer, TemporalWrapper) and not ctx.enable_cross_frames:
                continue
            if isinstance(inner, ResBlock):
                h = inner.run(ctx, h, skip if i == 0 else None)
            elif isinstance(inner, (AttentionBlock, TemporalAttention, BasicVSRPP)):
                h = inner.run(ctx, h)
            elif isinstance(inner, nn.Conv2d):
                h = run_conv(h, inner._pk, inner)
            elif isinstance(inner, nn.Identity):
                pass
            else:
                raise TypeError(f"flair_amd: no executor for {type(inner).__name__}")
        return h


class UNetModel(ClipModel, nn.Module):

    _name = "flair_amd.UNetModel"

    def __init__(self, image_size, in_channels, model_channels, out_channels, num_res_blocks,
                 attention_resolutions, rnn_resolutions, dropout=0, channel_mult=(1, 2, 4, 8),
                 conv_resample=True, dims=2, num_classes=None, use_checkpoint=False, use_fp16=False,
                 num_heads=1, num_head_channels=-1, num_heads_upsample=-1, use_scale_shift_norm=False,
                 resblock_updown=False, use_new_attention_order=False, temporal_block=False):
        super().__init__()
        if dims != 2 or num_classes is not None or not resblock_updown:
            raise NotImplementedError("flair_amd: UNetModel covers the FLAIR video configuration "
                                      "(dims=2, resblock_updown=True, no class conditioning)")
        if num_heads_upsample == -1:
            num_heads_upsample = num_heads
        self.image_size, self.in_channels, self.model_channels = image_size, in_channels, model_channels
        self.out_channels, self.num_res_blocks = out_channels, num_res_blocks
        self.attention_resolutions, self.rnn_resolutions = attention_resolutions, rnn_resolutions
        self.channel_mult = channel_mult
# ... 151 lines not shown
```

flair_amd/ops.py:

```python
import ctypes

import torch

from ._header import STRUCTS
from ._lib import ACT_DCN_OFFSETS, ACT_GELU, ACT_LRELU01, ACT_LRELU02, ACT_NONE, ACT_RELU, ACT_SILU, ConvParams, call, dtype_code, lib
from ._lib import check, ptr, stream

__all__ = ["conv", "conv_chain", "group_norm", "nchw_to_clip", "clip_to_nchw", "timestep_embedding", "linear",
           "qkv_attention", "temporal_attention", "flow_warp", "flow_compose", "resize",
           "dcn_align", "dcn_raw_permutation", "scale_pixels", "predict_xstart", "sampler_update",
           "ACT_NONE", "ACT_RELU", "ACT_LRELU01", "ACT_SILU", "ACT_DCN_OFFSETS", "ACT_LRELU02", "ACT_GELU"]


GnParams, SamplerCoefs, AttnParams = STRUCTS["flair_gn_params"], STRUCTS["flair_sampler_coefs"], STRUCTS["flair_attn_params"]
TAttnParams, DcnParams, ChainParams = STRUCTS["flair_tattn_params"], STRUCTS["flair_dcn_params"], STRUCTS["flair_chain_params"]


def _ld(t):
    assert t.dim() == 4 and t.stride(3) == 1, "clip tensors are (T,H,W,C) with C innermost"
    ld = t.stride(2)
    assert t.stride(1) == ld * t.shape[2] and (t.shape[0] == 1 or t.stride(0) == ld * t.shape[1] * t.shape[2]), \
        "clip tensor must be dense over (T,H,W)"
    return ld


def _dense(t):
    assert t is None or t.is_contiguous()
    return t


def k_align(dtype):
    return 32 if dtype == torch.bfloat16 else 16


def pad_channels(c, dtype):
    g = k_align(dtype)
    return (c + g - 1) // g * g


def conv(xs, weight, bias, cout, kernel, *, out=None, act=ACT_NONE, res0=None, res1=None,
         out_scale=1.0, stride=1, frame_bias=None, act_param=0.0, act_period=0, asym_pad=False, reflect_pad=False):
    if isinstance(xs, torch.Tensor):
        xs = [xs]
    x0 = xs[0]
    T, H, W, _ = x0.shape
    p = ConvParams()
    p.dtype = dtype_code(x0)
    p.T, p.H, p.W = T, H, W
    p.KT, p.KH, p.KW = kernel
    p.Cout = cout
    p.nseg = len(xs)
    arr = (ctypes.c_void_p * 4)()
    for i, x in enumerate(xs):
        assert x.dtype == x0.dtype and x.shape[:3] == x0.shape[:3]
        p.seg_c[i] = x.shape[3]
        p.seg_ld[i] = _ld(x)
        arr[i] = x.data_ptr()
    p.stride = stride
    p.asym_pad = asym_pad
    p.reflect_pad = reflect_pad
    p.frame_bias_ld = frame_bias.stride(0) if frame_bias is not None else 0
    if frame_bias is not None:
        assert frame_bias.dtype == torch.float32 and frame_bias.stride(1) == 1 and frame_bias.shape[0] == T
    Ho, Wo = (H + stride - 1) // stride, (W + stride - 1) // stride
    if out is None:
        out = torch.empty((T, Ho, Wo, cout), dtype=x0.dtype, device=x0.device)
    assert tuple(out.shape[:3]) == (T, Ho, Wo) and out.shape[3] >= cout and out.dtype == x0.dtype
    p.y_ld = _ld(out)
    p.res_ld[0] = _ld(res0) if res0 is not None else 0
    p.res_ld[1] = _ld(res1) if res1 is not None else 0
    p.act = act
    p.act_param, p.act_period = act_param, act_period
    p.out_scale = out_scale
    assert weight.dtype == x0.dtype and weight.is_contiguous()
    e0 = _prof_begin()
    wsb = _conv_ws_bytes(p)
    ws = _workspace(wsb, x0.device, "conv") if wsb else None

    def launch(_keep=xs):
        call.flair_conv_nhwc(ctypes.byref(p), arr, weight, _dense(bias), frame_bias, res0, res1, out, ws, wsb)
    launch()
    if e0 is not None:
        cin = sum(x.shape[3] for x in xs)
        taps = kernel[0] * kernel[1] * kernel[2]
        esz = x0.element_size()
        flops = 2.0 * T * Ho * Wo * cout * cin * taps
        nbytes = esz * (cin * T * H * W + cout * T * Ho * Wo * (1 + (res0 is not None) + (res1 is not None))
                        + cout * taps * cin)
        _prof_end(e0, ("conv", lib().flair_conv_variant(ctypes.byref(p))), x0.dtype, flops, nbytes, launch,
                  ("conv", T, H, W, tuple(x.shape[3] for x in xs), cout, tuple(kernel), stride, act,
                   res0 is not None, res1 is not None, frame_bias is not None))
    return out


PROFILE = None


def _prof_begin():
    if PROFILE is None:
        return None
    e0 = torch.cuda.Event(enable_timing=True)
    e0.record()
    return e0


def _prof_end(e0, family, dtype, flops, nbytes, replay=None, sig=None):
    e1 = torch.cuda.Event(enable_timing=True)
    e1.record()
    PROFILE.append((family, str(dtype), float(flops), float(nbytes), e0, e1, replay, sig))


def conv_variant(T, H, W, cins, cout, kernel, dtype=torch.bfloat16, stride=1, act=ACT_NONE):
    p = ConvParams()
    p.dtype = 1 if dtype == torch.bfloat16 else 0
    p.T, p.H, p.W = T, H, W
    p.KT, p.KH, p.KW = kernel
    p.Cout = cout
    p.nseg = len(cins)
    for i, c in enumerate(cins):
        p.seg_c[i] = c
        p.seg_ld[i] = c
    p.stride = stride
    p.y_ld = cout
    p.act = act
    return lib().flair_conv_variant(ctypes.byref(p))


def _conv_ws_bytes(p):
    return lib().flair_conv_workspace_bytes(ctypes.byref(p))


def pack_conv_weight(w, seg_channels, dtype, cout_pad=None):
    cout, cin = w.shape[:2]
    taps = 1
    for k in w.shape[2:]:
        taps *= k
    w = w.reshape(cout, cin, taps).permute(0, 2, 1).float()
    parts, o = [], 0
    for real, padded in seg_channels:
        seg = w[:, :, o:o + real]
        if padded > real:
            seg = torch.cat([seg, seg.new_zeros(cout, taps, padded - real)], dim=2)
        parts.append(seg)
        o += real
    assert o == cin, (o, cin)
    w = torch.cat(parts, dim=2)
    if cout_pad is not None and cout_pad > cout:
        w = torch.cat([w, w.new_zeros(cout_pad - cout, taps, w.shape[2])], dim=0)
    return w.to(dtype).contiguous()


def chain_supported(xs, c_mid):
    x0 = xs[0] if isinstance(xs, (list, tuple)) else xs
    T, H, W, _ = x0.shape
    tiles = T * ((H + 7) // 8) * (W // 32 if W % 32 == 0 and T * ((H + 7) // 8) * (W // 32) >= 192 else W // 8)
    return c_mid in (64, 128) and W % 8 == 0 and tiles <= 512


def conv_chain(xs, wA, bA, actA, wB, bB, actB, c_mid, coutB, *, res0=None, res1=None, out_scale=1.0, out=None,
               act_param=0.0, act_period=0):
    if isinstance(xs, torch.Tensor):
        xs = [xs]
    x0 = xs[0]
    T, H, W, _ = x0.shape
    p = ChainParams()
    p.dtype = dtype_code(x0)
    p.T, p.H, p.W = T, H, W
    p.C, p.CoutB = c_mid, coutB
    p.nseg = len(xs)
    arr = (ctypes.c_void_p * 4)()
    for i, x in enumerate(xs):
        assert x.dtype == x0.dtype and x.shape[:3] == x0.shape[:3]
        p.seg_c[i] = x.shape[3]
        p.seg_ld[i] = _ld(x)
        arr[i] = x.data_ptr()
    if out is None:
        out = torch.empty((T, H, W, coutB), dtype=x0.dtype, device=x0.device)
    assert tuple(out.shape[:3]) == (T, H, W) and out.shape[3] >= coutB and out.dtype == x0.dtype
    p.y_ld = _ld(out)
    p.res_ld[0] = _ld(res0) if res0 is not None else 0
    p.res_ld[1] = _ld(res1) if res1 is not None else 0
    p.actA, p.actB = actA, actB
    p.act_param, p.act_period = act_param, act_period
    p.out_scale = out_scale
    assert wB.dtype == x0.dtype and wB.is_contiguous() and (wA is None or (wA.dtype == x0.dtype and wA.is_contiguous()))
    e0 = _prof_begin()

    def launch(_keep=xs):
        call.flair_conv_chain(ctypes.byref(p), arr, wA, _dense(bA), wB, _dense(bB), res0, res1, out)
    launch()
    if e0 is not None:
        cin = sum(x.shape[3] for x in xs)
        esz = x0.element_size()
        px = T * H * W
        flops = 2.0 * 9 * px * (c_mid * coutB + (cin * c_mid if wA is not None else 0))
        nbytes = esz * (px * (cin + coutB * (1 + (res0 is not None) + (res1 is not None)))
                        + 9 * c_mid * coutB + (9 * cin * c_mid if wA is not None else 0))
        _prof_end(e0, ("chain", 2 if wA is not None else 1, c_mid), x0.dtype, flops, nbytes, launch,
                  ("chain", T, H, W, tuple(x.shape[3] for x in xs), c_mid, coutB, wA is not None, res0 is not None,
                   res1 is not None))
    return out


_gn_ws = {}


def _workspace(nbytes, device, tag="gn"):
    key = (tag, device, torch.cuda.current_stream().cuda_stream)
    buf = _gn_ws.get(key)
    if buf is None or buf.numel() < nbytes:
        buf = torch.empty(max(nbytes, 1 << 20), dtype=torch.uint8, device=device)
        _gn_ws[key] = buf
    return buf


def group_norm(x, gamma, beta, *, x1=None, groups=32, eps=1e-5, act=ACT_NONE, film=None,
               frames_per_stat=None, resample=0, out=None, want_raw=False):
    T, H, W, c0 = x.shape
    C = c0 + (x1.shape[3] if x1 is not None else 0)
    p = GnParams()
    p.dtype = dtype_code(x)
    p.C, p.c0 = C, c0
    p.ld0 = _ld(x)
    p.ld1 = _ld(x1) if x1 is not None else 0
    p.groups = groups
    p.F, p.H, p.W = T, H, W
    p.frames_per_stat = frames_per_stat or T
    p.eps = eps
    p.act = act
    p.resample = resample
    Ho, Wo = (H // 2, W // 2) if resample == 1 else ((H * 2, W * 2) if resample == 2 else (H, W))
    if out is None:
        out = torch.empty((T, Ho, Wo, C), dtype=x.dtype, device=x.device)
    raw = torch.empty((T, Ho, Wo, C), dtype=x.dtype, device=x.device) if want_raw else None
    p.y_ld = _ld(out)
    p.raw_ld = _ld(raw) if raw is not None else 0
    p.film_ld = film.stride(0) if film is not None else 0
    if film is not None:
        assert film.dtype == torch.float32 and film.stride(1) == 1 and film.shape[0] == T
    ws = _workspace(lib_ws_bytes(p), x.device)
    e0 = _prof_begin()

    def launch():
        call.flair_groupnorm_nhwc(ctypes.byref(p), x, x1, _dense(gamma), _dense(beta), film, out, raw, ws)
    launch()
    if e0 is not None:
        numel_in, numel_out = T * H * W * C, T * Ho * Wo * C
        _prof_end(e0, ("gn",), x.dtype, 8.0 * numel_in,
                  x.element_size() * (2 * numel_in + numel_out * (2 if want_raw else 1)), launch,
                  ("gn", T, H, W, C, c0, groups, p.frames_per_stat, act, resample, want_raw, film is not None))
    return (out, raw) if want_raw else out


def lib_ws_bytes(p):
    return lib().flair_groupnorm_workspace_bytes(ctypes.byref(p))


def nchw_to_clip(src, dst, coff=0):
    N, C, H, W = src.shape
    assert src.dtype == torch.float32 and src.is_contiguous()
    call.flair_nchw_f32_to_nhwc(src, N, C, H, W, dst, dtype_code(dst), _ld(dst), coff)
    return dst


def clip_to_nchw(src, C, coff=0, out=None):
    N, H, W, _ = src.shape
    if out is None:
        out = torch.empty((N, C, H, W), dtype=torch.float32, device=src.device)
    call.flair_nhwc_to_nchw_f32(src, dtype_code(src), _ld(src), coff, N, C, H, W, out)
    return out


def timestep_embedding(t, dim, max_period=10000.0, out=None, sin_first=False):
    assert t.dtype == torch.float32 and t.is_contiguous()
    N = t.shape[0]
    if out is None:
        out = torch.empty((N, dim), dtype=torch.float32, device=t.device)
    call.flair_timestep_embedding(t, N, dim, max_period, sin_first, out)
    return out


def linear(x, w, b, *, act_in=ACT_NONE, act_out=ACT_NONE, out=None):
    M, K = x.shape
    N = w.shape[0]
    assert x.dtype == torch.float32 and w.dtype == torch.float32 and x.is_contiguous() and w.is_contiguous()
    if out is None:
        out = torch.empty((M, N), dtype=torch.float32, device=x.device)
    call.flair_linear_f32(x, M, K, w, b, N, act_in, act_out, out, out.stride(0))
    return out


def qkv_attention(qkv, heads, *, new_order=False, out=None):
    F_, H, W, C3 = qkv.shape
    C = C3 // 3
    p = AttnParams()
    p.dtype = dtype_code(qkv)
    p.frames, p.L, p.heads, p.head_dim = F_, H * W, heads, C // heads
    p.ld = _ld(qkv)
    if out is None:
        out = torch.empty((F_, H, W, C), dtype=qkv.dtype, device=qkv.device)
    p.out_ld = _ld(out)
    d = C // heads
    if new_order:
        p.q_off, p.k_off, p.v_off, p.head_stride = 0, C, 2 * C, d
    else:
        p.q_off, p.k_off, p.v_off, p.head_stride = 0, d, 2 * d, 3 * d
    p.scale = 1.0 / (d ** 0.5)
    e0 = _prof_begin()

    def launch():
        call.flair_qkv_attention(ctypes.byref(p), qkv, out)
    launch()
    if e0 is not None:
        L = H * W
        _prof_end(e0, ("attn", L), qkv.dtype, 4.0 * F_ * heads * L * L * d, qkv.element_size() * 4.0 * F_ * L * C,
                  launch, ("attn", F_, L, heads, d, new_order))
    return out


def temporal_attention(qkv, kpos, window, *, round_fp16, head_dim=64, out=None):
    T, H, W, C3 = qkv.shape
    C = C3 // 3
    p = TAttnParams()
    p.dtype = dtype_code(qkv)
    p.T, p.H, p.W, p.C, p.window = T, H, W, C, window
    p.ld = _ld(qkv)
    if out is None:
        out = torch.empty((T, H, W, C), dtype=qkv.dtype, device=qkv.device)
    p.out_ld = _ld(out)
    p.round_fp16 = round_fp16
    p.head_dim = head_dim
    p.scale = 1.0 / (head_dim ** 0.5)
    assert kpos.shape == (window - 1, C)
    call.flair_temporal_attention(ctypes.byref(p), qkv, _dense(kpos), out)
    return out


def flow_warp(x, flow, *, border=False, out=None):
    F_, H, W, C = x.shape
    assert flow.dtype == torch.float32 and flow.shape == (F_, H, W, 2)
    if out is None:
        out = torch.empty((F_, H, W, C), dtype=x.dtype, device=x.device)
    call.flair_flow_warp(x, dtype_code(x), _ld(x), flow, _ld(flow), F_, H, W, C, border, out, _ld(out))
    return out


def flow_compose(f1, f2, out=None):
    F_, H, W, _ = f1.shape
    assert f1.dtype == torch.float32 and f1.is_contiguous() and f2.is_contiguous()
    if out is None:
        out = torch.empty_like(f1)
    call.flair_flow_compose(f1, f2, F_, H, W, out)
    return out


RESIZE_BILINEAR, RESIZE_BILINEAR_AC, RESIZE_BICUBIC, RESIZE_AVGPOOL2, RESIZE_NEAREST = 0, 1, 2, 3, 4


def resize(x, size, mode, *, channels=None, out=None, scale_c0=1.0, scale_c1=1.0):
    F_, Hi, Wi, Cx = x.shape
    C = channels or Cx
    Ho, Wo = size
    if out is None:
        out = torch.zeros((F_, Ho, Wo, Cx), dtype=x.dtype, device=x.device)
    call.flair_resize_nhwc(x, dtype_code(x), _ld(x), F_, Hi, Wi, C, mode, Ho, Wo, out, _ld(out), scale_c0, scale_c1)
    return out


def dcn_raw_permutation(groups):
    G = groups
    perm = torch.empty(27 * G, dtype=torch.long)
    for k in range(9):
        for g in range(G):
            for e in range(2):
                perm[3 * G * k + 2 * g + e] = 2 * (g * 9 + k) + e
            perm[3 * G * k + 2 * G + g] = 18 * G + g * 9 + k
    return perm


def dcn_align(x0, x1, raw, flow1, flow2, weight, bias, cout, *, groups=16, max_mag=10.0, out=None, raw_activated=False):
    F_, H, W, ch = x0.shape
    p = DcnParams()
    p.dtype = dtype_code(x0)
    p.F, p.H, p.W = F_, H, W
    p.Cin, p.Cout, p.G = 2 * ch, cout, groups
    p.x_ld[0], p.x_ld[1] = _ld(x0), _ld(x1)
    p.raw_ld = _ld(raw)
    if out is None:
        out = torch.empty((F_, H, W, cout), dtype=x0.dtype, device=x0.device)
    p.y_ld = _ld(out)
    p.max_residue_magnitude = max_mag
    p.raw_activated = raw_activated
    e0 = _prof_begin()

    def launch():
        call.flair_dcn_align(ctypes.byref(p), x0, x1, raw, flow1, flow2, weight, _dense(bias), out)
    launch()
    if e0 is not None:
        px = F_ * H * W
        _prof_end(e0, ("dcn", cout), x0.dtype, px * (2.0 * 9 * 2 * ch * cout + 9.0 * 2 * ch * 8),
                  x0.element_size() * px * (2 * ch + 27 * groups + cout), launch,
                  ("dcn", F_, H, W, ch, cout, groups, flow2 is not None))
    return out


def dcn_pack(x, raw, weight, bias, cout, *, groups, out=None):
    c = x.shape[3]
    assert c % 2 == 0
    return dcn_align(x[..., :c // 2], x[..., c // 2:], raw, None, None, weight, bias, cout, groups=groups, out=out,
                     raw_activated=2)


def scale_pixels(x, wmap):
    T, H, W, C = x.shape
    call.flair_scale_pixels(x, dtype_code(x), _ld(x), C, T * H * W, _dense(wmap))
    return x


def predict_xstart(x, model_out, c_recip, c_recipm1, clip, out=None):
    N, C, H, W = x.shape
    Cm = model_out.shape[1]
    assert x.dtype == torch.float32 and x.is_contiguous() and model_out.is_contiguous()
    if out is None:
        out = torch.empty_like(x)
    call.flair_predict_xstart(x, model_out, N, C, Cm, H, W, c_recip, c_recipm1, clip, out)
    return out


def sampler_update(coefs, x, x0, restored, aux, z, prev_recon, out=None):
    if out is None:
        out = torch.empty_like(x)
    for t in (x, x0, restored, aux, z, prev_recon):
        assert t is None or (t.dtype == torch.float32 and t.is_contiguous())
    call.flair_sampler_update(ctypes.byref(coefs), x, x0, restored, aux, z, prev_recon, x.numel(), out)
    return out


def affine_channels(x, C, a, b, lo, hi, sub, mul, out):
    T, H, W, _ = x.shape
    assert x.dtype == torch.float32 and out.dtype == torch.float32
    call.flair_affine_channels_f32(x, _ld(x), C, T * H * W, a, b, lo, hi, sub, mul, out, _ld(out))
    return out


def add_frame_bias(x, bias):
    T, H, W, C = x.shape
    assert bias.dtype == torch.float32 and bias.stride(1) == 1
    call.flair_add_frame_bias(x, dtype_code(x), _ld(x), C, T, H * W, bias, bias.stride(0))
    return x


def cast_channels(src, dst, coff=0):
    T, H, W, C = src.shape
    assert src.dtype == torch.float32
    call.flair_cast_channels(src, _ld(src), C, T * H * W, dst, dtype_code(dst), _ld(dst), coff)
    return dst


def axpby(x, y, a, b, out=None, lo=float("-inf"), hi=float("inf")):
    assert x.dtype == torch.float32 and x.is_contiguous() and (y is None or y.is_contiguous())
    if out is None:
        out = torch.empty_like(x)
    call.flair_axpby_f32(x, y, a, b, lo, hi, x.numel(), out)
    return out


def learned_range_variance(model_out, C, min_log, max_log, out=None):
    N, C2, H, W = model_out.shape
    if out is None:
        var = torch.empty((N, C, H, W), dtype=torch.float32, device=model_out.device)
        logvar = torch.empty_like(var)
    else:
        var, logvar = out
        assert all(t.dtype == torch.float32 and t.is_contiguous() and t.shape == (N, C, H, W) for t in out)
    call.flair_learned_range_variance(model_out, N, C, H, W, min_log, max_log, var, logvar)
    return var, logvar


def depthwise_filter(x, filt, *, pad, out_stride=1, out_offset=0, stuff=1, stuff_offset=0, out_hw=None,
                     reflect=False, out=None):
    N, C, H, W = x.shape
    assert x.dtype == torch.float32 and x.is_contiguous() and filt.dtype == torch.float32 and filt.is_contiguous()
    Ho, Wo = out_hw
    if out is None:
        out = torch.empty((N, C, Ho, Wo), dtype=torch.float32, device=x.device)
    assert out.dtype == torch.float32 and out.is_contiguous() and out.shape == (N, C, Ho, Wo)
    call.flair_depthwise_filter(x, N * C, H, W, filt, filt.shape[0], filt.shape[1], pad, out_stride, out_offset, stuff,
         stuff_offset, Ho, Wo, reflect, out)
    return out


def jpeg_roundtrip(x, q_luma, q_chroma, dct8, want_levels=False, entry="hw", out=None, levels=None, workspace=None):
    N, C, H, W = x.shape
    assert C == 3 and x.dtype == torch.float32 and x.is_contiguous()
    if H % 16 or W % 16:
        raise ValueError(f"jpeg_roundtrip: the codec works on whole 16x16 MCUs, got {H}x{W}")
    if entry not in ("hw", "square"):
        raise ValueError(f"jpeg_roundtrip: unknown entry {entry!r}")
    arr = ctypes.c_float * 64
    tables = [arr(*[float(v) for v in t]) for t in (q_luma, q_chroma, dct8)]
    if out is None:
        out = torch.empty_like(x)
    if levels is not None:
        want_levels = True
        luma, chroma = levels
    else:
        luma = torch.empty((N, 1, H, W), dtype=torch.float32, device=x.device) if want_levels else None
        chroma = torch.empty((N, 2, H // 2, W // 2), dtype=torch.float32, device=x.device) if want_levels else None
    for t, shape in ((out, (N, 3, H, W)), (luma, (N, 1, H, W)), (chroma, (N, 2, H // 2, W // 2)), (workspace, (N, 3, H, W))):
        assert t is None or (t.dtype == torch.float32 and t.is_contiguous() and t.shape == shape), (t.shape, shape)
    if entry == "square":
        if H != W:
            raise ValueError(f"jpeg_roundtrip: the square entry cannot take {H}x{W}")
        ws = torch.empty_like(x) if workspace is None else workspace
        call.flair_jpeg_roundtrip(x, N, H, *tables, ws, out, luma, chroma)
    else:
        call.flair_jpeg_roundtrip_hw(x, N, H, W, *tables, out, luma, chroma)
    return (out, [luma, chroma]) if want_levels else out


def matmul(a, b, out=None):
    assert a.dtype == torch.float32 and b.dtype == torch.float32 and a.is_contiguous() and b.is_contiguous()
    batch = a.shape[0] if a.dim() == 3 else (b.shape[0] if b.dim() == 3 else 1)
    M, K = a.shape[-2:]
    N = b.shape[-1]
    assert b.shape[-2] == K
    if out is None:
        out = torch.empty((batch, M, N), dtype=torch.float32, device=a.device)
    assert out.dtype == torch.float32 and out.is_contiguous() and out.shape == (batch, M, N)
    call.flair_matmul_f32(a, M * K if a.dim() == 3 else 0, b, K * N if b.dim() == 3 else 0, out, batch, M, N, K)
    return out


def gather_mac(x, outer, lin, inner, fov, w, out=None):
    taps, lout = fov.shape
    assert x.dtype == torch.float32 and x.is_contiguous() and fov.dtype == torch.int32 and w.dtype == torch.float32
    if out is None:
        out = torch.empty((outer, lout, inner), dtype=torch.float32, device=x.device)
    assert out.dtype == torch.float32 and out.is_contiguous() and out.shape == (outer, lout, inner)
    call.flair_gather_mac_f32(x, outer, lin, inner, fov.contiguous(), w.contiguous(), taps, lout, out)
    return out


def vsrpp_prep(prop, feat2, flow1, flow_prev, cond1, cond2, flow2_out, flowpad):
    _, H, W, C = prop.shape
    second = flow_prev is not None
    e0 = _prof_begin()

    def launch():
        call.flair_vsrpp_prep(prop, _ld(prop), feat2 if second else None, _ld(feat2) if second else 0, _dense(flow1),
             _dense(flow_prev), dtype_code(prop), H, W, C, cond1, _ld(cond1), cond2 if second else None,
             _ld(cond2) if second else 0, flow2_out if second else None, flowpad, _ld(flowpad))
    launch()
    if e0 is not None:
        n = 2 if second else 1
# ... 770 lines not shown
```

Before: 0.8980.

## Skip all-zero input segments in conv, chain and DCN kernels

Input segments that would be all-zero tensors (the initial propagation state and the absent second-order features in the BasicVSR++ propagation) can now be passed as None. The conv, chain and DCN kernels drop those segments from the K loop, using per-segment weight offsets (segK) so the packed weights are still indexed correctly. This removes the loads and MFMA work spent multiplying zeros, and the zero-tensor allocations. The risk is that im2col conv variants are rejected with null segments, and the new DCN staging path for the one-half case must be correct.

After: 0.9024, median of 6. Within noise of the previous version (+0.5%).

```diff
diff --git a/flair_amd/csrc/chain.hip b/flair_amd/csrc/chain.hip
--- a/flair_amd/csrc/chain.hip
+++ b/flair_amd/csrc/chain.hip
@@ -16,6 +16,7 @@
     float actParam; int actPeriod;
     void* y; int yLd;
     int T, H, W;
+    int segK[4], CinAct;
 };
 
 template <int N>
@@ -90,7 +91,7 @@
     }
     uint4 hreg[2][HI], wreg[2][WI];
 
-    int seg = 0, cb = 0, segOff = 0;
+    int seg = 0, cb = 0;
     auto issue_in = [&](int set) {
         const unsigned ld = (unsigned)a.segLd[seg] * ESZ;
         const char* frame = reinterpret_cast<const char*>(a.x[seg]) + (size_t)frameOff * ld;
@@ -104,7 +105,6 @@
         ++cb;
         if (cb * BKE >= a.segC[seg]) {
             cb = 0;
-            segOff += a.segC[seg];
             ++seg;
         }
     };
@@ -162,11 +162,11 @@
 
     if constexpr (HASA) {
         const __amdgpu_buffer_rsrc_t wArs = make_rsrc(a.wA, a.wABytes);
-        const int nkA = a.CinA / BKE;
+        const int nkA = a.CinAct / BKE;
         auto issue_step = [&](int k, int set) {
             if (k < nkA) {
                 issue_in(set);
-                issue_w(set, wArs, 0, C, a.CinA, segOff + cb * BKE);
+                issue_w(set, wArs, 0, C, a.CinA, a.segK[seg] + cb * BKE);
                 advance_in();
             } else if (k == nkA) {
                 issue_w(set, wBrs, 0, a.CoutB, C, 0);
@@ -831,20 +831,23 @@
     FLAIR_CHECK(p->CoutB > 0 && p->CoutB % (16 / esz) == 0 && p->CoutB <= CHAIN_MAX_COUTB,
                 "flair_conv_chain: CoutB %d must be a multiple of %d and at most %d", p->CoutB, 16 / esz, CHAIN_MAX_COUTB);
     ChainArgs a{};
-    int cin = 0;
-    for (int i = 0; i < p->nseg; ++i) {
-        FLAIR_CHECK(x[i], "flair_conv_chain: segment %d is null", i);
+    int cin = 0, nPresent = 0;
+    for (int i = 0; i < p->nseg; cin += p->seg_c[i], ++i) {
         FLAIR_CHECK(p->seg_c[i] > 0 && p->seg_c[i] % bke == 0, "flair_conv_chain: segment %d has %d channels; must be a "
                     "multiple of %d", i, p->seg_c[i], bke);
+        if (!x[i]) continue;
         FLAIR_CHECK(p->seg_ld[i] >= p->seg_c[i] && (p->seg_ld[i] * esz) % 16 == 0 && ((uintptr_t)x[i]) % 16 == 0,
                     "flair_conv_chain: segment %d stride/alignment", i);
         const unsigned long long bytes = (unsigned long long)p->H * p->W * p->seg_ld[i] * esz;
         FLAIR_CHECK(bytes < 0x40000000ull, "flair_conv_chain: one frame of segment %d spans %llu bytes (limit 1 GiB)", i, bytes);
-        a.x[i] = x[i]; a.segC[i] = p->seg_c[i]; a.segLd[i] = p->seg_ld[i]; a.segBytes[i] = (unsigned)bytes;
-        cin += p->seg_c[i];
-    }
-    a.nseg = p->nseg;
+        const int n = nPresent++;
+        a.x[n] = x[i]; a.segC[n] = p->seg_c[i]; a.segLd[n] = p->seg_ld[i]; a.segBytes[n] = (unsigned)bytes;
+        a.segK[n] = cin;
+        a.CinAct += p->seg_c[i];
+    }
+    a.nseg = nPresent;
     const bool hasA = wA != nullptr;
+    FLAIR_CHECK(nPresent == p->nseg || (hasA && nPresent > 0), "flair_conv_chain: a null input segment needs stage A and at least one present segment");
     FLAIR_CHECK(hasA || (p->nseg == 1 && cin == p->C), "flair_conv_chain: without stage A the single input must have C channels");
     a.wA = wA; a.biasA = biasA; a.actA = p->actA; a.CinA = cin;
     a.wABytes = (unsigned)((unsigned long long)p->C * 9 * cin * esz);
diff --git a/flair_amd/csrc/conv.hip b/flair_amd/csrc/conv.hip
--- a/flair_amd/csrc/conv.hip
+++ b/flair_amd/csrc/conv.hip
@@ -38,6 +38,8 @@
     int actPeriod;
     int Hin, Win;
     int esz;
+    int segK[4];
+    int CinAct;
 };
 
 __device__ __forceinline__ int lds_off(int row, int chunk) {
@@ -211,7 +213,7 @@
     const int pt = a.KT / 2;
 
     uint4 hreg[PF][HI], wreg[PF][WI];
-    int dt = -pt, seg = 0, cb = 0, segOff = 0;
+    int dt = -pt, seg = 0, cb = 0;
     auto dt_valid = [&](int d) { return (unsigned)(t + d) < (unsigned)a.T; };
     while (dt <= pt && !dt_valid(dt)) ++dt;
 
@@ -248,7 +250,7 @@
             const unsigned off = hpix[i] >= 0 ? (unsigned)hpix[i] * ld + cofs + hq[i] : FLAIR_OOB;
             hr[i] = buf_load16(xr, off);
         }
-        const unsigned kofs = (unsigned)((dt + pt) * 9 * a.CinTot + segOff + cb * BKE) * ESZ;
+        const unsigned kofs = (unsigned)((dt + pt) * 9 * a.CinTot + a.segK[seg] + cb * BKE) * ESZ;
 #pragma unroll
         for (int i = 0; i < WI; ++i) wr[i] = buf_load16(wrs, woff[i] == FLAIR_OOB ? FLAIR_OOB : woff[i] + kofs);
     };
@@ -256,10 +258,8 @@
         ++cb;
         if (cb * BKE >= a.segC[seg]) {
             cb = 0;
-            segOff += a.segC[seg];
             if (++seg >= a.nseg) {
                 seg = 0;
-                segOff = 0;
                 ++dt;
                 while (dt <= pt && !dt_valid(dt)) ++dt;
             }
@@ -280,7 +280,7 @@
     };
     int nValidDt = 0;
     for (int d = -pt; d <= pt; ++d) nValidDt += dt_valid(d) ? 1 : 0;
-    const int nch = nValidDt * (a.CinTot / BKE);
+    const int nch = nValidDt * (a.CinAct / BKE);
 
     f32x16 acc[RPW][2];
 #pragma unroll
@@ -492,7 +492,7 @@
         for (int e = 0; e < VEC; ++e) biasv[e] = (a.bias && bco < a.Cout) ? a.bias[bco + e] : 0.f;
     }
     uint4 hreg[HI], wreg[WI];
-    int dt = -pt, seg = 0, cb = 0, segOff = 0;
+    int dt = -pt, seg = 0, cb = 0;
     auto dt_valid = [&](int d) { return (unsigned)(t + d) < (unsigned)a.T; };
     while (dt <= pt && !dt_valid(dt)) ++dt;
 
@@ -525,16 +525,14 @@
 #pragma unroll
         for (int i = 0; i < HI; ++i)
             hreg[i] = buf_load16(xr, hpix[i] >= 0 ? (unsigned)hpix[i] * ld + cofs + hq[i] : FLAIR_OOB);
-        const unsigned kofs = (unsigned)((dt + pt) * 9 * a.CinTot + segOff + cb * BKE) * ESZ;
+        const unsigned kofs = (unsigned)((dt + pt) * 9 * a.CinTot + a.segK[seg] + cb * BKE) * ESZ;
 #pragma unroll
         for (int i = 0; i < WI; ++i) wreg[i] = buf_load16(wrs, woff[i] == FLAIR_OOB ? FLAIR_OOB : woff[i] + kofs);
         ++cb;
         if (cb * BKE >= a.segC[seg]) {
             cb = 0;
-            segOff += a.segC[seg];
             if (++seg >= a.nseg) {
                 seg = 0;
-                segOff = 0;
                 ++dt;
                 while (dt <= pt && !dt_valid(dt)) ++dt;
             }
@@ -557,7 +555,7 @@
     };
     int nValidDt = 0;
     for (int d = -pt; d <= pt; ++d) nValidDt += dt_valid(d) ? 1 : 0;
-    const int nch = nValidDt * (a.CinTot / BKE);
+    const int nch = nValidDt * (a.CinAct / BKE);
 
     f32x16 acc[2];
 #pragma unroll
@@ -722,7 +720,7 @@
     const int wave = __builtin_amdgcn_readfirstlane(tid >> 6);
     const int lr = lane & 31, lh = lane >> 5;
     const int taps = a.KT * 9, pt = a.KT / 2;
-    const int chunksPerTap = a.CinTot / 32;
+    const int chunksPerTap = a.CinAct / 32;
     const int H = a.H, W = a.W, T = a.T;
 
     const int xcd = blockIdx.x & 7, slot = blockIdx.x >> 3, slotsPerXcd = gridDim.x >> 3;
@@ -775,11 +773,11 @@
 
     const u32x4_t wdesc = make_desc(a.w, a.wBytes);
     struct Walk {
-        int dt, seg, cb, segOff, j;
+        int dt, seg, cb, j;
     };
     auto dt_at = [&](int t, int j) { return a.tFast ? (j + a.KT * T - t) % a.KT - pt : j - pt; };
     auto walk_first = [&](int t, Walk& wk) {
-        wk.j = 0; wk.seg = 0; wk.cb = 0; wk.segOff = 0;
+        wk.j = 0; wk.seg = 0; wk.cb = 0;
         while (wk.j < a.KT && (unsigned)(t + dt_at(t, wk.j)) >= (unsigned)T) ++wk.j;
         wk.dt = dt_at(t, wk.j);
     };
@@ -787,10 +785,8 @@
         ++wk.cb;
         if (wk.cb * 32 >= a.segC[wk.seg]) {
             wk.cb = 0;
-            wk.segOff += a.segC[wk.seg];
             if (++wk.seg >= a.nseg) {
                 wk.seg = 0;
-                wk.segOff = 0;
                 ++wk.j;
                 while (wk.j < a.KT && (unsigned)(t + dt_at(t, wk.j)) >= (unsigned)T) ++wk.j;
                 wk.dt = dt_at(t, wk.j);
@@ -807,7 +803,7 @@
         const char* frame = reinterpret_cast<const char*>(a.x[wk.seg]) + (size_t)(tl.t + wk.dt) * H * W * ld;
         const u32x4_t xdesc = make_desc(frame, a.segBytes[wk.seg]);
         const unsigned cofs = (unsigned)(wk.cb * 64);
-        const unsigned kofs = (unsigned)((wk.dt + pt) * 9 * a.CinTot + wk.segOff + wk.cb * 32) * 2u;
+        const unsigned kofs = (unsigned)((wk.dt + pt) * 9 * a.CinTot + a.segK[wk.seg] + wk.cb * 32) * 2u;
         const unsigned sbase = (unsigned)(stage * STAGE_BYTES + wave * NSLOT * 1024);
 #pragma unroll
         for (int i = 0; i < NSLOT; ++i) {
@@ -1157,7 +1153,7 @@
     const int bid = xcd_remap(blockIdx.x, gridDim.x);
     const int t = bid / perFrame, tile = bid - t * perFrame;
     const int h0 = (tile / tilesW) * 8, w0 = (tile % tilesW) * 32;
-    const int nS = a.CinTot / 32;
+    const int nS = a.CinAct / 32;
 
     const u32x4_t wdesc = make_desc(a.w, a.wBytes);
     const u32x4_t bdesc = make_desc(a.bias, a.bias ? (unsigned)a.Cout * 4u : 0u);
@@ -1187,11 +1183,17 @@
             ++hseg;
         }
     };
+    int wseg = 0, wcb = 0;
     auto issue_w = [&](int s_) {
+        const unsigned kofs = (unsigned)(a.segK[wseg] + wcb * 32) * 2u;
 #pragma unroll
         for (int i = 0; i < NWS; ++i) {
             const int id = (wave * NWS + i) % WINSTR;
-            dma16(wdesc, wlane[i] == FLAIR_OOB ? FLAIR_OOB : wlane[i] + (unsigned)(s_ * 64), (unsigned)(RING + (s_ % WR) * SLOT + id * 1024));
+            dma16(wdesc, wlane[i] == FLAIR_OOB ? FLAIR_OOB : wlane[i] + kofs, (unsigned)(RING + (s_ % WR) * SLOT + id * 1024));
+        }
+        if (++wcb * 32 >= a.segC[wseg]) {
+            wcb = 0;
+            ++wseg;
         }
     };
     issue_halo(0);
@@ -1612,6 +1614,8 @@
 int dispatch(const ConvArgs& a0, hipStream_t s) {
     ConvArgs a = a0;
     const ConvVariant variant = choose_variant(a);
+    FLAIR_CHECK(a.CinAct == a.CinTot || variant > IGEMM_64x64,
+                "flair_conv_nhwc: a null input segment needs a 3x3 halo / LDS-DMA form (variant 3..9); this geometry takes im2col variant %d", (int)variant);
     a.splitK = a.part ? choose_split(a, variant) : 1;
     switch (variant) {
         case IGEMM_128x128: return launch<E, 128, 128, 2, 2>(a, s);
@@ -1671,21 +1675,26 @@
     const int esz = p->dtype == FLAIR_BF16 ? 2 : 4;
     ConvArgs a{};
     fill_geometry(a, p);
-    for (int i = 0; i < p->nseg; ++i) {
-        FLAIR_CHECK(x[i], "flair_conv_nhwc: segment %d is null", i);
+    int nPresent = 0, kOff = 0;
+    for (int i = 0; i < p->nseg; kOff += p->seg_c[i], ++i) {
         FLAIR_CHECK(p->seg_c[i] > 0 && p->seg_c[i] % bke == 0,
                     "flair_conv_nhwc: segment %d has %d channels; must be a multiple of %d", i, p->seg_c[i], bke);
+        if (!x[i]) continue;
         FLAIR_CHECK(p->seg_ld[i] >= p->seg_c[i] && (p->seg_ld[i] * esz) % 16 == 0 &&
                         ((uintptr_t)x[i]) % 16 == 0,
                     "flair_conv_nhwc: segment %d stride/alignment", i);
-        a.x[i] = x[i];
-        a.segC[i] = p->seg_c[i];
-        a.segLd[i] = p->seg_ld[i];
+        const int n = nPresent++;
+        a.x[n] = x[i];
+        a.segC[n] = p->seg_c[i];
+        a.segLd[n] = p->seg_ld[i];
+        a.segK[n] = kOff;
+        a.CinAct += p->seg_c[i];
         const unsigned long long bytes = (unsigned long long)p->H * p->W * p->seg_ld[i] * esz;
         FLAIR_CHECK(bytes < 0x40000000ull, "flair_conv_nhwc: one frame of segment %d spans %llu bytes (limit 1 GiB)",
                     i, bytes);
-        a.segBytes[i] = (unsigned)bytes;
-    }
+        a.segBytes[n] = (unsigned)bytes;
+    }
+    FLAIR_CHECK(nPresent > 0, "flair_conv_nhwc: every input segment is null (at least one must be present)");
     {
         const unsigned long long wb = (unsigned long long)p->Cout * p->KT * p->KH * p->KW * a.CinTot * esz;
         FLAIR_CHECK(wb < 0x80000000ull, "flair_conv_nhwc: weights span %llu bytes (limit 2 GiB)", wb);
@@ -1702,7 +1711,7 @@
                 p->res_ld[1], p->Cout, gran);
     FLAIR_CHECK(((uintptr_t)w) % 16 == 0, "flair_conv_nhwc: weight alignment");
     FLAIR_CHECK(!bias || ((uintptr_t)bias) % 16 == 0, "flair_conv_nhwc: bias alignment");
-    a.nseg = p->nseg;
+    a.nseg = nPresent;
     a.w = w;
     a.bias = bias;
     a.fbias = frame_bias;
diff --git a/flair_amd/csrc/dcn.hip b/flair_amd/csrc/dcn.hip
--- a/flair_amd/csrc/dcn.hip
+++ b/flair_amd/csrc/dcn.hip
@@ -123,11 +123,12 @@
     int cpgShift = 0;
     while ((1 << cpgShift) < cpg) ++cpgShift;
     const int halfC = a.Cin / 2;
-    const int cbPerTap = a.Cin / BKE;
+    const bool have2 = a.x[1] != nullptr;
+    const int cbPerTap = have2 ? a.Cin / BKE : halfC / BKE;
     const int nk = 9 * cbPerTap;
     const size_t fo0 = ONEFRAME ? (size_t)pf * a.H * a.W * a.xLd[0] * ESZ : 0, fo1 = ONEFRAME ? (size_t)pf * a.H * a.W * a.xLd[1] * ESZ : 0;
     const __amdgpu_buffer_rsrc_t xr0 = make_rsrc(reinterpret_cast<const char*>(a.x[0]) + fo0, a.xBytes[0]);
-    const __amdgpu_buffer_rsrc_t xr1 = make_rsrc(reinterpret_cast<const char*>(a.x[1]) + fo1, a.xBytes[1]);
+    const __amdgpu_buffer_rsrc_t xr1 = have2 ? make_rsrc(reinterpret_cast<const char*>(a.x[1]) + fo1, a.xBytes[1]) : xr0;
     const __amdgpu_buffer_rsrc_t wrs = make_rsrc(a.w, a.wBytes);
     const unsigned frameBase = (unsigned)pf * a.H * a.W;
 
@@ -325,8 +326,16 @@
         }
     };
 #pragma unroll
-    for (int u = 0; u < PFD - 1; ++u)
+    for (int u = 0; u < PFD - 1; ++u) {
         if (u < nk) issue(rs[u]);
+        if (stageAt == u - (PFD - 1) && stageTap < 9) {
+            __syncthreads();
+            stage_raw(stageTap);
+            ++stageTap;
+            stageAt += cbPerTap;
+            __syncthreads();
+        }
+    }
     constexpr int UNR = 2 * PFD;
     for (int k = 0; k < nk; k += UNR) {
 #pragma unroll
@@ -502,11 +511,13 @@
 extern "C" int flair_dcn_align(const flair_dcn_params* p, const void* x0, const void* x1, const void* raw,
                                const float* flow1, const float* flow2, const void* w, const float* bias, void* y,
                                hipStream_t stream) {
-    FLAIR_CHECK(p && x0 && x1 && raw && w && y, "flair_dcn_align: null argument");
+    FLAIR_CHECK(p && x0 && raw && w && y, "flair_dcn_align: null argument");
     FLAIR_CHECK_DTYPE("flair_dcn_align", p->dtype);
     FLAIR_CHECK(p->raw_activated >= 0 && p->raw_activated <= 2, "flair_dcn_align: raw_activated = %d (0, 1 or 2)", p->raw_activated);
     const bool vqfr = p->raw_activated == 2;
     FLAIR_CHECK(!vqfr || (!flow1 && !flow2), "flair_dcn_align: raw_activated = 2 takes no flows");
+    FLAIR_CHECK(x1 || !vqfr, "flair_dcn_align: raw_activated = 2 takes both input halves (x1 is null)");
+    const int xLd1 = x1 ? p->x_ld[1] : p->x_ld[0];
     const int vec = p->dtype == FLAIR_BF16 ? 8 : 4;
     const int bke = vqfr ? vqfr_tile(p).bke : vec * (p->Cout <= 64 && p->dtype != FLAIR_BF16 ? 4 : 8);
     const int esz = p->dtype == FLAIR_BF16 ? 2 : 4;
@@ -518,13 +529,13 @@
                     (p->raw_ld * esz) % 16 == 0,
                 "flair_dcn_align: Cout = %d (a multiple of 4, <= 128; <= 1024 with raw_activated = 2) / raw_ld = %d (>= 27 G, "
                 "16-byte granular)", p->Cout, p->raw_ld);
-    FLAIR_CHECK(p->x_ld[0] >= p->Cin / 2 && p->x_ld[1] >= p->Cin / 2 && (p->x_ld[0] * esz) % 16 == 0 &&
-                    (p->x_ld[1] * esz) % 16 == 0 && ((uintptr_t)x0) % 16 == 0 && ((uintptr_t)x1) % 16 == 0 &&
+    FLAIR_CHECK(p->x_ld[0] >= p->Cin / 2 && xLd1 >= p->Cin / 2 && (p->x_ld[0] * esz) % 16 == 0 &&
+                    (xLd1 * esz) % 16 == 0 && ((uintptr_t)x0) % 16 == 0 && ((uintptr_t)x1) % 16 == 0 &&
                     ((uintptr_t)raw) % 16 == 0 && p->y_ld >= p->Cout,
                 "flair_dcn_align: strides/alignment (x_ld = %d, %d: >= Cin / 2 = %d, 16-byte granular; x0, x1, raw 16-byte "
-                "aligned; y_ld = %d >= Cout = %d)", p->x_ld[0], p->x_ld[1], p->Cin / 2, p->y_ld, p->Cout);
+                "aligned; y_ld = %d >= Cout = %d)", p->x_ld[0], xLd1, p->Cin / 2, p->y_ld, p->Cout);
     DcnArgs a;
-    a.x[0] = x0; a.x[1] = x1; a.xLd[0] = p->x_ld[0]; a.xLd[1] = p->x_ld[1];
+    a.x[0] = x0; a.x[1] = x1; a.xLd[0] = p->x_ld[0]; a.xLd[1] = xLd1;
     a.Cin = p->Cin; a.raw = raw; a.rawLd = p->raw_ld; a.flow1 = flow1; a.flow2 = flow2;
     a.w = w; a.bias = bias; a.y = y; a.yLd = p->y_ld;
     a.F = p->F; a.H = p->H; a.W = p->W; a.Cout = p->Cout; a.G = p->G; a.maxMag = p->max_residue_magnitude;
@@ -532,11 +543,11 @@
     a.P = (long)p->F * p->H * p->W;
     const unsigned long long half = p->Cin / 2;
     const unsigned long long b0 = ((unsigned long long)(a.P - 1) * p->x_ld[0] + half) * esz;
-    const unsigned long long b1 = ((unsigned long long)(a.P - 1) * p->x_ld[1] + half) * esz;
+    const unsigned long long b1 = ((unsigned long long)(a.P - 1) * xLd1 + half) * esz;
     const unsigned long long br = ((unsigned long long)(a.P - 1) * p->raw_ld + 27 * p->G) * esz;
     const unsigned long long by = (unsigned long long)a.P * p->y_ld * esz;
     FLAIR_CHECK(b0 < 0x80000000ull && b1 < 0x80000000ull && br < 0x80000000ull && by < 0x80000000ull, "flair_dcn_align: tensor spans >= 2 GiB");
-    FLAIR_CHECK(a.P + 2l * p->W + 2 < (1l << 23) && (long)p->x_ld[0] * esz < (1l << 23) && (long)p->x_ld[1] * esz < (1l << 23),
+    FLAIR_CHECK(a.P + 2l * p->W + 2 < (1l << 23) && (long)p->x_ld[0] * esz < (1l << 23) && (long)xLd1 * esz < (1l << 23),
                 "flair_dcn_align: F*H*W = %ld pixels (limit 2^23 per call: call per frame)", a.P);
     a.xBytes[0] = (unsigned)b0; a.xBytes[1] = (unsigned)b1; a.rawBytes = (unsigned)((br + 15) / 16 * 16);
     a.wBytes = (unsigned)((unsigned long long)p->Cout * 9 * p->Cin * esz);
diff --git a/flair_amd/guided_diffusion/unet_new.py b/flair_amd/guided_diffusion/unet_new.py
--- a/flair_amd/guided_diffusion/unet_new.py
+++ b/flair_amd/guided_diffusion/unet_new.py
@@ -311,6 +311,8 @@
 
 class BasicVSRPP(nn.Module):
 
+    zero_fill_absent = False
+
     def __init__(self, mid_channels=64, max_residue_magnitude=10, use_checkpoint=False):
         super().__init__()
         self.mid_channels = mid_channels
@@ -341,7 +343,7 @@
         if "backward" in name:
             order = order[::-1]
             flow_idx = order
-        zero_c = torch.zeros((1, H, W, c), dtype=ctx.dtype, device=ctx.device)
+        absent = torch.zeros((1, H, W, c), dtype=ctx.dtype, device=ctx.device) if self.zero_fill_absent else None
         ka = ops.k_align(ctx.dtype)
         k3 = (1, 3, 3)
         G = self.deform_align[name].deform_groups
@@ -350,15 +352,15 @@
         key = (name, H, W, ctx.dtype, ka)
         cached = store.get(key) if store is not None else None
         fill = [] if (cached is None and store is not None) else None
-        prop, prev2 = zero_c, None
+        prop, prev2 = None, None
         for i, idx in enumerate(order):
             cur = hidden[idx:idx + 1]
             if i > 0:
                 flow_n1 = flows[flow_idx[i]:flow_idx[i] + 1]
-                cond_n1 = torch.empty_like(zero_c)
+                cond_n1 = torch.empty((1, H, W, c), dtype=ctx.dtype, device=ctx.device)
                 second = i > 1
-                feat_n2 = prev2 if second else zero_c
-                cond_n2 = torch.empty_like(zero_c) if second else zero_c
+                feat_n2 = prev2 if second else absent
+                cond_n2 = torch.empty_like(cond_n1) if second else absent
                 if cached is not None:
                     flow_n2, flowpad = cached[i - 1]
                     ops.vsrpp_warp2(prop, feat_n2 if second else None, flow_n1, flow_n2, cond_n1, cond_n2 if second else None)
@@ -387,7 +389,7 @@
                                         groups=G, max_mag=mag, raw_activated=True)
 
             else:
-                aligned = zero_c
+                aligned = absent
             segs = [cur] + [o_[idx:idx + 1] for o_ in others] + [aligned]
             new = run_trunk(pk_t, segs, c, extra_res=aligned, out=dest[idx:idx + 1], out_scale=weight)
             if wmaps is not None:
diff --git a/flair_amd/ops.py b/flair_amd/ops.py
--- a/flair_amd/ops.py
+++ b/flair_amd/ops.py
@@ -42,7 +42,7 @@
          out_scale=1.0, stride=1, frame_bias=None, act_param=0.0, act_period=0, asym_pad=False, reflect_pad=False):
     if isinstance(xs, torch.Tensor):
         xs = [xs]
-    x0 = xs[0]
+    x0, seg_c = _segments(xs, lambda: weight.shape[-1])
     T, H, W, _ = x0.shape
     p = ConvParams()
     p.dtype = dtype_code(x0)
@@ -52,8 +52,10 @@
     p.nseg = len(xs)
     arr = (ctypes.c_void_p * 4)()
     for i, x in enumerate(xs):
+        p.seg_c[i] = seg_c[i]
+        if x is None:
+            continue
         assert x.dtype == x0.dtype and x.shape[:3] == x0.shape[:3]
-        p.seg_c[i] = x.shape[3]
         p.seg_ld[i] = _ld(x)
         arr[i] = x.data_ptr()
     p.stride = stride
@@ -81,16 +83,31 @@
         call.flair_conv_nhwc(ctypes.byref(p), arr, weight, _dense(bias), frame_bias, res0, res1, out, ws, wsb)
     launch()
     if e0 is not None:
-        cin = sum(x.shape[3] for x in xs)
+        cin = sum(x.shape[3] for x in xs if x is not None)
         taps = kernel[0] * kernel[1] * kernel[2]
         esz = x0.element_size()
         flops = 2.0 * T * Ho * Wo * cout * cin * taps
         nbytes = esz * (cin * T * H * W + cout * T * Ho * Wo * (1 + (res0 is not None) + (res1 is not None))
                         + cout * taps * cin)
         _prof_end(e0, ("conv", lib().flair_conv_variant(ctypes.byref(p))), x0.dtype, flops, nbytes, launch,
-                  ("conv", T, H, W, tuple(x.shape[3] for x in xs), cout, tuple(kernel), stride, act,
+                  ("conv", T, H, W, _seg_sig(xs, seg_c), cout, tuple(kernel), stride, act,
                    res0 is not None, res1 is not None, frame_bias is not None))
     return out
+
+
+def _segments(xs, cin_packed):
+    present = [x for x in xs if x is not None]
+    assert present, "every input segment is None"
+    n_absent = len(xs) - len(present)
+    if n_absent == 0:
+        return xs[0], [x.shape[3] for x in xs]
+    rest = cin_packed() - sum(x.shape[3] for x in present)
+    assert rest > 0 and rest % n_absent == 0, (cin_packed(), [None if x is None else x.shape[3] for x in xs])
+    return present[0], [rest // n_absent if x is None else x.shape[3] for x in xs]
+
+
+def _seg_sig(xs, seg_c):
+    return tuple(-c if x is None else c for x, c in zip(xs, seg_c))
 
 
 PROFILE = None
@@ -161,7 +178,7 @@
                act_param=0.0, act_period=0):
     if isinstance(xs, torch.Tensor):
         xs = [xs]
-    x0 = xs[0]
+    x0, seg_c = _segments(xs, lambda: wA.shape[-1] if wA is not None else c_mid)
     T, H, W, _ = x0.shape
     p = ChainParams()
     p.dtype = dtype_code(x0)
@@ -170,8 +187,10 @@
     p.nseg = len(xs)
     arr = (ctypes.c_void_p * 4)()
     for i, x in enumerate(xs):
+        p.seg_c[i] = seg_c[i]
+        if x is None:
+            continue
         assert x.dtype == x0.dtype and x.shape[:3] == x0.shape[:3]
-        p.seg_c[i] = x.shape[3]
         p.seg_ld[i] = _ld(x)
         arr[i] = x.data_ptr()
     if out is None:
@@ -190,14 +209,14 @@
         call.flair_conv_chain(ctypes.byref(p), arr, wA, _dense(bA), wB, _dense(bB), res0, res1, out)
     launch()
     if e0 is not None:
-        cin = sum(x.shape[3] for x in xs)
+        cin = sum(x.shape[3] for x in xs if x is not None)
         esz = x0.element_size()
         px = T * H * W
         flops = 2.0 * 9 * px * (c_mid * coutB + (cin * c_mid if wA is not None else 0))
         nbytes = esz * (px * (cin + coutB * (1 + (res0 is not None) + (res1 is not None)))
                         + 9 * c_mid * coutB + (9 * cin * c_mid if wA is not None else 0))
         _prof_end(e0, ("chain", 2 if wA is not None else 1, c_mid), x0.dtype, flops, nbytes, launch,
-                  ("chain", T, H, W, tuple(x.shape[3] for x in xs), c_mid, coutB, wA is not None, res0 is not None,
+                  ("chain", T, H, W, _seg_sig(xs, seg_c), c_mid, coutB, wA is not None, res0 is not None,
                    res1 is not None))
     return out
 
@@ -384,7 +403,7 @@
     p.dtype = dtype_code(x0)
     p.F, p.H, p.W = F_, H, W
     p.Cin, p.Cout, p.G = 2 * ch, cout, groups
-    p.x_ld[0], p.x_ld[1] = _ld(x0), _ld(x1)
+    p.x_ld[0], p.x_ld[1] = _ld(x0), _ld(x1) if x1 is not None else 0
     p.raw_ld = _ld(raw)
     if out is None:
         out = torch.empty((F_, H, W, cout), dtype=x0.dtype, device=x0.device)
@@ -398,9 +417,10 @@
     launch()
     if e0 is not None:
         px = F_ * H * W
-        _prof_end(e0, ("dcn", cout), x0.dtype, px * (2.0 * 9 * 2 * ch * cout + 9.0 * 2 * ch * 8),
-                  x0.element_size() * px * (2 * ch + 27 * groups + cout), launch,
-                  ("dcn", F_, H, W, ch, cout, groups, flow2 is not None))
+        halves = 2 if x1 is not None else 1
+        _prof_end(e0, ("dcn", cout), x0.dtype, px * (2.0 * 9 * halves * ch * cout + 9.0 * halves * ch * 8),
+                  x0.element_size() * px * (halves * ch + 27 * groups + cout), launch,
+                  ("dcn", F_, H, W, ch, cout, groups, flow2 is not None, x1 is not None))
     return out
 
 
```
